# fferflo/semantic-meshes

Measured on AMD Instinct MI355X. Metric: views/sec fused (1080p, 19 classes, 1M-tri mesh), higher is better.
Workload: dtype f32; 1 GPU; cfg2: 1000000-triangle grid mesh, 11763 views/GPU at 1920x1080, 19 classes, probs resident in HBM; views_per_call=8, group_pipeline=True, repeats=1, allreduce=none, exchange=allreduce, nranks=1, allreduce_bytes=0, exchange_parts=1, held_views=0

## Files before the change

semantic_meshes_amd/csrc/common.hpp:

```cpp
#pragma once

#include <hip/hip_runtime.h>

#include <algorithm>
#include <cstdint>
#include <cstdio>
#include <cstdlib>
#include <functional>
#include <mutex>
#include <string>
#include <vector>

#include "../../include/smesh.h"

namespace smesh {

int fail(int code, const std::string& msg);
int fail_hip(hipError_t e, const char* what, const char* file, int line);

#define SMESH_HIP(expr)                                                         \
  do {                                                                          \
    hipError_t _e = (expr);                                                     \
    if (_e != hipSuccess) return ::smesh::fail_hip(_e, #expr, __FILE__, __LINE__); \
  } while (0)

#define SMESH_TRY(expr)              \
  do {                               \
    int _s = (expr);                 \
    if (_s != SMESH_OK) return _s;   \
  } while (0)

struct ProfSlot {
  std::vector<std::pair<hipEvent_t, hipEvent_t>> pending;
  std::vector<std::pair<hipEvent_t, hipEvent_t>> pool;
  double total_ms = 0.0;
  uint64_t launches = 0;
  uint64_t seen = 0;
  int depth = 0;
  bool open_timed = false;
  uint64_t timed_launches = 0;
  uint64_t timed_views = 0;
};

struct DeviceCtx {
  int device = -1;
  hipStream_t stream = nullptr;
  hipStream_t raster_stream = nullptr;
  hipStream_t exchange_stream = nullptr;
  hipEvent_t ev_order = nullptr;
  hipEvent_t ev_release = nullptr;
  int num_cus = 256;
  uint32_t lds_per_cu = 65536;
  unsigned profiling = 0;
  unsigned profile_every = 1;
  ProfSlot slots[SMESH_PROF_SLOTS];
  hipEvent_t marks[SMESH_STREAM_MARKS] = {};
  std::vector<hipEvent_t> token_pool;
  std::recursive_mutex mu;
};

int get_ctx(int device, DeviceCtx** out);

struct ProfScope {
  DeviceCtx* ctx;
  int slot;
  hipEvent_t start = nullptr, stop = nullptr;
  hipStream_t st;
  bool counted = false;
  ProfScope(DeviceCtx* c, int s, hipStream_t stream = nullptr);
  ~ProfScope();
};

void prof_note(DeviceCtx* ctx, int slot, uint64_t launches, uint64_t views);

hipError_t dev_malloc(void** out, size_t bytes);
hipError_t dev_free(void* p, bool foreign = false);
uint64_t dev_cached_bytes(int device);
void dev_trim(int device);
void dev_cache_stats(uint64_t* live_blocks, uint64_t* cached_blocks, uint64_t* cached_bytes);

bool opt_group_pipeline();
constexpr int kRasterMeshletsDefault = 1;
bool opt_raster_meshlets();
constexpr int kPipelineFitDefault = 1;
constexpr int kPipelineFuseWaves = 5;
int opt_pipeline_fit();
int opt_pipeline_fuse_waves();
int opt_pipeline_fuse_pad();

struct PipelineNeighbour {
  uint32_t wg_lds = 0, wg_vgprs = 0;
};

inline uint32_t pipeline_fuse_pad(uint32_t lds_per_cu, uint32_t static_lds, uint32_t vgprs, int want, const PipelineNeighbour& nb,
                                  int* beside = nullptr) {
  constexpr uint32_t kBlock = 1280u;
  auto blocks = [&](uint32_t bytes) { return (bytes + kBlock - 1u) / kBlock * kBlock; };
  const uint32_t n = (uint32_t)std::min(32, std::max(2, want));
  const uint32_t wg = std::max(blocks(static_lds), (lds_per_cu / (n + 1u)) / kBlock * kBlock + kBlock);
  if (beside) {
    const uint32_t alloc_f = std::max(8u, (vgprs + 7u) / 8u * 8u), alloc_r = std::max(8u, (nb.wg_vgprs + 7u) / 8u * 8u);
    const uint32_t per_simd = (n + 3u) / 4u;
    const uint32_t left = (uint64_t)wg * n <= lds_per_cu ? lds_per_cu - wg * n : 0u;
    const uint32_t regs_left = per_simd * alloc_f < 512u ? 512u - per_simd * alloc_f : 0u;
    const uint32_t by_regs = std::min(regs_left / alloc_r, per_simd < 8u ? 8u - per_simd : 0u);
    *beside = (int)std::min(by_regs, nb.wg_lds ? left / blocks(nb.wg_lds) : by_regs);
  }
  return wg - static_lds;
}
bool opt_confusion_wave_aggregate();

bool opt_probs_labels_tiles();
bool opt_resize_vector();
bool opt_fuse_sampled();
bool opt_points_grid();
constexpr uint32_t kProbsLabelsTileMaxC = 255;

constexpr uint32_t kConfusionLdsMaxC = 180;

struct Scratch {
  void* ptr = nullptr;
  size_t bytes = 0;
  int reserve(size_t need);
  void release();
};

inline uint64_t div_up(uint64_t a, uint64_t b) { return (a + b - 1) / b; }

inline int env_int(const char* name, int def) {
  const char* e = getenv(name);
  return e ? atoi(e) : def;
}

struct TriFrag {
  uint16_t x0, y0;
  uint16_t kind;
  uint16_t pad;
  unsigned long long mask;
};
static_assert(sizeof(TriFrag) == 16, "TriFrag must be 16 bytes");

struct TriFuseArgs {
  const TriFrag* frags;
  const uint32_t* idx;
  const float* probs;
  const float* weights;
  float* acc;
  float* acc_lo;
  uint64_t F;
  uint32_t C, W, H;
  float iew;
  const uint32_t* big_queue;
  const uint32_t* big_len;
  uint32_t big_capacity;
  uint32_t tri_blocks;
  uint32_t big_blocks;
  const uint32_t* prim_id;
  const uint32_t* tex_first;
  const uint32_t* tex_res;
  const uint8_t* tex_kinds;
  uint32_t* count;
  double* acc_d;
  int mid;
  uint32_t ps0, ps1;
  uint32_t blk_first;
  uint32_t f_lo, f_hi;
  uint32_t lds_pad;
};

struct TriView {
  const TriFrag* frags;
  const uint32_t* idx;
  const float* probs;
  const float* weights;
  const uint32_t* big_queue;
  const uint32_t* big_len;
  uint32_t W, H;
  uint32_t ps0, ps1;
  const uint8_t* kinds;
};
template <int NV>
struct TriViews {
  TriView v[NV];
};

struct RenderedView {
  const TriFrag* frags;
  const uint32_t* big_queue;
  const uint32_t* big_len;
  const uint32_t* idx;
  const float* probs;
  const float* weights;
  uint64_t W, H;
  int64_t ps0 = 0, ps1 = 0;
  bool mid_queue = false;
  bool no_big = false;
  const uint8_t* kinds = nullptr;
  bool fine = false;
  PipelineNeighbour beside;
  const void* image = nullptr;
};

constexpr int kMidBox = 256;

struct ImageRecords {
  TriFrag* frags = nullptr;
  uint32_t* cand = nullptr;
  uint4* big4 = nullptr;
  uint32_t* big_queue = nullptr;
  uint32_t* big_count = nullptr;
  unsigned long long* mom = nullptr;
  uint64_t P = 0;
  bool clean = false;
  bool moments = false;
  uint32_t tag = 2;
  void release();
};
int image_records_build(DeviceCtx* ctx, ImageRecords& r, const uint32_t* d_idx, uint64_t W, uint64_t H, uint64_t P);
int image_records_pending(DeviceCtx* ctx, ImageRecords& r, const uint32_t* d_idx, uint64_t W, uint64_t H, hipStream_t st);
int image_records_scatter_sparse(DeviceCtx* ctx, ImageRecords& r, int kind, const uint32_t* d_idx, const float* d_probs, const float* d_w,
                                 uint64_t W, uint64_t H, uint32_t C, float iew, float* acc, float* acc_lo, double* acc_d, hipStream_t st);
int image_records_clear(DeviceCtx* ctx, ImageRecords& r, const uint32_t* d_idx, uint64_t W, uint64_t H, hipStream_t st);
bool image_records_build_group(DeviceCtx* ctx, ImageRecords* const* recs, const uint32_t* const* d_idx, int n, uint64_t W, uint64_t H, uint64_t P,
                               int* status);
int image_records_scatter_sparse_group(DeviceCtx* ctx, ImageRecords* const* recs, int n, int kind, const uint32_t* const* d_idx,
                                       const float* const* d_probs, const float* const* d_w, uint64_t W, uint64_t H, uint32_t C, float iew,
                                       float* acc, float* acc_lo, double* acc_d, hipStream_t st);

}

struct smesh_aggregator;
struct smesh_renderer;
int smesh_aggregator_with_final_rows(smesh_aggregator* a,
                                     const std::function<int(smesh::DeviceCtx* ctx, const float* rows, uint64_t P, uint32_t C)>& use);
int smesh_renderer_texel_tables(const smesh_renderer* r, smesh::DeviceCtx** ctx, uint64_t* F, uint64_t* P, const uint32_t** first,
                                const uint32_t** res);
int smesh_rows_labels(smesh::DeviceCtx* ctx, const float* d_rows, uint64_t n, uint32_t C, float dont_care_threshold, int32_t* out_labels,
                      int out_memkind);
struct smesh_vertex_map;
int smesh_rows_finish(smesh::DeviceCtx* ctx, const float* d_rows, uint64_t n, uint32_t C, int mode, float dont_care_threshold,
                      float* out_rows, int32_t* out_labels, int out_memkind);
int smesh_vertex_map_tables(const smesh_vertex_map* m, smesh::DeviceCtx** ctx, const uint32_t** offsets, const uint32_t** list);
struct smesh_face_graph;
int smesh_face_graph_tables(const smesh_face_graph* graph, smesh::DeviceCtx** ctx, const uint32_t** offsets, const uint32_t** neighbours,
                            uint64_t* F, uint64_t* nnz);
int smesh_renderer_with_index_planes(smesh_renderer* r, const smesh_camera_t* cams, int n, uint64_t P, smesh::DeviceCtx* ctx,
                                     const std::function<int(int view, const uint32_t* idx, uint64_t W, uint64_t H)>& use);
```

semantic_meshes_amd/csrc/context.cpp:

```cpp
#include "common.hpp"
#include "labels_scratch.hpp"
#include "half_scratch.hpp"
#include "../../include/smesh_label_prep.h"
#include "../../include/smesh_label_colors.h"

#include <algorithm>
#include <atomic>

#include <cstdlib>
#include <cstring>
#include <map>
#include <memory>
#include <unordered_map>
#include <vector>

namespace smesh {

static thread_local std::string g_err;

int fail(int code, const std::string& msg) {
  g_err = msg;
  return code;
}

int fail_hip(hipError_t e, const char* what, const char* file, int line) {
  char buf[512];
  snprintf(buf, sizeof buf, "HIP error %d (%s) at %s:%d: %s", (int)e, hipGetErrorString(e), file, line, what);
  g_err = buf;
  (void)hipGetLastError();
  return (e == hipErrorNoDevice || e == hipErrorInvalidDevice) ? SMESH_ERR_NODEVICE : SMESH_ERR_RUNTIME;
}

static std::atomic<int> g_confusion_wave_aggregate{1};
bool opt_confusion_wave_aggregate() { return g_confusion_wave_aggregate.load() != 0; }

static std::atomic<int> g_probs_labels_tiles{1};
bool opt_probs_labels_tiles() { return g_probs_labels_tiles.load() != 0; }

static std::atomic<int> g_resize_vector{1};
bool opt_resize_vector() { return g_resize_vector.load() != 0; }

static std::atomic<int> g_points_grid{1};
bool opt_points_grid() { return g_points_grid.load() != 0; }

uint64_t smesh_label_prep_launches();
uint64_t smesh_label_colors_launches();
uint64_t smesh_depth_weights_launches();
uint64_t smesh_view_weights_launches();

static std::atomic<int> g_fuse_sampled{-1};
bool opt_fuse_sampled() {
  const int v = g_fuse_sampled.load();
  return (v < 0 ? env_int("SMESH_FUSE_SAMPLED", 1) : v) != 0;
}

static std::atomic<int> g_group_pipeline{-1};
bool opt_group_pipeline() {
  int v = g_group_pipeline.load();
  if (v < 0) {
    const char* e = getenv("SMESH_GROUP_PIPELINE");
    v = e ? (atoi(e) != 0 ? 1 : 0) : 1;
    g_group_pipeline.store(v);
  }
  return v != 0;
}

static std::atomic<int> g_raster_meshlets{-1};
bool opt_raster_meshlets() {
  int v = g_raster_meshlets.load();
  if (v < 0) {
    const char* e = getenv("SMESH_RASTER_MESHLETS");
    v = e ? (atoi(e) != 0 ? 1 : 0) : kRasterMeshletsDefault;
    g_raster_meshlets.store(v);
  }
  return v != 0;
}

static std::atomic<int> g_pipeline_fit{-2}, g_pipeline_fuse_waves{-2}, g_pipeline_fuse_pad{-2};
static int opt_env_once(std::atomic<int>& g, const char* env, int def, int lo, int hi) {
  int v = g.load();
  if (v == -2) {
    v = std::min(hi, std::max(lo, env_int(env, def)));
    g.store(v);
  }
  return v;
}
int opt_pipeline_fit() { return opt_env_once(g_pipeline_fit, "SMESH_PIPELINE_FIT", kPipelineFitDefault, 0, 1); }
int opt_pipeline_fuse_waves() { return opt_env_once(g_pipeline_fuse_waves, "SMESH_PIPELINE_FUSE_WAVES", kPipelineFuseWaves, 2, 32); }
int opt_pipeline_fuse_pad() { return opt_env_once(g_pipeline_fuse_pad, "SMESH_PIPELINE_FUSE_PAD", -1, -1, 65536 - 16384); }

static std::mutex g_ctx_mu;
static std::vector<std::unique_ptr<DeviceCtx>> g_ctx;

DeviceCtx* peek_ctx(int device) {
  std::lock_guard<std::mutex> lock(g_ctx_mu);
  return (device >= 0 && device < (int)g_ctx.size()) ? g_ctx[device].get() : nullptr;
}

int get_ctx(int device, DeviceCtx** out) {
  std::lock_guard<std::mutex> lock(g_ctx_mu);
  int n = 0;
  hipError_t e = hipGetDeviceCount(&n);
  if (e != hipSuccess || n <= 0) {
    (void)hipGetLastError();
    return fail(SMESH_ERR_NODEVICE, "no HIP device available (libsmesh_hip has no CPU fallback)");
  }
  if (device < 0 || device >= n) return fail(SMESH_ERR_INVALID, "device index out of range");
  if ((int)g_ctx.size() < n) g_ctx.resize(n);
  if (!g_ctx[device]) {
    SMESH_HIP(hipSetDevice(device));
    auto ctx = std::make_unique<DeviceCtx>();
    ctx->device = device;
    hipDeviceProp_t prop;
    SMESH_HIP(hipGetDeviceProperties(&prop, device));
    ctx->num_cus = prop.multiProcessorCount > 0 ? prop.multiProcessorCount : 256;
    ctx->lds_per_cu = (uint32_t)std::min<size_t>(std::max<size_t>(prop.maxSharedMemoryPerMultiProcessor, 65536), 1u << 20);
    SMESH_HIP(hipStreamCreateWithFlags(&ctx->stream, hipStreamNonBlocking));
    SMESH_HIP(hipStreamCreateWithFlags(&ctx->raster_stream, hipStreamNonBlocking));
    {
      int least = 0, greatest = 0;
      if (hipDeviceGetStreamPriorityRange(&least, &greatest) != hipSuccess) { (void)hipGetLastError(); least = greatest = 0; }
      if (hipStreamCreateWithPriority(&ctx->exchange_stream, hipStreamNonBlocking, greatest) != hipSuccess) {
        (void)hipGetLastError();
        SMESH_HIP(hipStreamCreateWithFlags(&ctx->exchange_stream, hipStreamNonBlocking));
      }
    }
    g_ctx[device] = std::move(ctx);
  }
  *out = g_ctx[device].get();
  return SMESH_OK;
}

ProfScope::ProfScope(DeviceCtx* c, int s, hipStream_t stream) : ctx(c), slot(s), st(stream ? stream : c->stream) {
  if (!(ctx->profiling & (1u << slot))) return;
  ProfSlot& ps = ctx->slots[slot];
  if (ps.depth++ > 0) { counted = true; return; }
  counted = true;
  if (ps.seen++ % (slot <= SMESH_PROF_RASTER ? std::max(1u, ctx->profile_every) : 1u) != 0) return;
  if (!ps.pool.empty()) {
    start = ps.pool.back().first;
    stop = ps.pool.back().second;
    ps.pool.pop_back();
  } else {
    if (hipEventCreate(&start) != hipSuccess || hipEventCreate(&stop) != hipSuccess) {
      start = stop = nullptr;
      return;
    }
  }
  (void)hipEventRecord(start, st);
  ps.open_timed = true;
}

void prof_note(DeviceCtx* ctx, int slot, uint64_t launches, uint64_t views) {
  ProfSlot& ps = ctx->slots[slot];
  if (ps.depth > 0 && ps.open_timed) { ps.timed_launches += launches; ps.timed_views += views; }
}
// ... 94 lines not shown
    std::lock_guard<std::mutex> lock(g_alloc_mu);
    auto it = g_live.find(p);
    if (it != g_live.end()) owner = it->second.device;
  }
  int cur = 0;
  (void)hipGetDevice(&cur);
  if (owner >= 0 && owner != cur) (void)hipSetDevice(owner);
  DeviceCtx* ctx = (owner >= 0 && !foreign) ? peek_ctx(owner) : nullptr;
  hipError_t e = hipSuccess;
  if (ctx) {
    for (hipStream_t st : {ctx->raster_stream, ctx->stream, ctx->exchange_stream})
      if (st && e == hipSuccess) e = hipStreamSynchronize(st);
  } else {
    e = hipDeviceSynchronize();
  }
  if (e != hipSuccess) (void)hipGetLastError();
  hipError_t ret = hipSuccess;
  {
    std::lock_guard<std::mutex> lock(g_alloc_mu);
    auto it = g_live.find(p);
    if (it == g_live.end()) ret = hipFree(p);
    else {
      const DevBlock b = it->second;
      g_live.erase(it);
      const size_t cap = cache_cap(b.device);
      if (b.bytes > cap) ret = hipFree(p);
      else {
        evict_locked(b.device, b.bytes, cap);
        g_cached.emplace(b.bytes, CachedBlock{p, b.device, g_alloc_stamp++});
        g_cached_bytes[b.device] += b.bytes;
      }
    }
  }
  if (owner >= 0 && owner != cur) (void)hipSetDevice(cur);
  return ret;
}

void dev_trim(int device) {
  std::lock_guard<std::mutex> lock(g_alloc_mu);
  for (auto it = g_cached.begin(); it != g_cached.end();) {
    if (device >= 0 && it->second.device != device) { ++it; continue; }
    auto victim = it++;
    really_free_locked(victim);
  }
}

void dev_cache_stats(uint64_t* live_blocks, uint64_t* cached_blocks, uint64_t* cached_bytes) {
  std::lock_guard<std::mutex> lock(g_alloc_mu);
  if (live_blocks) *live_blocks = g_live.size();
  if (cached_blocks) *cached_blocks = g_cached.size();
  if (cached_bytes) { *cached_bytes = 0; for (auto& kv : g_cached_bytes) *cached_bytes += kv.second; }
}
uint64_t dev_cached_bytes(int device) {
  std::lock_guard<std::mutex> lock(g_alloc_mu);
  uint64_t n = 0;
  for (auto& kv : g_cached_bytes) if (device < 0 || kv.first == device) n += kv.second;
  return n;
}

int Scratch::reserve(size_t need) {
  if (need <= bytes) return SMESH_OK;
  if (ptr) SMESH_HIP(dev_free(ptr));
  ptr = nullptr;
  bytes = 0;
  size_t want = need + need / 8 + 256;
  SMESH_HIP(dev_malloc(&ptr, want));
  bytes = want;
  return SMESH_OK;
}

void Scratch::release() {
  if (ptr) (void)dev_free(ptr);
  ptr = nullptr;
  bytes = 0;
}

}

using namespace smesh;

void smesh_last_fuse_instance(int* slot, int* views);
uint32_t smesh_last_fuse_lds_pad();
int smesh_last_fuse_beside();
int smesh_last_fuse_probs_dtype();

extern "C" {

const char* smesh_backend(void) { return "hip-gfx950"; }

const char* smesh_last_error(void) { return g_err.c_str(); }

int smesh_set_option(const char* name, int64_t value) {
  if (!name) return fail(SMESH_ERR_INVALID, "option name is NULL");
  if (!strcmp(name, "group_pipeline")) { g_group_pipeline.store(value != 0 ? 1 : 0); return SMESH_OK; }
  if (!strcmp(name, "raster_meshlets")) { g_raster_meshlets.store(value != 0 ? 1 : 0); return SMESH_OK; }
  if (!strcmp(name, "pipeline_fit")) { g_pipeline_fit.store(value != 0 ? 1 : 0); return SMESH_OK; }
  if (!strcmp(name, "pipeline_fuse_waves")) { g_pipeline_fuse_waves.store((int)std::min<int64_t>(32, std::max<int64_t>(2, value))); return SMESH_OK; }
  if (!strcmp(name, "pipeline_fuse_pad")) { g_pipeline_fuse_pad.store((int)std::min<int64_t>(65536 - 16384, std::max<int64_t>(-1, value))); return SMESH_OK; }
  if (!strcmp(name, "confusion_wave_aggregate")) { g_confusion_wave_aggregate.store(value != 0 ? 1 : 0); return SMESH_OK; }
  if (!strcmp(name, "probs_labels_tiles")) { g_probs_labels_tiles.store(value != 0 ? 1 : 0); return SMESH_OK; }
  if (!strcmp(name, "resize_vector")) { g_resize_vector.store(value != 0 ? 1 : 0); return SMESH_OK; }
  if (!strcmp(name, "fuse_sampled")) { g_fuse_sampled.store(value != 0 ? 1 : 0); return SMESH_OK; }
  if (!strcmp(name, "points_grid")) { g_points_grid.store(value != 0 ? 1 : 0); return SMESH_OK; }
  return fail(SMESH_ERR_INVALID, std::string("unknown option: ") + name);
}
int smesh_get_option(const char* name, int64_t* value) {
  if (!name || !value) return fail(SMESH_ERR_INVALID, "NULL argument");
  if (!strcmp(name, "group_pipeline")) { *value = opt_group_pipeline() ? 1 : 0; return SMESH_OK; }
  if (!strcmp(name, "raster_meshlets")) { *value = opt_raster_meshlets() ? 1 : 0; return SMESH_OK; }
  if (!strcmp(name, "pipeline_fit")) { *value = opt_pipeline_fit(); return SMESH_OK; }
  if (!strcmp(name, "pipeline_fuse_waves")) { *value = opt_pipeline_fuse_waves(); return SMESH_OK; }
  if (!strcmp(name, "pipeline_fuse_pad")) { *value = opt_pipeline_fuse_pad(); return SMESH_OK; }
  if (!strcmp(name, "last_fuse_lds_pad")) { *value = (int64_t)smesh_last_fuse_lds_pad(); return SMESH_OK; }
  if (!strcmp(name, "last_fuse_beside")) { *value = (int64_t)smesh_last_fuse_beside(); return SMESH_OK; }
  if (!strcmp(name, "labels_lds_max_classes")) { *value = (int64_t)kLabelsLdsMaxC; return SMESH_OK; }
  if (!strcmp(name, "half_max_classes")) { *value = (int64_t)kHalfMaxClasses; return SMESH_OK; }
  if (!strcmp(name, "last_fuse_probs_dtype")) { *value = (int64_t)smesh_last_fuse_probs_dtype(); return SMESH_OK; }
  if (!strcmp(name, "confusion_lds_max_classes")) { *value = (int64_t)kConfusionLdsMaxC; return SMESH_OK; }
  if (!strcmp(name, "confusion_wave_aggregate")) { *value = opt_confusion_wave_aggregate() ? 1 : 0; return SMESH_OK; }
  if (!strcmp(name, "probs_labels_tiles")) { *value = opt_probs_labels_tiles() ? 1 : 0; return SMESH_OK; }
  if (!strcmp(name, "resize_vector")) { *value = opt_resize_vector() ? 1 : 0; return SMESH_OK; }
  if (!strcmp(name, "fuse_sampled")) { *value = opt_fuse_sampled() ? 1 : 0; return SMESH_OK; }
  if (!strcmp(name, "points_grid")) { *value = opt_points_grid() ? 1 : 0; return SMESH_OK; }
  if (!strcmp(name, "labels_prepare_map_lds_max")) { *value = (int64_t)SMESH_LABEL_PREP_MAP_LDS_MAX; return SMESH_OK; }
  if (!strcmp(name, "labels_prepare_launches")) { *value = (int64_t)smesh_label_prep_launches(); return SMESH_OK; }
  if (!strcmp(name, "labels_colors_lds_max")) { *value = (int64_t)SMESH_LABEL_COLORS_LDS_MAX; return SMESH_OK; }
  if (!strcmp(name, "labels_colors_launches")) { *value = (int64_t)smesh_label_colors_launches(); return SMESH_OK; }
  if (!strcmp(name, "depth_weights_launches")) { *value = (int64_t)smesh_depth_weights_launches(); return SMESH_OK; }
  if (!strcmp(name, "view_weights_launches")) { *value = (int64_t)smesh_view_weights_launches(); return SMESH_OK; }
  if (!strcmp(name, "probs_labels_tile_max_classes")) { *value = (int64_t)kProbsLabelsTileMaxC; return SMESH_OK; }
  const bool want_slot = !strcmp(name, "last_fuse_slot");
  if (want_slot || !strcmp(name, "last_fuse_views")) {
    int slot, views;
    smesh_last_fuse_instance(&slot, &views);
    *value = want_slot ? slot : views;
    return SMESH_OK;
  }
  return fail(SMESH_ERR_INVALID, std::string("unknown option: ") + name);
}

int smesh_device_count(int* count) {
  if (!count) return fail(SMESH_ERR_INVALID, "count is NULL");
  int n = 0;
  if (hipGetDeviceCount(&n) != hipSuccess) {
    (void)hipGetLastError();
    n = 0;
  }
  *count = n;
  return SMESH_OK;
}

int smesh_synchronize(int device) {
  DeviceCtx* ctx;
  SMESH_TRY(get_ctx(device, &ctx));
  SMESH_HIP(hipSetDevice(device));
  SMESH_HIP(hipStreamSynchronize(ctx->raster_stream));
  SMESH_HIP(hipStreamSynchronize(ctx->stream));
  SMESH_HIP(hipStreamSynchronize(ctx->exchange_stream));
  return SMESH_OK;
}

int smesh_stream_wait(int device, void* producer_stream) {
  DeviceCtx* ctx;
  SMESH_TRY(get_ctx(device, &ctx));
  std::lock_guard<std::recursive_mutex> lock(ctx->mu);
  SMESH_HIP(hipSetDevice(device));
  hipStream_t ps = static_cast<hipStream_t>(producer_stream);
  if (ps == ctx->raster_stream) return SMESH_OK;
  if (!ctx->ev_order) SMESH_HIP(hipEventCreateWithFlags(&ctx->ev_order, hipEventDisableTiming));
  SMESH_HIP(hipEventRecord(ctx->ev_order, ps));
  if (ps != ctx->stream) SMESH_HIP(hipStreamWaitEvent(ctx->stream, ctx->ev_order, 0));
  SMESH_HIP(hipStreamWaitEvent(ctx->raster_stream, ctx->ev_order, 0));
  return SMESH_OK;
}

int smesh_stream_release(int device, void* consumer_stream) {
  DeviceCtx* ctx;
  SMESH_TRY(get_ctx(device, &ctx));
  std::lock_guard<std::recursive_mutex> lock(ctx->mu);
  SMESH_HIP(hipSetDevice(device));
  hipStream_t cs = static_cast<hipStream_t>(consumer_stream);
  if (cs == ctx->stream) return SMESH_OK;
  if (!ctx->ev_release) SMESH_HIP(hipEventCreateWithFlags(&ctx->ev_release, hipEventDisableTiming));
  SMESH_HIP(hipEventRecord(ctx->ev_release, ctx->stream));
  SMESH_HIP(hipStreamWaitEvent(cs, ctx->ev_release, 0));
  return SMESH_OK;
}

int smesh_stream_handle(int device, void** stream) {
  if (!stream) return fail(SMESH_ERR_INVALID, "stream is NULL");
  DeviceCtx* ctx;
  SMESH_TRY(get_ctx(device, &ctx));
// ... 212 lines not shown
```

semantic_meshes_amd/csrc/fuse_mid.inc.hpp:

```cpp

constexpr int kMidHits = 256;
constexpr int kRowRor1 = 0x121, kRowRor2 = 0x122, kRowRor4 = 0x124, kRowRor8 = 0x128;

__device__ __forceinline__ float row16_sum(float v) {
  v += dpp_f<kRowRor8>(0.0f, v);
  v += dpp_f<kRowRor4>(0.0f, v);
  v += dpp_f<kRowRor2>(0.0f, v);
  v += dpp_f<kRowRor1>(0.0f, v);
  return v;
}
__device__ __forceinline__ uint32_t row16_sum_u(uint32_t v) {
  v += dpp_u<kRowRor8>(0u, v);
  v += dpp_u<kRowRor4>(0u, v);
  v += dpp_u<kRowRor2>(0u, v);
  v += dpp_u<kRowRor1>(0u, v);
  return v;
}
__device__ __forceinline__ float row16_max(float v) {
  v = fmaxf(v, dpp_f<kRowRor8>(-INFINITY, v));
  v = fmaxf(v, dpp_f<kRowRor4>(-INFINITY, v));
  v = fmaxf(v, dpp_f<kRowRor2>(-INFINITY, v));
  v = fmaxf(v, dpp_f<kRowRor1>(-INFINITY, v));
  return v;
}
__device__ __forceinline__ double row16_sum_d(double v) {
#define SMESH_ROR_D(CTRL)                                                                               \
  {                                                                                                     \
    const int hi = __builtin_amdgcn_update_dpp(0, __double2hiint(v), CTRL, 0xF, 0xF, false);            \
    const int lo = __builtin_amdgcn_update_dpp(0, __double2loint(v), CTRL, 0xF, 0xF, false);            \
    v += __hiloint2double(hi, lo);                                                                      \
  }
  SMESH_ROR_D(kRowRor8) SMESH_ROR_D(kRowRor4) SMESH_ROR_D(kRowRor2) SMESH_ROR_D(kRowRor1)
#undef SMESH_ROR_D
  return v;
}

typedef __attribute__((address_space(3))) uint16_t lds_u16;
template <int CT, int KIND, int NV>
__device__ __forceinline__ void fuse_mid_entries(const TriFuseArgs& a, const TriViews<NV>& vw, const uint32_t worker, const uint32_t nworkers,
                                                 lds_u16* __restrict__ hit_lds) {
  static_assert(KIND != SMESH_AGG_MUL, "fuse_mid_entries adds with float atomics: Sum and Summax only");
  const int C = (int)a.C;
  const int l16 = (int)(threadIdx.x & 15u);
  const uint32_t slot = worker * 4u + (threadIdx.x >> 4), nslots = nworkers * 4u;
  uint32_t len[NV], total = 0u;
#pragma unroll
  for (int v = 0; v < NV; v++) { len[v] = min(vw.v[v].big_len[3], a.big_capacity); total += len[v]; }
  if (total == 0u) return;
  lds_u16* __restrict__ my_hits = hit_lds + ((threadIdx.x >> 4) & 3u) * kMidHits;
  struct Entry { uint32_t fi; int view; TriFrag rec; };
  auto fetch = [&](const uint32_t q) -> Entry {
    Entry e;
    e.fi = 0u; e.view = -1;
    e.rec.x0 = 0; e.rec.y0 = 0; e.rec.kind = 0; e.rec.pad = 0; e.rec.mask = 0ull;
    uint32_t qq = q;
    int jsel = -1;
    bool located = q >= total;
#pragma unroll
    for (int j = 0; j < NV; j++) {
      if (!located) {
        if (qq < len[j]) { jsel = j; located = true; }
        else qq -= len[j];
      }
    }
    if (jsel >= 0) {
      const TriView& w = vw.v[jsel];
      e.fi = w.big_queue[(uint64_t)a.big_capacity + qq];
      e.rec = w.frags[e.fi];
      e.view = jsel;
    }
    return e;
  };
  Entry next = fetch(slot);
  for (uint32_t q0 = 0; q0 < total; q0 += nslots) {
    const uint32_t q = q0 + slot;
    const Entry cur = next;
    next = fetch(q + nslots);
    const uint32_t fi = cur.fi;
    const TriFrag rec = cur.rec;
    const TriView& cw = vw.v[cur.view >= 0 ? cur.view : 0];
    const uint32_t* __restrict__ idx = cw.idx;
    const float* __restrict__ probs = cw.probs;
    const float* __restrict__ weights = cw.weights;
    const uint32_t vH = cw.H, ps0 = cw.ps0, ps1 = cw.ps1;
    const bool on = cur.view >= 0 && rec.kind == 2 && mid_box(rec, 0u, 0u);
    if (__ballot(on) == 0ull) continue;
    const uint32_t pid = (a.prim_id && on) ? a.prim_id[fi] : fi;
    const int x0 = rec.x0, y0 = rec.y0;
    const int x1 = (int)(rec.mask & 0xFFFFu), y1 = (int)((rec.mask >> 16) & 0xFFFFu);
    const int bh = on ? y1 - y0 + 1 : 1;
    const int npx = on ? (x1 - x0 + 1) * bh : 0;
    unsigned long long hits = 0ull;
    {
      int cx = l16 / bh, cy = l16 - cx * bh;
      for (int base = 0; __ballot(base < npx) != 0ull; base += 16 * 8) {
        uint32_t got[8];
#pragma unroll
        for (int u = 0; u < 8; u++) {
          const bool in = base + u * 16 + l16 < npx;
          got[u] = idx[(uint64_t)(uint32_t)(x0 + (in ? cx : 0)) * vH + (uint32_t)(y0 + (in ? cy : 0))];
          if (!in) got[u] = ~pid;
          cy += 16;
          while (cy >= bh) { cy -= bh; cx++; }
        }
#pragma unroll
        for (int u = 0; u < 8; u++) if (got[u] == pid) hits |= 1ull << (base / 16 + u);
      }
    }
    const uint32_t mine_n = (uint32_t)__popcll(hits);
    const uint32_t ntot = row16_sum_u(mine_n);
    const float w0 = ntot ? a.iew * (1.0f / (float)ntot) + (1 - a.iew) * 1.0f : 0.0f;
    uint32_t incl = mine_n;
    incl += dpp_u<kDppRowShr1>(0u, incl);
    incl += dpp_u<kDppRowShr2>(0u, incl);
    incl += dpp_u<kDppRowShr4>(0u, incl);
    incl += dpp_u<kDppRowShr8>(0u, incl);
    const bool compact = ntot <= (uint32_t)kMidHits;
    if (compact) {
      uint32_t at = incl - mine_n;
      for (unsigned long long m = hits; m; m &= m - 1ull) my_hits[at++] = (uint16_t)(l16 + 16 * (__ffsll((long long)m) - 1));
    }
    wave_sync();
    float tri[CT];
#pragma unroll
    for (int c = 0; c < CT; c++) tri[c] = 0.0f;
    const float inv_bh = 1.0f / (float)bh;
    uint32_t round = 0u;
    while (true) {
      bool have;
      int i;
      if (compact) {
        const uint32_t e = round * 16u + (uint32_t)l16;
        have = e < ntot;
        i = have ? (int)my_hits[e] : 0;
      } else {
        have = hits != 0ull;
        i = have ? l16 + 16 * (__ffsll((long long)hits) - 1) : 0;
        hits &= hits - 1ull;
      }
      round++;
      if (__ballot(have) == 0ull) break;
      int ix = (int)(((float)i + 0.5f) * inv_bh);
      int iy = i - ix * bh;
      if (iy < 0) { ix--; iy += bh; } else if (iy >= bh) { ix++; iy -= bh; }
      const uint32_t hx = (uint32_t)(x0 + ix), hy = (uint32_t)(y0 + iy);
      float p[CT];
      load_row<CT, false>(probs + ((uint64_t)hx * ps0 + (uint64_t)hy * ps1), C, p);
      const float wt = (weights && have) ? weights[(uint64_t)hx * vH + hy] : 1.0f;
      float sum = 0.0f;
#pragma unroll
      for (int c = 0; c < CT; c++) if (c < C) sum = sum + p[c];
// ... 34 lines not shown
```

semantic_meshes_amd/csrc/fuse_tri.inc.hpp:

```cpp

constexpr int kWave = 64;

__device__ __forceinline__ float log_spec(float x) {
  if (!(x > 0.0f)) return x == 0.0f ? -INFINITY : NAN;
  if (x == INFINITY) return INFINITY;
  int e_adj = 0;
  uint32_t ix = __float_as_uint(x);
  if (ix < 0x00800000u) { x = x * 8388608.0f; e_adj = -23; ix = __float_as_uint(x); }
  int e = (int)(ix >> 23) - 127 + e_adj;
  uint32_t im = (ix & 0x007FFFFFu) | 0x3F800000u;
  if ((ix & 0x007FFFFFu) > 0x003504F3u) { im -= 0x00800000u; e += 1; }
  const float f = __uint_as_float(im) - 1.0f;
  const float z = f * f;
  float y = 7.0376836292e-2f;
  y = __builtin_fmaf(y, f, -1.1514610310e-1f);
  y = __builtin_fmaf(y, f, 1.1676998740e-1f);
  y = __builtin_fmaf(y, f, -1.2420140846e-1f);
  y = __builtin_fmaf(y, f, 1.4249322787e-1f);
  y = __builtin_fmaf(y, f, -1.6668057665e-1f);
  y = __builtin_fmaf(y, f, 2.0000714765e-1f);
  y = __builtin_fmaf(y, f, -2.4999993993e-1f);
  y = __builtin_fmaf(y, f, 3.3333331174e-1f);
  y = (y * f) * z;
  const float fe = (float)e;
// ... 189 lines not shown
    if (KIND == SMESH_AGG_SUMMAX) {
      float best = p[0];
      int am = 0;
#pragma unroll
      for (int c = 1; c < CT; c++) if (EXACT || c < C) if (p[c] > best) { best = p[c]; am = c; }
#pragma unroll
      for (int c = 0; c < CT; c++) if (EXACT || c < C) part[c] = (c == am) ? part[c] + p[c] * w : part[c];
    } else {
#pragma unroll
      for (int c = 0; c < CT; c++) if (EXACT || c < C) part[c] += (bpart_t)contribution<KIND>(p[c], w);
    }
  };
  if (one_step && n <= (uint32_t)kWave) {
    uint32_t at = upto - mine_n;
#pragma unroll
    for (int u = 0; u < U; u++)
      if (hits & (1u << u)) lds_list[at++] = (uint32_t)pix_of((long long)u * kWave + l);
    wave_sync();
    const bool hit = (uint32_t)l < n;
    const uint64_t pix = lds_list[hit ? l : 0];
    wave_sync();
    float p[CT];
    load_row<CT, EXACT>(probs_at(pix), C, p);
    const float wt = (a.weights && hit) ? a.weights[pix] : 1.0f;
    accumulate(p, hit, wt);
    float* rows = reinterpret_cast<float*>(lds_list);
    if (hit) {
#pragma unroll
      for (int c = 0; c < CT; c++) if (EXACT || c < C) rows[l * C + c] = (float)part[c];
    }
    wave_sync();
    bpart_t col = (bpart_t)0;
    if (l < C)
      for (uint32_t j = 0; j < n; j++) col += (bpart_t)rows[j * (uint32_t)C + (uint32_t)l];
    wave_sync();
    if (l < C) write_back(col);
    return;
  } else {
    for (long long base = 0; base < npx; base += (long long)kWave * U) {
      uint64_t pix[U];
      bool hit[U];
#pragma unroll
      for (int u = 0; u < U; u++) {
        const long long i = base + (long long)u * kWave + l;
        pix[u] = i < npx ? pix_of(i) : pix_of(0);
        hit[u] = a.idx[pix[u]] == f && i < npx;
      }
      float p[U][CT];
      float wt[U];
#pragma unroll
      for (int u = 0; u < U; u++) {
        const float* __restrict__ pr = probs_at(hit[u] ? pix[u] : pix_of(0));
        load_row<CT, EXACT>(pr, C, p[u]);
        wt[u] = (a.weights && hit[u]) ? a.weights[pix[u]] : 1.0f;
      }
#pragma unroll
      for (int u = 0; u < U; u++) accumulate(p[u], hit[u], wt[u]);
    }
  }
  bpart_t mine = (bpart_t)0;
#pragma unroll
  for (int c = 0; c < CT; c++) if (EXACT || c < C) {
    bpart_t v;
    if constexpr (KIND == SMESH_AGG_MUL) v = wave_sum_d(part[c]); else v = wave_sum(part[c]);
    if (l == c) mine = v;
  }
  if (l < C) write_back(mine);
}

__device__ __forceinline__ TriFuseArgs with_view(const TriFuseArgs& a, const TriView& w) {
  TriFuseArgs x = a;
  x.frags = w.frags; x.idx = w.idx; x.probs = w.probs; x.weights = w.weights; x.big_queue = w.big_queue; x.big_len = w.big_len;
  x.W = w.W; x.H = w.H; x.ps0 = w.ps0; x.ps1 = w.ps1;
  return x;
}

__device__ __forceinline__ bool mid_box(const TriFrag& rec, uint32_t W, uint32_t H) {
  (void)W; (void)H;
  if (rec.kind != 2) return true;
  const int w = (int)(rec.mask & 0xFFFFu) - (int)rec.x0 + 1, h = (int)((rec.mask >> 16) & 0xFFFFu) - (int)rec.y0 + 1;
  return w * h <= kMidBox;
}

template <int CT, int KIND, bool EXACT, int NV>
__device__ __forceinline__ void fuse_big_triangles(const TriFuseArgs& a, const TriViews<NV>& vw, uint32_t worker, uint32_t nworkers,
                                                   uint32_t* __restrict__ lds_list) {
  uint32_t len[NV], total = 0u;
#pragma unroll
  for (int v = 0; v < NV; v++) { len[v] = min(*vw.v[v].big_len, a.big_capacity); total += len[v]; }
  const int l = threadIdx.x;
  const uint32_t chunk = max(1u, min((uint32_t)kWave, total / max(nworkers, 1u)));
  const uint32_t steps = (total + chunk - 1u) / chunk;
  for (uint32_t step = worker; step < steps; step += nworkers) {
    const uint32_t q = (uint32_t)l < chunk ? (uint32_t)l * steps + step : total;
    uint32_t fi = 0u;
    bool take = false;
    {
      uint32_t qq = q;
      bool located = q >= total;
      int jsel = -1;
#pragma unroll
      for (int j = 0; j < NV; j++) {
        if (!located) {
          if (qq < len[j]) { fi = vw.v[j].big_queue[qq]; jsel = j; located = true; }
          else qq -= len[j];
        }
      }
      if (jsel >= 0) {
        bool mine = false, earlier = false;
#pragma unroll
        for (int i = 0; i < NV; i++) {
          if (i <= jsel) {
            const TriFrag rec = vw.v[i].frags[fi];
            const bool counts = rec.kind == 2 && !(a.mid && mid_box(rec, vw.v[i].W, vw.v[i].H));
            if (i < jsel) earlier = earlier || counts;
            else mine = counts;
          }
        }
        take = mine && !earlier && fi >= a.f_lo && fi < a.f_hi;
      }
    }
    unsigned long long todo = __ballot(take);
    while (todo) {
      const int src = __ffsll((long long)todo) - 1;
      todo &= todo - 1ull;
      const uint32_t fq = (uint32_t)__builtin_amdgcn_readlane((int)fi, src);
      const uint32_t f = a.prim_id ? a.prim_id[fq] : fq;
#pragma unroll
      for (int j = 0; j < NV; j++) {
        const TriFrag rec = vw.v[j].frags[fq];
        if (rec.kind == 0 || (a.mid && rec.kind == 2 && mid_box(rec, 0u, 0u))) continue;
        const TriFuseArgs x = with_view(a, vw.v[j]);
        int x1, y1;
        if (rec.kind == 2) { x1 = (int)(rec.mask & 0xFFFFu); y1 = (int)((rec.mask >> 16) & 0xFFFFu); }
        else { x1 = min((int)rec.x0 + 7, (int)x.W - 1); y1 = min((int)rec.y0 + 7, (int)x.H - 1); }
        const bool by_mask = rec.kind == 1 && !a.prim_id && vw.v[j].big_len[1] == 0u;
        fuse_box<CT, KIND, EXACT>(x, f, rec.x0, rec.y0, x1, y1, lds_list, by_mask, rec.mask);
      }
    }
  }
}

#include "fuse_mid.inc.hpp"

constexpr int fuse_tri_min_waves(int ct, int kind, int nv) { return (ct >= 19 && ct <= 21 && kind != SMESH_AGG_MUL && (nv != 2 || ct == 19)) ? 3 : 1; }
template <int CT, int KIND, bool EXACT, int NV>
__global__ __launch_bounds__(kWave) __attribute__((amdgpu_waves_per_eu(fuse_tri_min_waves(CT, KIND, NV)))) void k_fuse_tri(TriFuseArgs a, TriViews<NV> vw) {
  const int C = EXACT ? CT : (int)a.C;
  constexpr int PB = CT <= 24 ? 2 : 1;
  constexpr int KV = (kWave * CT / 4 + kWave - 1) / kWave;
  constexpr int kSrow = (kWave * CT + 4) > (4 * kMidHits / 2) ? (kWave * CT + 4) : (4 * kMidHits / 2);
  __shared__ __attribute__((aligned(16))) float srow[kSrow];
  const int l = threadIdx.x;
  if (blockIdx.x >= a.tri_blocks) {
    const uint32_t tail = blockIdx.x - a.tri_blocks;
    if (tail < a.big_blocks) {
      uint32_t* lds_list = reinterpret_cast<uint32_t*>(srow);
      fuse_big_triangles<CT, KIND, EXACT, NV>(a, vw, tail, a.big_blocks, lds_list);
    } else if constexpr (KIND != SMESH_AGG_MUL) {
      constexpr int MCT = (CT + 7) / 8 * 8;
      fuse_mid_entries<MCT, KIND, NV>(a, vw, tail - a.big_blocks, gridDim.x - a.tri_blocks - a.big_blocks, (lds_u16*)srow);
    }
    return;
  }
  const uint64_t f0 = ((uint64_t)a.blk_first + blockIdx.x) * kWave;
  const uint64_t f = f0 + l;
  uint32_t org[NV];
  unsigned long long msk[NV];
  bool big = false, large = false;
#pragma unroll
  for (int v = 0; v < NV; v++) { org[v] = 0u; msk[v] = 0ull; }
  if (f < a.F) {
#pragma unroll
    for (int v = 0; v < NV; v++) {
      const TriFrag rec = vw.v[v].frags[f];
      org[v] = (uint32_t)rec.x0 | ((uint32_t)rec.y0 << 16);
      msk[v] = rec.kind == 1 ? rec.mask : 0ull;
      big = big || rec.kind == 2;
      large = large || (rec.kind == 2 && !(KIND != SMESH_AGG_MUL && a.mid && mid_box(rec, 0u, 0u)));
    }
  }
  if (large) {
#pragma unroll
    for (int v = 0; v < NV; v++) msk[v] = 0ull;
  }
  const bool scattered = a.prim_id != nullptr;
  const uint32_t pid = (scattered && f < a.F) ? a.prim_id[f] : (uint32_t)f;
  auto pixel = [&](int v, int k) -> uint64_t {
    return (uint64_t)((org[v] & 0xFFFFu) + (uint32_t)(k >> 3)) * vw.v[v].H + (org[v] >> 16) + (uint32_t)(k & 7);
  };

  bool verify = scattered;
#pragma unroll
  for (int v = 0; v < NV; v++) verify = verify || vw.v[v].big_len[1] != 0u;
  if (verify) {
#pragma unroll
    for (int v = 0; v < NV; v++) {
      if (!scattered && vw.v[v].big_len[1] == 0u) continue;
      const uint32_t* __restrict__ idx = vw.v[v].idx;
      unsigned long long m = msk[v], win = 0ull;
      while (__ballot(m != 0ull) != 0ull) {
        int k[4];
        uint32_t got[4];
#pragma unroll
        for (int j = 0; j < 4; j++) {
          k[j] = -1;
          if (m) { k[j] = __ffsll((long long)m) - 1; m &= m - 1ull; }
          got[j] = idx[k[j] >= 0 ? pixel(v, k[j]) : 0];
        }
#pragma unroll
        for (int j = 0; j < 4; j++)
          if (k[j] >= 0 && got[j] == pid) win |= 1ull << k[j];
      }
      msk[v] = win;
    }
  }
  unsigned long long any_win = 0ull;
#pragma unroll
  for (int v = 0; v < NV; v++) any_win |= msk[v];
  if (__ballot(any_win != 0ull) == 0ull) return;

  const int nrows = (int)min((uint64_t)kWave, a.F - f0);
  float* __restrict__ blk = a.acc + f0 * C;
  f4 br[KV];
  if (nrows == kWave && !scattered) {
    const f4* b4 = reinterpret_cast<const f4*>(blk);
#pragma unroll
    for (int q = 0; q < KV; q++) br[q] = b4[min(l + q * kWave, kWave * C / 4 - 1)];
  }
  float accr[CT];
  bool rows_loaded = false;
  typedef double part_t;
  constexpr int PT = KIND == SMESH_AGG_MUL ? CT : 1;
#pragma unroll
  for (int v = 0; v < NV; v++) {
    part_t part[PT];
#pragma unroll
    for (int c = 0; c < PT; c++) part[c] = (part_t)0;
    const float* __restrict__ probs = vw.v[v].probs;
    const float* __restrict__ weights = vw.v[v].weights;
    const uint32_t nv = (uint32_t)__popcll(msk[v]);
    float w0 = 0.0f;
    if (nv) {
      const float image_weight = 1.0f / ((float)nv);
      const float pixel_w = 1.0f;
      w0 = a.iew * image_weight + (1 - a.iew) * pixel_w;
    }
    unsigned long long mm = msk[v];
    while (__ballot(mm != 0ull) != 0ull) {
      float p[PB][CT];
      float wt[PB];
      bool have[PB];
#pragma unroll
      for (int j = 0; j < PB; j++) {
        have[j] = mm != 0ull;
// ... 100 lines not shown
```

semantic_meshes_amd/csrc/fusion.hip:

```cpp
#include "common.hpp"
#include "labels_scratch.hpp"
#include "half_scratch.hpp"

#include <algorithm>
#include <cmath>
#include <cstdlib>
#include <new>
#include <cstring>
#include <string>
#include <sys/mman.h>
#include <thread>
#include <type_traits>

using namespace smesh;

void smesh_launch_fuse_tri_multi(int kind, int tri_ct, int nviews, dim3 grid, hipStream_t st, const TriFuseArgs& t, const TriViews<8>& tv);
bool smesh_fuse_tri_8_resources(int kind, int tri_ct, uint32_t* static_lds, uint32_t* vgprs);

namespace {

#include "fuse_tri.inc.hpp"


template <typename T>
// ... 2006 lines not shown
      SMESH_HIP(hipGetLastError());
    }
  }
  return SMESH_OK;
}

int normalize_idx(DeviceCtx* ctx, Scratch& scratch, const void* d_idx, int idx_dtype, const int64_t is[2],
                  uint64_t W, uint64_t H, const uint32_t** out) {
  const uint64_t N = W * H;
  if (is[0] == (int64_t)H && is[1] == 1 && (idx_dtype == SMESH_IDX_U32 || idx_dtype == SMESH_IDX_I32)) {
    *out = static_cast<const uint32_t*>(d_idx);
    return SMESH_OK;
  }
  SMESH_TRY(scratch.reserve(N * 4));
  uint32_t* o = static_cast<uint32_t*>(scratch.ptr);
  const dim3 g((uint32_t)div_up(N, 256)), b(256);
  hipStream_t st = ctx->stream;
  switch (idx_dtype) {
    case SMESH_IDX_U32: hipLaunchKernelGGL(k_gather_idx<uint32_t>, g, b, 0, st, (const uint32_t*)d_idx, is[0], is[1], o, N, (uint32_t)H); break;
    case SMESH_IDX_I32: hipLaunchKernelGGL(k_gather_idx<int32_t>, g, b, 0, st, (const int32_t*)d_idx, is[0], is[1], o, N, (uint32_t)H); break;
    case SMESH_IDX_U64: hipLaunchKernelGGL(k_gather_idx<uint64_t>, g, b, 0, st, (const uint64_t*)d_idx, is[0], is[1], o, N, (uint32_t)H); break;
    default:            hipLaunchKernelGGL(k_gather_idx<int64_t>, g, b, 0, st, (const int64_t*)d_idx, is[0], is[1], o, N, (uint32_t)H); break;
  }
  SMESH_HIP(hipGetLastError());
  *out = o;
  return SMESH_OK;
}

int check_strides(const int64_t* s, int n, const char* what) {
  if (!s) return fail(SMESH_ERR_INVALID, std::string(what) + ": strides are NULL");
  for (int i = 0; i < n; i++)
    if (s[i] < 0) return fail(SMESH_ERR_INVALID, std::string(what) + ": negative strides are not supported");
  return SMESH_OK;
}

}

int smesh_aggregator_add_device_contig(smesh_aggregator* a, const uint32_t* d_idx, const float* d_probs,
                                       const float* d_w, uint64_t W, uint64_t H) {
  const int64_t is[2] = {(int64_t)H, 1};
  const int64_t ps[3] = {(int64_t)(H * a->C), (int64_t)a->C, 1};
  return add_device(a, d_idx, SMESH_IDX_U32, is, d_probs, ps, d_w, is, W, H);
}

static bool fuse_strip_forced() {
  static const bool on = [] { const char* e = getenv("SMESH_FUSE"); return e && std::string(e) == "strip"; }();
  return on;
}

bool smesh_aggregator_can_fuse_triangles(smesh_aggregator* a, uint64_t F) {
  return !fuse_strip_forced() && a->P == F && a->C <= 64u * (uint32_t)kSliceAny;
}

constexpr uint32_t kFuseTriMaxC = 48;

static bool fuse_wide_enabled() {
  static const bool on = env_int("SMESH_FUSE_WIDE", 1) != 0;
  return on;
}
const char* smesh_aggregator_fuse_kernel_name(smesh_aggregator* a, bool reordered) {
  if (a->C <= kFuseTriMaxC) return "k_fuse_tri";
  (void)reordered;
  if (fuse_wide_enabled() && a->C >= 128 && a->C <= 1024) return "k_fuse_tri_wide";
  return "k_fuse_tri_any";
}

int smesh_aggregator_max_fused_views(smesh_aggregator* a);
bool smesh_aggregator_fuses_small_views_by_mask(smesh_aggregator* a);
bool smesh_aggregator_takes_strided_probs(smesh_aggregator* a, int64_t ps0, int64_t ps1, int nviews);
bool smesh_aggregator_can_fuse_pair(smesh_aggregator* a) { return smesh_aggregator_max_fused_views(a) >= 2; }

int smesh_aggregator_max_fused_views(smesh_aggregator* a) {
  static const int cap = std::max(1, env_int("SMESH_FUSE_VIEWS", 8));
  int m = a->C <= 40u ? 8 : (a->C <= (uint32_t)kFuseTriMaxC ? 2 : 1);
  if (a->C > (uint32_t)kFuseTriMaxC) m = 8;
  if (a->C > 40u && a->C <= (uint32_t)kFuseTriMaxC && a->kind != SMESH_AGG_MUL) m = 8;
  return std::min(m, cap);
}

bool smesh_aggregator_fuses_small_views_by_mask(smesh_aggregator* a) {
  return a->C <= 40u || (a->C <= (uint32_t)kFuseTriMaxC && a->kind == SMESH_AGG_MUL && smesh_aggregator_max_fused_views(a) <= 2);
}

bool smesh_aggregator_takes_strided_probs(smesh_aggregator* a, int64_t ps0, int64_t ps1, int nviews) {
  if (ps0 <= 0 || ps1 <= 0 || ps0 > 0xFFFFFFFFll || ps1 > 0xFFFFFFFFll) return false;
  return a->C <= kFuseTriMaxC && !(a->C > 40u && nviews > 2);
}

void smesh_fuse_part_rows(uint64_t F, int part, int nparts, uint64_t* f_lo, uint64_t* f_hi) {
  const uint64_t B = div_up(F, 64);
  *f_lo = std::min(F, 64 * (B * (uint64_t)part / (uint64_t)nparts));
  *f_hi = std::min(F, 64 * (B * (uint64_t)(part + 1) / (uint64_t)nparts));
}

template <int KIND>
static bool launch_fuse_wide_list(int wide_chunks, uint32_t C, dim3 grid, hipStream_t st, const TriFuseArgs& t, const TriViews<8>& tv, int nviews) {
  static const bool off = env_int("SMESH_WIDE_LIST", 1) == 0;
  if constexpr (KIND != SMESH_AGG_SUM) return false;
  else {
    if (off || wide_chunks != 1 || C >= 256u) return false;
    hipLaunchKernelGGL((k_fuse_tri_wide_list<KIND, 1>), grid, dim3(kWave), 0, st, t, tv, nviews);
    return true;
  }
}

static thread_local int g_last_fuse_slot = -1;
static thread_local int g_last_fuse_views = 0;
static thread_local uint32_t g_last_fuse_lds_pad = 0u;
static thread_local int g_last_fuse_beside = -1;
uint32_t smesh_last_fuse_lds_pad() { return g_last_fuse_lds_pad; }
int smesh_last_fuse_beside() { return g_last_fuse_beside; }
void smesh_last_fuse_instance(int* slot, int* views) { *slot = g_last_fuse_slot; *views = g_last_fuse_views; }
void smesh_set_last_fuse_instance(int slot, int views) { g_last_fuse_slot = slot; g_last_fuse_views = views; }

int smesh_aggregator_fuse_triangles(smesh_aggregator* a, uint64_t F, const uint32_t* prim_id, uint32_t big_capacity,
                                    const RenderedView* views, int nviews, int part, int nparts) {
  DeviceCtx* ctx = a->ctx;
  hipStream_t st = ctx->stream;
  if (F == 0) return SMESH_OK;
  if (nparts < 1 || part < 0 || part >= nparts) return fail(SMESH_ERR_INVALID, "fuse_triangles: bad part");
  SMESH_TRY(smesh_aggregator_refuse_scattered(a, "fuse_view()"));
  uint64_t f_lo, f_hi;
  smesh_fuse_part_rows(F, part, nparts, &f_lo, &f_hi);
  if (f_lo >= f_hi && part != 0) return SMESH_OK;
  if ((nviews != 1 && nviews != 2 && nviews != 4 && nviews != 8) || nviews > smesh_aggregator_max_fused_views(a))
    return fail(SMESH_ERR_INVALID, "fuse_triangles: unsupported view count");
  const uint64_t N = views[0].W * views[0].H;
  TriFuseArgs t;
  TriViews<8> tv;
  for (int v = 0; v < 8; v++) {
    const RenderedView& rv = views[v < nviews ? v : 0];
    tv.v[v] = TriView{rv.frags, rv.idx, rv.probs, rv.weights, rv.big_queue, rv.big_len, (uint32_t)rv.W, (uint32_t)rv.H,
                      rv.ps0 ? (uint32_t)rv.ps0 : (uint32_t)(rv.H * a->C), rv.ps1 ? (uint32_t)rv.ps1 : a->C};
  }
  for (int v = 0; v < nviews; v++)
    if ((views[v].ps0 || views[v].ps1) && !smesh_aggregator_takes_strided_probs(a, views[v].ps0, views[v].ps1, nviews))
      return fail(SMESH_ERR_INVALID, "fuse_triangles: strided class vectors need the narrow-row kernel");
  for (int v = 0; v < 1; v++) {
    const RenderedView& rv = views[0];
    TriFuseArgs& x = t;
    x.frags = rv.frags; x.idx = rv.idx; x.probs = rv.probs; x.weights = rv.weights; x.acc = a->acc; x.acc_lo = a->acc_lo; x.F = F; x.C = a->C;
    x.W = (uint32_t)rv.W; x.H = (uint32_t)rv.H; x.iew = a->iew; x.big_queue = rv.big_queue; x.big_len = rv.big_len;
    x.ps0 = tv.v[0].ps0; x.ps1 = tv.v[0].ps1;
    x.big_capacity = big_capacity;
    x.tri_blocks = (uint32_t)div_up(F, kWave);
    x.tex_first = nullptr; x.tex_res = nullptr; x.count = nullptr; x.acc_d = nullptr;
    x.prim_id = prim_id;
    x.mid = 0;
    x.lds_pad = 0u;
    x.blk_first = (uint32_t)(f_lo / kWave);
    x.tri_blocks = (uint32_t)div_up(f_hi - f_lo, kWave);
    x.f_lo = (uint32_t)f_lo; x.f_hi = (uint32_t)f_hi;
  }
  int tri_ct = 0;
  if (a->C <= kFuseTriMaxC && !(a->C > 40u && nviews > 2)) {
    if (a->C == 5 || a->C == 13 || a->C == 19 || a->C == 20 || a->C == 21 || a->C == 40) tri_ct = (int)a->C;
    else tri_ct = a->C <= 8 ? 8 : a->C <= 16 ? 16 : a->C <= 24 ? 24 : a->C <= 32 ? 32 : a->C <= 40 ? 41 : 48;
  }
  const bool specialised = tri_ct != 0;
  float* pw = nullptr;
  uint32_t* amax = nullptr;
  uint64_t scratch_stride = N;
  int G = 1;
  const int wide_chunks = (fuse_wide_enabled() && a->C >= 128 && a->C <= 1024) ? (a->C <= 256 ? 1 : a->C <= 512 ? 2 : 4) : 0;
  if (!specialised) {
    while ((((a->C + G - 1) / G + 3u) & ~3u) > (uint32_t)kSliceAny) G *= 2;
    for (int v = 0; v < nviews; v++) scratch_stride = std::max<uint64_t>(scratch_stride, views[v].W * views[v].H);
    SMESH_TRY(a->pw.reserve(scratch_stride * (uint64_t)nviews * 4));
    pw = static_cast<float*>(a->pw.ptr);
    if (a->kind == SMESH_AGG_SUMMAX) {
      SMESH_TRY(a->fb_amax.reserve(scratch_stride * (uint64_t)nviews * 4));
      amax = static_cast<uint32_t*>(a->fb_amax.ptr);
    }
    const uint64_t tpb = wide_chunks ? (uint64_t)kWave : (uint64_t)(kWave / G);
    t.blk_first = (uint32_t)(f_lo / tpb);
    t.tri_blocks = (uint32_t)div_up(f_hi - f_lo, tpb);
  }
  constexpr uint32_t big_per_cu = 16;
  bool no_big = true;
  for (int v = 0; v < nviews; v++) no_big = no_big && views[v].no_big;
  const uint32_t big_waves = no_big ? 0u : std::max((uint32_t)std::max(1, ctx->num_cus), big_per_cu * (uint32_t)std::max(1, ctx->num_cus) / (uint32_t)nparts);
  uint32_t mid_waves = 0;
  if (specialised) {
    bool listed = true;
    for (int v = 0; v < nviews; v++) listed = listed && views[v].mid_queue;
    if (listed && a->kind != SMESH_AGG_MUL) {
      t.mid = 1;
      constexpr uint32_t mid_per_cu = 32;
      if (part == 0 && !no_big) mid_waves = mid_per_cu * (uint32_t)std::max(1, ctx->num_cus);
    }
  }
  t.big_blocks = big_waves;
  {
    bool fine = true;
    for (int v = 0; v < nviews; v++) fine = fine && views[v].fine;
    t.lds_pad = 0u;
    if (fine && opt_group_pipeline() && nparts == 1 && nviews == 8 && specialised) {
      uint32_t static_lds = 0u, vgprs = 0u;
      const int forced = opt_pipeline_fuse_pad();
      if (forced >= 0) t.lds_pad = (uint32_t)forced;
      else if (!opt_pipeline_fit() || !smesh_fuse_tri_8_resources(a->kind, tri_ct, &static_lds, &vgprs)) t.lds_pad = 24576u;
      else t.lds_pad = pipeline_fuse_pad(ctx->lds_per_cu, static_lds, vgprs, opt_pipeline_fuse_waves(), views[0].beside, &g_last_fuse_beside);
    }
    g_last_fuse_lds_pad = t.lds_pad;
  }
  const dim3 grid(t.tri_blocks + big_waves + mid_waves), block(kWave);
  const dim3 tgrid(t.tri_blocks), bgrid(big_waves);
  if (!specialised && part == 0) SMESH_TRY(mul_recentre(a));
  {
    ProfScope prof(ctx, SMESH_PROF_FUSE_SCATTER);
    prof_note(ctx, SMESH_PROF_FUSE_SCATTER, 1, part == 0 ? (uint64_t)nviews : 0);
    g_last_fuse_slot = tri_ct; g_last_fuse_views = nviews;
#define SMESH_FA(K)                                                                            \
    switch (G) {                                                                               \
      case 1:  hipLaunchKernelGGL((k_fuse_tri_any<K, 1>), tgrid, block, 0, st, t, tv, nviews); break;  \
      case 2:  hipLaunchKernelGGL((k_fuse_tri_any<K, 2>), tgrid, block, 0, st, t, tv, nviews); break;  \
      case 4:  hipLaunchKernelGGL((k_fuse_tri_any<K, 4>), tgrid, block, 0, st, t, tv, nviews); break;  \
      case 8:  hipLaunchKernelGGL((k_fuse_tri_any<K, 8>), tgrid, block, 0, st, t, tv, nviews); break;  \
      case 16: hipLaunchKernelGGL((k_fuse_tri_any<K, 16>), tgrid, block, 0, st, t, tv, nviews); break; \
      case 32: hipLaunchKernelGGL((k_fuse_tri_any<K, 32>), tgrid, block, 0, st, t, tv, nviews); break; \
      default: hipLaunchKernelGGL((k_fuse_tri_any<K, 64>), tgrid, block, 0, st, t, tv, nviews); break; \
    }
#define SMESH_FW(K)                                                                            \
    switch (wide_chunks) {                                                                     \
      case 1:  if (K == SMESH_AGG_MUL) hipLaunchKernelGGL((k_fuse_tri_wide<K, 1, 4>), tgrid, block, 0, st, t, tv, nviews); \
               else hipLaunchKernelGGL((k_fuse_tri_wide<K, 1, 2>), tgrid, block, 0, st, t, tv, nviews); break; \
      case 2:  hipLaunchKernelGGL((k_fuse_tri_wide<K, 2, 2>), tgrid, block, 0, st, t, tv, nviews); break; \
      default: hipLaunchKernelGGL((k_fuse_tri_wide<K, 4, 2>), tgrid, block, 0, st, t, tv, nviews); break; \
    }
#define SMESH_FT(K)                                                                           \
    switch (tri_ct) {                                                                         \
      case 5:  hipLaunchKernelGGL((k_fuse_tri<5, K, true, 1>), grid, block, 0, st, t, tv1); break;     \
      case 13: hipLaunchKernelGGL((k_fuse_tri<13, K, true, 1>), grid, block, 0, st, t, tv1); break;    \
      case 19: hipLaunchKernelGGL((k_fuse_tri<19, K, true, 1>), grid, block, 0, st, t, tv1); break;    \
      case 20: hipLaunchKernelGGL((k_fuse_tri<20, K, true, 1>), grid, block, 0, st, t, tv1); break;    \
      case 21: hipLaunchKernelGGL((k_fuse_tri<21, K, true, 1>), grid, block, 0, st, t, tv1); break;    \
      case 40: hipLaunchKernelGGL((k_fuse_tri<40, K, true, 1>), grid, block, 0, st, t, tv1); break;    \
      case 8:  hipLaunchKernelGGL((k_fuse_tri<8, K, false, 1>), grid, block, 0, st, t, tv1); break;    \
      case 16: hipLaunchKernelGGL((k_fuse_tri<16, K, false, 1>), grid, block, 0, st, t, tv1); break;   \
      case 24: hipLaunchKernelGGL((k_fuse_tri<24, K, false, 1>), grid, block, 0, st, t, tv1); break;   \
      case 32: hipLaunchKernelGGL((k_fuse_tri<32, K, false, 1>), grid, block, 0, st, t, tv1); break;   \
      case 41: hipLaunchKernelGGL((k_fuse_tri<40, K, false, 1>), grid, block, 0, st, t, tv1); break;   \
// ... 761 lines not shown
```

semantic_meshes_amd/csrc/raster.hip:

```cpp
#include "common.hpp"
#include "meshlets.hpp"
#include "half_scratch.hpp"
#include "depth_gate.hpp"
#include "../../include/smesh_meshlets.h"

#include <algorithm>
#include <cmath>
#include <cstdlib>
#include <cstring>
#include <new>
#include <string>
#include <utility>
#include <vector>

#pragma clang fp contract(off)

using namespace smesh;

struct smesh_aggregator;
int smesh_aggregator_add_device_contig(smesh_aggregator* a, const uint32_t* d_idx, const float* d_probs,
                                       const float* d_w, uint64_t W, uint64_t H);
bool smesh_aggregator_can_fuse_triangles(smesh_aggregator* a, uint64_t F);
bool smesh_aggregator_can_fuse_pair(smesh_aggregator* a);
int smesh_aggregator_max_fused_views(smesh_aggregator* a);
bool smesh_aggregator_takes_strided_probs(smesh_aggregator* a, int64_t ps0, int64_t ps1, int nviews);
int smesh_aggregator_dense_probs(smesh_aggregator* a, const float* d_probs, const int64_t ps[3], uint64_t W, uint64_t H, const float** out);
bool smesh_aggregator_fuses_small_views_by_mask(smesh_aggregator* a);
int smesh_aggregator_fuse_triangles(smesh_aggregator* a, uint64_t F, const uint32_t* prim_id, uint32_t big_capacity,
                                    const RenderedView* views, int nviews, int part = 0, int nparts = 1);
void smesh_fuse_part_rows(uint64_t F, int part, int nparts, uint64_t* f_lo, uint64_t* f_hi);
uint64_t smesh_aggregator_primitives(smesh_aggregator* a);
int smesh_aggregator_join_exchange(smesh_aggregator* a);
const char* smesh_aggregator_fuse_kernel_name(smesh_aggregator* a, bool reordered);
bool smesh_aggregator_can_fuse_texels(smesh_aggregator* a, uint64_t P);
int smesh_aggregator_fuse_texels(smesh_aggregator* a, const TriFrag* frags, const uint8_t* kinds, uint64_t F, const uint32_t* tex_first,
                                 const uint32_t* tex_res, const uint32_t* big_queue, const uint32_t* big_len,
                                 uint32_t big_capacity, const uint32_t* d_idx, const float* d_probs, const float* d_w, uint64_t H);
int smesh_aggregator_fuse_texels_multi(smesh_aggregator* a, uint64_t F, const uint32_t* tex_first, const uint32_t* tex_res, uint32_t big_capacity,
                                       const RenderedView* views, int nviews);
DeviceCtx* smesh_aggregator_ctx(smesh_aggregator* a);
uint32_t smesh_aggregator_classes(smesh_aggregator* a);
std::mutex& smesh_aggregator_mutex(smesh_aggregator* a);
Scratch& smesh_aggregator_stage_probs(smesh_aggregator* a);
Scratch& smesh_aggregator_stage_w(smesh_aggregator* a);
bool smesh_labels_native(smesh_aggregator* a, uint64_t F, uint64_t N);
int smesh_labels_fuse_triangles(smesh_aggregator* a, uint64_t F, uint32_t big_capacity, const RenderedView* views, int nviews, int label_bytes);
int smesh_labels_expand(smesh_aggregator* a, const void* plane, int label_bytes, uint64_t N, const float** probs);
bool smesh_half_native(smesh_aggregator* a, uint64_t F);
bool smesh_half_takes_strides(int64_t ps0, int64_t ps1);
int smesh_half_fuse_triangles(smesh_aggregator* a, uint64_t F, uint32_t big_capacity, const RenderedView* views, int nviews, int probs_dtype);
bool smesh_sampled_native(smesh_aggregator* a, uint64_t F);
int smesh_sampled_fuse_triangles(smesh_aggregator* a, uint64_t F, uint32_t big_capacity, const RenderedView* views, int nviews, const SampledSrc& src);
int smesh_half_widen(smesh_aggregator* a, const void* probs, int probs_dtype, const int64_t s[3], uint64_t W, uint64_t H, const float** out,
                     int slot = 0, size_t slot_bytes = 0, int nslots = 1);

namespace {

constexpr float kNear = 1e-6f;
constexpr unsigned long long kBackgroundKey = (0x7F800000ull << 32) | 0xFFFFFFFFull;

struct ScreenVertex {
  double u, v;
  double iz;
};
constexpr double kBehind = -1.0;

struct CameraArgs {
  float R[9];
  float t[3];
  double fx, fy, cx, cy;
  uint32_t W, H;
};

__device__ __forceinline__ ScreenVertex project_point(const CameraArgs& cam, const float X, const float Y, const float Z) {
  const float xc = ((cam.R[0] * X + cam.R[1] * Y) + cam.R[2] * Z) + cam.t[0];
  const float yc = ((cam.R[3] * X + cam.R[4] * Y) + cam.R[5] * Z) + cam.t[1];
  const float zc = ((cam.R[6] * X + cam.R[7] * Y) + cam.R[8] * Z) + cam.t[2];
  ScreenVertex s;
  s.u = 0.0; s.v = 0.0; s.iz = 0.0;
  const bool fin = isfinite(xc) && isfinite(yc) && isfinite(zc);
  if (zc > kNear && fin) {
    const double zd = (double)zc;
    const double u = cam.fx * ((double)xc / zd) + cam.cx;
    const double v = cam.fy * ((double)yc / zd) + cam.cy;
    if (isfinite(u) && isfinite(v)) {
      s.u = u; s.v = v; s.iz = 1.0 / zd;
    }
  } else if (fin) {
    s.iz = kBehind;
  }
  return s;
}

__device__ __forceinline__ void project_vertex(const float* __restrict__ verts, uint64_t V, const CameraArgs& cam,
                                               ScreenVertex* __restrict__ sv, uint32_t* __restrict__ big_count, const uint64_t i) {
  if (i == 0) { big_count[0] = 0u; big_count[1] = 0u; big_count[2] = 0u; big_count[3] = 0u; big_count[4] = 0u; big_count[5] = 0u; }
  if (i >= V) return;
  sv[i] = project_point(cam, verts[3 * i + 0], verts[3 * i + 1], verts[3 * i + 2]);
}

__global__ void k_project_vertices(const float* __restrict__ verts, uint64_t V, CameraArgs cam,
                                   ScreenVertex* __restrict__ sv, uint32_t* __restrict__ big_count) {
  project_vertex(verts, V, cam, sv, big_count, (uint64_t)blockIdx.x * blockDim.x + threadIdx.x);
}

constexpr int kMaxGroup = 8;
struct ProjectGroup {
  const float* verts;
  uint64_t V;
  CameraArgs cam[kMaxGroup];
// ... 55 lines not shown
  t.e0 = make_edge(b.u, b.v, c.u, c.v);
  t.e1 = make_edge(c.u, c.v, a.u, a.v);
  t.e2 = make_edge(a.u, a.v, b.u, b.v);
  const double area2 = eval_edge(t.e2, c.u, c.v);
  if (!(area2 != 0.0) || !isfinite(area2)) return false;
  if (area2 < 0.0) { flip_edge(t.e0); flip_edge(t.e1); flip_edge(t.e2); }
  t.cls0 = edge_classes(t.e0);
  t.cls1 = edge_classes(t.e1);
  t.cls2 = edge_classes(t.e2);
  t.iz0 = a.iz; t.iz1 = b.iz; t.iz2 = c.iz;
  return true;
}

struct Shaded { bool ok; float z; double b1, b2; };
__device__ __forceinline__ Shaded shade(const Tri& t, int x, int y, bool want_bary) {
  Shaded r; r.ok = false; r.z = 0.0f; r.b1 = 0.0; r.b2 = 0.0;
  const double px = (double)x + 0.5, py = (double)y + 0.5;
  const double w0 = eval_edge(t.e0, px, py);
  if (!edge_accepts(w0, t.cls0)) return r;
  const double w1 = eval_edge(t.e1, px, py);
  if (!edge_accepts(w1, t.cls1)) return r;
  const double w2 = eval_edge(t.e2, px, py);
  if (!edge_accepts(w2, t.cls2)) return r;
  const double num = (w0 + w1) + w2;
  const double den = __builtin_fma(w2, t.iz2, __builtin_fma(w1, t.iz1, w0 * t.iz0));
  const float zf = (float)(num / den);
  if (!(zf > 0.0f) || !isfinite(zf)) return r;
  r.ok = true; r.z = zf;
  if (want_bary) { r.b1 = w1 / num; r.b2 = w2 / num; }
  return r;
}

__device__ __forceinline__ bool covered(const Tri& t, int x, int y) {
  const double px = (double)x + 0.5, py = (double)y + 0.5;
  const double w0 = eval_edge(t.e0, px, py);
  if (!edge_accepts(w0, t.cls0)) return false;
  const double w1 = eval_edge(t.e1, px, py);
  if (!edge_accepts(w1, t.cls1)) return false;
  const double w2 = eval_edge(t.e2, px, py);
  return edge_accepts(w2, t.cls2);
}

__device__ __forceinline__ uint32_t texel_of(uint32_t res, double b1, double b2) {
  const float u = (float)b1, v = (float)b2;
  const float fu = (u - 1e-6f) * (float)res, fv = (v - 1e-6f) * (float)res;
  int tu = (int)fu, tv = (int)fv;
  if (tu < 0) tu = 0;
  if (tv < 0) tv = 0;
  const int r1 = (int)res - 1;
  if (tu > r1) tu = r1;
  if (tv > r1 - tu) tv = r1 - tu;
  const int row = tu + tv;
  return (uint32_t)(row * (row + 1) / 2 + tu);
}

constexpr int kQW = 32, kQH = 64, kQPixels = kQW * kQH;
constexpr int kQSub = 4;
constexpr int kMedium = 64;
constexpr unsigned long long kNullKey = ~0ull;

struct FragQueues {
  unsigned long long* key = nullptr;
  uint16_t* pix = nullptr;
  uint32_t* count = nullptr;
  uint32_t* flag = nullptr;
  uint32_t cap = 0, tiles_y = 0;
};

struct RasterArgs {
  const int32_t* faces;
  const float* verts;
  CameraArgs cam;
  const ScreenVertex* sv;
  const uint32_t* prim_id;
  const uint32_t* tex_res;
  const uint32_t* tex_first;
  unsigned long long* keys;
  uint64_t F, V;
  uint32_t W, H;
  uint32_t* big_queue;
  uint32_t* huge_queue;
  uint32_t* big_count;
  uint32_t big_capacity;
  TriFrag* frags;
  uint8_t* kinds;
  FragQueues q;
  uint32_t tpw;
  uint32_t groups;
  uint32_t* med_queue;
  uint32_t balance;
  uint32_t wg_push;
  uint32_t spread;
  uint32_t idx_optional;
};

__device__ __forceinline__ uint64_t key_index(uint32_t x, uint32_t y, uint32_t H) { return (uint64_t)x * H + y; }

__device__ __forceinline__ ScreenVertex screen_vertex(const RasterArgs& a, const int32_t i) {
  if (a.sv) return a.sv[i];
  return project_point(a.cam, a.verts[3 * (uint64_t)i + 0], a.verts[3 * (uint64_t)i + 1], a.verts[3 * (uint64_t)i + 2]);
}

__device__ __forceinline__ bool load_tri(const RasterArgs& a, uint64_t f, Tri& t, const int32_t i0, const int32_t i1, const int32_t i2);
__device__ __forceinline__ bool load_tri(const RasterArgs& a, uint64_t f, Tri& t) {
  return load_tri(a, f, t, a.faces[3 * f + 0], a.faces[3 * f + 1], a.faces[3 * f + 2]);
}
__device__ __forceinline__ bool load_tri(const RasterArgs& a, uint64_t f, Tri& t, const int32_t i0, const int32_t i1, const int32_t i2) {
  if ((uint64_t)max((uint32_t)i0, max((uint32_t)i1, (uint32_t)i2)) >= a.V) return false;
  if (a.tex_res && a.tex_res[f] == 0) return false;
  const ScreenVertex va = screen_vertex(a, i0), vb = screen_vertex(a, i1), vc = screen_vertex(a, i2);
  return setup_tri(va, vb, vc, a.W, a.H, t);
}

struct CamPoint { float x, y, z; };
__device__ __forceinline__ CamPoint camera_point(const CameraArgs& cam, const float* __restrict__ verts, const int32_t i) {
  const float X = verts[3 * (uint64_t)i + 0], Y = verts[3 * (uint64_t)i + 1], Z = verts[3 * (uint64_t)i + 2];
  CamPoint c;
  c.x = ((cam.R[0] * X + cam.R[1] * Y) + cam.R[2] * Z) + cam.t[0];
  c.y = ((cam.R[3] * X + cam.R[4] * Y) + cam.R[5] * Z) + cam.t[1];
  c.z = ((cam.R[6] * X + cam.R[7] * Y) + cam.R[8] * Z) + cam.t[2];
  return c;
}
struct ClipVertex { ScreenVertex s; double b1, b2; };
__device__ __forceinline__ bool clip_edge(const CameraArgs& cam, const CamPoint& F, const double fb1, const double fb2,
                                          const CamPoint& B, const double bb1, const double bb2, ClipVertex& out) {
  const double zn = (double)kNear;
  const double t = ((double)F.z - zn) / ((double)F.z - (double)B.z);
  const double x = __builtin_fma(t, (double)B.x - (double)F.x, (double)F.x);
  const double y = __builtin_fma(t, (double)B.y - (double)F.y, (double)F.y);
  const double u = cam.fx * (x / zn) + cam.cx;
  const double v = cam.fy * (y / zn) + cam.cy;
  out.s.u = u; out.s.v = v; out.s.iz = 1.0 / zn;
  out.b1 = __builtin_fma(t, bb1 - fb1, fb1);
  out.b2 = __builtin_fma(t, bb2 - fb2, fb2);
  return isfinite(u) && isfinite(v);
}

__device__ __forceinline__ int clip_class(const ScreenVertex& va, const ScreenVertex& vb, const ScreenVertex& vc) {
  if (va.iz == 0.0 || vb.iz == 0.0 || vc.iz == 0.0) return -1;
  const int nfront = (va.iz > 0.0 ? 1 : 0) + (vb.iz > 0.0 ? 1 : 0) + (vc.iz > 0.0 ? 1 : 0);
  return nfront == 3 ? 0 : (nfront == 0 ? -1 : nfront);
}

__device__ __forceinline__ bool clip_piece(const RasterArgs& a, const int32_t i0, const int32_t i1, const int32_t i2,
                                           const ScreenVertex& va, const ScreenVertex& vb, const ScreenVertex& vc,
                                           const int nfront, const int p, ClipVertex& q0, ClipVertex& q1, ClipVertex& q2) {
  if (nfront == 1 && p != 0) return false;
  const int k = nfront == 1 ? (va.iz > 0.0 ? 0 : (vb.iz > 0.0 ? 1 : 2)) : (!(va.iz > 0.0) ? 0 : (!(vb.iz > 0.0) ? 1 : 2));
  const int32_t is = k == 0 ? i0 : (k == 1 ? i1 : i2), in = k == 0 ? i1 : (k == 1 ? i2 : i0), ip = k == 0 ? i2 : (k == 1 ? i0 : i1);
  const CamPoint cs = camera_point(a.cam, a.verts, is), cn = camera_point(a.cam, a.verts, in), cp = camera_point(a.cam, a.verts, ip);
  const double s1 = k == 1 ? 1.0 : 0.0, s2 = k == 2 ? 1.0 : 0.0;
  const double n1 = k == 0 ? 1.0 : 0.0, n2 = k == 1 ? 1.0 : 0.0;
  const double p1 = k == 2 ? 1.0 : 0.0, p2 = k == 0 ? 1.0 : 0.0;
  const ScreenVertex& ss = k == 0 ? va : (k == 1 ? vb : vc);
  const ScreenVertex& sn = k == 0 ? vb : (k == 1 ? vc : va);
  const ScreenVertex& sp = k == 0 ? vc : (k == 1 ? va : vb);
  if (nfront == 1) {
    q0.s = ss; q0.b1 = s1; q0.b2 = s2;
    const bool ok1 = clip_edge(a.cam, cs, s1, s2, cn, n1, n2, q1);
    const bool ok2 = clip_edge(a.cam, cs, s1, s2, cp, p1, p2, q2);
    return ok1 && ok2;
  }
  ClipVertex inb, ipb;
  const bool ok1 = clip_edge(a.cam, cn, n1, n2, cs, s1, s2, inb);
  const bool ok2 = clip_edge(a.cam, cp, p1, p2, cs, s1, s2, ipb);
  if (!ok1 || !ok2) return false;
  q0.s = sn; q0.b1 = n1; q0.b2 = n2;
  if (p == 0) { q1.s = sp; q1.b1 = p1; q1.b2 = p2; q2 = ipb; }
  else        { q1 = ipb; q2 = inb; }
  return true;
}

__device__ __forceinline__ bool clip_bbox(const RasterArgs& a, const int32_t i0, const int32_t i1, const int32_t i2,
                                          const ScreenVertex& va, const ScreenVertex& vb, const ScreenVertex& vc, const int nfront,
                                          int& x0, int& y0, int& x1, int& y1) {
  ClipVertex q0, q1, q2;
  if (!clip_piece(a, i0, i1, i2, va, vb, vc, nfront, nfront == 2 ? 1 : 0, q0, q1, q2)) return false;
  double minu = fmin(q0.s.u, fmin(q1.s.u, q2.s.u)), maxu = fmax(q0.s.u, fmax(q1.s.u, q2.s.u));
  double minv = fmin(q0.s.v, fmin(q1.s.v, q2.s.v)), maxv = fmax(q0.s.v, fmax(q1.s.v, q2.s.v));
// ... 277 lines not shown
constexpr int kSpread = (kLaneBox / 8) * (kLaneBox / 8);
constexpr int kSpreadTris = 64 / kSpread;
__device__ __forceinline__ void coop_reserve(const RasterArgs& a, const Tri& t, const uint32_t sub, uint32_t (&rb)[6]) {
  const int tX0 = t.x0 / kQW, tY0 = t.y0 / kQH;
  const int ntx = t.x1 / kQW - tX0 + 1, nty = t.y1 / kQH - tY0 + 1;
  auto reserve = [&](int j) -> uint32_t {
    if (j >= ntx * nty) return 0u;
    const int jx = tX0 + j / nty, jy = tY0 + j % nty;
    const int wx = min(t.x1, jx * kQW + kQW - 1) - max(t.x0, jx * kQW) + 1, hy = min(t.y1, jy * kQH + kQH - 1) - max(t.y0, jy * kQH) + 1;
    return atomicAdd(&a.q.count[((uint32_t)jx * a.q.tiles_y + (uint32_t)jy) * kQSub + sub], (uint32_t)(wx * hy));
  };
#pragma unroll
  for (int j = 0; j < 6; j++) rb[j] = reserve(j);
}
template <bool TEX>
__device__ __forceinline__ void coop_walk(const RasterArgs& a, const Tri& t, const uint32_t (&rb)[6], const int src, const uint64_t fsrc,
                                          const uint32_t psrc, const uint32_t sub) {
  const int lane = threadIdx.x & 63;
  const uint32_t rb0 = rb[0], rb1 = rb[1], rb2 = rb[2], rb3 = rb[3], rb4 = rb[4], rb5 = rb[5];
    auto bi = [&](int v) -> int { return __builtin_amdgcn_readlane(v, src); };
    auto bd = [&](double v) -> double { return __hiloint2double(bi(__double2hiint(v)), bi(__double2loint(v))); };
    const int X0 = bi(t.x0), X1 = bi(t.x1), Y0 = bi(t.y0), Y1 = bi(t.y1);
    const double e0A = bd(t.e0.A), e0B = bd(t.e0.B), e0C = bd(t.e0.C);
    const double e1A = bd(t.e1.A), e1B = bd(t.e1.B), e1C = bd(t.e1.C);
    const double e2A = bd(t.e2.A), e2B = bd(t.e2.B), e2C = bd(t.e2.C);
    const double iz0 = bd(t.iz0), iz1 = bd(t.iz1), iz2 = bd(t.iz2);
    const int c0 = bi(t.cls0), c1 = bi(t.cls1), c2 = bi(t.cls2);
    const uint32_t fb = (uint32_t)bi((int)(uint32_t)fsrc);
    const uint32_t fbid = (uint32_t)bi((int)psrc);
    uint32_t tfirst = 0u, tres = 0u;
    if constexpr (TEX) { tfirst = a.tex_first[fb]; tres = a.tex_res[fb]; }
    const int tX0 = X0 / kQW, tY0 = Y0 / kQH, nty = Y1 / kQH - tY0 + 1;
    const uint32_t sb0 = (uint32_t)bi((int)rb0), sb1 = (uint32_t)bi((int)rb1), sb2 = (uint32_t)bi((int)rb2),
                   sb3 = (uint32_t)bi((int)rb3), sb4 = (uint32_t)bi((int)rb4), sb5 = (uint32_t)bi((int)rb5);
    const int bh = Y1 - Y0 + 1, area = (X1 - X0 + 1) * bh;
    const uint32_t bh_rcp = bh > 1 ? 0xFFFFFFFFu / (uint32_t)bh + 1u : 0u;
    for (int i = lane; i < area + lane; i += 64) {
      const bool in_box = i < area;
      const int col = bh > 1 ? (int)__umulhi((uint32_t)i, bh_rcp) : i;
      const int x = X0 + (in_box ? col : 0), y = Y0 + (in_box ? i - col * bh : 0);
      const double px = (double)x + 0.5, py = (double)y + 0.5;
      const double w0 = __builtin_fma(e0A, px, __builtin_fma(e0B, py, e0C));
      const double w1 = __builtin_fma(e1A, px, __builtin_fma(e1B, py, e1C));
      const double w2 = __builtin_fma(e2A, px, __builtin_fma(e2B, py, e2C));
      const bool cov = edge_accepts(w0, c0) && edge_accepts(w1, c1) && edge_accepts(w2, c2);
      unsigned long long key = kNullKey;
      if (in_box && cov) {
        const double num = (w0 + w1) + w2;
        const double den = __builtin_fma(w2, iz2, __builtin_fma(w1, iz1, w0 * iz0));
        const float zf = (float)(num / den);
        if (zf > 0.0f && isfinite(zf)) {
          uint32_t prim = fbid;
          if constexpr (TEX) prim = tfirst + texel_of(tres, w1 / num, w2 / num);
          key = ((unsigned long long)__float_as_uint(zf) << 32) | prim;
        }
      }
      const int jx = x / kQW, jy = y / kQH;
      const int xlo = max(X0, jx * kQW), ylo = max(Y0, jy * kQH), hy = min(Y1, jy * kQH + kQH - 1) - ylo + 1;
      const int jt = (jx - tX0) * nty + (jy - tY0);
      const uint32_t tb = jt == 0 ? sb0 : jt == 1 ? sb1 : jt == 2 ? sb2 : jt == 3 ? sb3 : jt == 4 ? sb4 : sb5;
      const uint32_t slot = tb + (uint32_t)((x - xlo) * hy + (y - ylo));
      const uint32_t tile = (uint32_t)jx * a.q.tiles_y + (uint32_t)jy;
      if (!in_box) continue;
      if (slot < a.q.cap) {
        const uint64_t e = ((uint64_t)tile * kQSub + sub) * a.q.cap + slot;
        a.q.key[e] = key;
        a.q.pix[e] = (uint16_t)((x - jx * kQW) * kQH + (y - jy * kQH));
      } else if (key != kNullKey) {
        atomicMin(&a.keys[key_index((uint32_t)x, (uint32_t)y, a.H)], key);
        atomicOr(&a.q.flag[tile], 1u);
        a.big_count[1] = 1u;
      }
    }
}

template <int MODE, bool ML = false, bool NULLABLE_SV = false>
__device__ __forceinline__ void raster_frag_64(const RasterArgs& a, const uint64_t f, const int32_t i0, const int32_t i1, const int32_t i2,
                                               const uint32_t sub, const int part_in = -1, const bool listed = false,
                                               const MeshletTri* ml = nullptr) {
  constexpr bool kWgPush = (MODE & 1) != 0, kSpreadMode = (MODE & 2) != 0, kTex = (MODE & 4) != 0;
  const int lane = threadIdx.x & 63;
  const int part = kSpreadMode ? part_in : -1;
  const bool owner = part <= 0 && !listed;
  TriFrag rec;
  rec.x0 = 0; rec.y0 = 0; rec.kind = 0; rec.pad = 0; rec.mask = 0ull;
  Tri t;
  t.x0 = 0; t.y0 = 0; t.x1 = -1; t.y1 = -1;
  unsigned long long cover = 0ull;
  int CX0 = 0, CY0 = 0;
  bool medium = false, lanebox = false, small = false;
  bool q_big = false, q_mid = false, q_huge = false;
  const uint32_t pid = (a.prim_id && f < a.F) ? a.prim_id[f] : (uint32_t)f;
  int have = 0;
  if constexpr (ML) { if (f < a.F) have = load_tri_ml(a, f, t, *ml); }
  else { if (f < a.F) have = load_tri_ex<NULLABLE_SV>(a, f, t, i0, i1, i2); }
  if (have) {
    const int bw = t.x1 - t.x0 + 1, bh = t.y1 - t.y0 + 1;
    rec.x0 = (uint16_t)t.x0; rec.y0 = (uint16_t)t.y0;
    CX0 = t.x0; CY0 = t.y0;
    if (bw > 8 || bh > 8 || have == 2) {
      q_big = owner;
      q_mid = owner && bw * bh <= kMidBox;
      rec.kind = 2;
      rec.mask = (unsigned long long)(uint32_t)t.x1 | ((unsigned long long)(uint32_t)t.y1 << 16);
      if (bw <= kLaneBox && bh <= kLaneBox && have == 1) {
        if (part < 0) lanebox = true;
        else {
          constexpr int kSub = kLaneBox / 8;
          CX0 = t.x0 + 8 * (part / kSub); CY0 = t.y0 + 8 * (part % kSub);
          const int sw = min(t.x1 - CX0 + 1, 8), sh = min(t.y1 - CY0 + 1, 8);
          if (sw > 0 && sh > 0) cover = walk_box(t, CX0, CY0, sw, sh);
        }
      } else if (owner) {
        if (bw <= kMedium && bh <= kMedium && have == 1) medium = true;
        else q_huge = true;
      }
    } else if (owner) {
      small = true;
      cover = walk_box(t, t.x0, t.y0, bw, bh);
    }
  }
  {
    __shared__ uint32_t s_push[kWgPush ? 3 : 1][6];
    const int wv = (int)(threadIdx.x >> 6);
    (void)wv; (void)s_push;
    uint32_t* const counter[3] = {a.big_count, a.big_count + 3, a.big_count + 2};
    const bool want[3] = {q_big, q_mid, q_huge};
    uint32_t slot[3];
    if constexpr (kWgPush) {
      unsigned long long m[3];
#pragma unroll
      for (int q = 0; q < 3; q++) {
        m[q] = __ballot(want[q]);
        if (lane == 0) s_push[q][wv] = (uint32_t)__popcll(m[q]);
      }
      __syncthreads();
      if (threadIdx.x == 0u) {
        uint32_t total[3], base[3] = {0u, 0u, 0u};
#pragma unroll
        for (int q = 0; q < 3; q++) total[q] = s_push[q][0] + s_push[q][1] + s_push[q][2] + s_push[q][3];
        if (total[0]) base[0] = atomicAdd(a.big_count, total[0]);
        if (total[1]) base[1] = atomicAdd(a.big_count + 3, total[1]);
        if (total[2]) base[2] = atomicAdd(a.big_count + 2, total[2]);
#pragma unroll
        for (int q = 0; q < 3; q++) s_push[q][4] = base[q];
      }
      __syncthreads();
#pragma unroll
      for (int q = 0; q < 3; q++) {
        uint32_t before = s_push[q][4];
        for (int w = 0; w < wv; w++) before += s_push[q][w];
        slot[q] = want[q] ? before + (uint32_t)__popcll(m[q] & ((1ull << lane) - 1ull)) : 0xFFFFFFFFu;
      }
      __syncthreads();
    } else {
#pragma unroll
      for (int q = 0; q < 3; q++) {
        const unsigned long long m = __ballot(want[q]);
        slot[q] = 0xFFFFFFFFu;
        if (m == 0ull) continue;
        const int leader = __ffsll((long long)m) - 1;
        uint32_t base = 0u;
        if (lane == leader) base = atomicAdd(counter[q], (uint32_t)__popcll(m));
        base = (uint32_t)__shfl((int)base, leader);
        if (want[q]) slot[q] = base + (uint32_t)__popcll(m & ((1ull << lane) - 1ull));
      }
    }
    if (q_big && slot[0] < a.big_capacity) a.big_queue[slot[0]] = (uint32_t)f;
    if (q_mid && slot[1] < a.big_capacity) a.big_queue[(uint64_t)a.big_capacity + slot[1]] = (uint32_t)f;
    if (q_huge && slot[2] < a.big_capacity) a.huge_queue[slot[2]] = (uint32_t)f;
  }
  {
    const unsigned long long mask = emit_cover<kTex>(a, t, f, pid, CX0, CY0, cover, sub);
    if (mask && small) rec.kind = 1;
    if (rec.kind == 1) rec.mask = mask;
  }
  if (owner) {
    if (a.frags && f < a.F && (rec.kind != 0 || !a.kinds)) a.frags[f] = rec;
    if (a.kinds && f < a.F) a.kinds[f] = (uint8_t)rec.kind;
  }
  if constexpr (kWgPush && !kSpreadMode) {
    if (a.balance >= 2u) {
      const unsigned long long m = __ballot(lanebox);
      if (m != 0ull) {
        const int leader = __ffsll((long long)m) - 1;
        uint32_t base = 0u;
        if (lane == leader) base = atomicAdd(a.big_count + 5, (uint32_t)__popcll(m));
        base = (uint32_t)__shfl((int)base, leader);
        if (lanebox) a.med_queue[a.big_capacity - 1u - (base + (uint32_t)__popcll(m & ((1ull << lane) - 1ull)))] = (uint32_t)f;
      }
      lanebox = false;
    }
  }
  if ((int)__popcll(__ballot(lanebox)) < kLaneBoxMin) { medium = medium || lanebox; lanebox = false; }
  if (__ballot(lanebox) != 0ull) {
    constexpr int kSub = kLaneBox / 8;
    for (int k = 0; k < kSub * kSub; k++) {
      const int X0 = t.x0 + 8 * (k / kSub), Y0 = t.y0 + 8 * (k % kSub);
      const int bw = lanebox ? min(t.x1 - X0 + 1, 8) : 0, bh = lanebox ? min(t.y1 - Y0 + 1, 8) : 0;
      const bool on = bw > 0 && bh > 0;
      if (__ballot(on) == 0ull) continue;
      const unsigned long long cv = on ? walk_box(t, X0, Y0, bw, bh) : 0ull;
      (void)emit_cover<kTex>(a, t, f, pid, on ? X0 : 0, on ? Y0 : 0, cv, sub);
    }
  }

  uint32_t rb[6] = {0u, 0u, 0u, 0u, 0u, 0u};
  if constexpr (kWgPush) {
    if (a.balance) {
      const unsigned long long m = __ballot(medium);
      if (m != 0ull) {
        const int leader = __ffsll((long long)m) - 1;
        uint32_t base = 0u;
        if (lane == leader) base = atomicAdd(a.big_count + 4, (uint32_t)__popcll(m));
        base = (uint32_t)__shfl((int)base, leader);
        if (medium) a.med_queue[base + (uint32_t)__popcll(m & ((1ull << lane) - 1ull))] = (uint32_t)f;
      }
      return;
    }
  }
  if (medium) coop_reserve(a, t, sub, rb);
  unsigned long long todo = __ballot(medium);
  while (todo) {
    const int src = __ffsll((long long)todo) - 1;
    todo &= todo - 1ull;
    coop_walk<kTex>(a, t, rb, src, f, pid, sub);
  }
}

template <bool TEX>
__device__ __forceinline__ void raster_medium_wave(const RasterArgs& a, const uint32_t wave, const uint32_t nwaves) {
  const int lane = threadIdx.x & 63;
  const uint32_t n = min(a.big_count[4], a.big_capacity);
  for (uint32_t i = wave; i < n; i += nwaves) {
    const uint32_t g = a.med_queue[i];
    if (g >= a.F) continue;
    const int32_t g0 = a.faces[3 * (uint64_t)g + 0], g1 = a.faces[3 * (uint64_t)g + 1], g2 = a.faces[3 * (uint64_t)g + 2];
    Tri t;
    if (load_tri_ex<true>(a, g, t, g0, g1, g2) != 1) continue;
    uint32_t rb[6] = {0u, 0u, 0u, 0u, 0u, 0u};
    if (lane == 0) coop_reserve(a, t, i & (kQSub - 1), rb);
    coop_walk<TEX>(a, t, rb, 0, g, a.prim_id ? a.prim_id[g] : g, i & (kQSub - 1));
  }
  constexpr int kLanes = kSpread, kTris = kSpreadTris;
  const uint32_t nl = min(a.big_count[5], a.big_capacity);
  const uint32_t turns = (nl + (uint32_t)kTris - 1u) / (uint32_t)kTris;
  for (uint32_t i = wave; i < turns; i += nwaves) {
    const int tri = lane / kLanes;
    const uint32_t e = i * (uint32_t)kTris + (uint32_t)tri;
    uint64_t fs = a.F;
    if (tri < kTris && e < nl) fs = a.med_queue[a.big_capacity - 1u - e];
    int32_t s0 = 0, s1 = 0, s2 = 0;
    if (fs < a.F) { s0 = a.faces[3 * fs + 0]; s1 = a.faces[3 * fs + 1]; s2 = a.faces[3 * fs + 2]; }
    raster_frag_64<TEX ? 6 : 2, false, true>(a, fs, s0, s1, s2, i & (kQSub - 1), lane % kLanes, true);
  }
}
template <bool TEX>
__global__ __launch_bounds__(256) void k_raster_medium(RasterArgs a) {
  raster_medium_wave<TEX>(a, (blockIdx.x * blockDim.x + threadIdx.x) >> 6, (gridDim.x * blockDim.x) >> 6);
}

template <bool LOOP, int MODE>
// ... 51 lines not shown
__global__ __launch_bounds__(256) __attribute__((amdgpu_waves_per_eu((MODE & 3) ? 4 : 5, 5))) void k_raster_frag_group(RasterGroup g) {
  uint32_t v, tb;
  if (g.chunk) {
    const uint32_t k = blockIdx.x >> 3, sq = k / g.n;
    v = k - sq * g.n;
    tb = xcd_block(blockIdx.x & 7u, sq, g.chunk);
    if (tb >= g.blocks_per_view) return;
  } else {
    v = blockIdx.x / g.blocks_per_view;
    tb = blockIdx.x - v * g.blocks_per_view;
  }
  raster_frag_wave<true, MODE>(g.view[v], ((uint64_t)tb * blockDim.x + threadIdx.x) >> 6);
}
template <int MODE>
__global__ __launch_bounds__(256) __attribute__((amdgpu_waves_per_eu(5, 5))) void k_raster_frag_group_ml(RasterGroup g) {
  static_assert((MODE & 3) == 0, "one triangle per lane only");
  __shared__ double s_u[kMeshletMaxVerts], s_v[kMeshletMaxVerts], s_iz[kMeshletMaxVerts];
  uint32_t v, tb;
  if (g.chunk) {
    const uint32_t k = blockIdx.x >> 3, sq = k / g.n;
    v = k - sq * g.n;
    tb = xcd_block(blockIdx.x & 7u, sq, g.chunk);
    if (tb >= g.blocks_per_view) return;
  } else {
    v = blockIdx.x / g.blocks_per_view;
    tb = blockIdx.x - v * g.blocks_per_view;
  }
  const RasterArgs& a = g.view[v];
  const uint32_t id0 = g.ml_first[tb];
  const uint32_t nv = min(g.ml_first[tb + 1] - id0, kMeshletMaxVerts);
  const uint32_t* __restrict__ ids = g.ml_ids + id0;
  const float* __restrict__ pos = g.ml_pos + 3u * (uint64_t)id0;
  for (uint32_t i = threadIdx.x; i < nv; i += 256u) {
    const ScreenVertex s = project_point(a.cam, pos[3u * i + 0u], pos[3u * i + 1u], pos[3u * i + 2u]);
    s_u[i] = s.u; s_v[i] = s.v; s_iz[i] = s.iz;
  }
  __syncthreads();
  const uint64_t f = (uint64_t)tb * 256u + threadIdx.x;
  MeshletTri m;
  m.ids = ids;
  m.l0 = 0u; m.l1 = 0u; m.l2 = 0u;
  if (f < a.F) {
    const uint32_t w = g.ml_tris[f];
    constexpr uint32_t kMask = (1u << kMeshletIndexBits) - 1u;
    m.l0 = min(w & kMask, kMeshletMaxVerts - 1u); m.l1 = min((w >> kMeshletIndexBits) & kMask, kMeshletMaxVerts - 1u);
    m.l2 = min((w >> (2u * kMeshletIndexBits)) & kMask, kMeshletMaxVerts - 1u);
  }
  m.va.u = s_u[m.l0]; m.va.v = s_v[m.l0]; m.va.iz = s_iz[m.l0];
  m.vb.u = s_u[m.l1]; m.vb.v = s_v[m.l1]; m.vb.iz = s_iz[m.l1];
  m.vc.u = s_u[m.l2]; m.vc.v = s_v[m.l2]; m.vc.iz = s_iz[m.l2];
  const uint64_t wave_id = ((uint64_t)tb * 256u + threadIdx.x) >> 6;
  raster_frag_64<MODE, true>(a, f < a.F ? f : a.F, 0, 0, 0, (uint32_t)wave_id & (kQSub - 1), -1, false, &m);
}
struct CountGroup {
  uint32_t* big_count[kMaxGroup];
  uint32_t n;
};
__global__ void k_reset_big_counts(CountGroup g) {
  const uint32_t v = threadIdx.x / 6u, k = threadIdx.x - v * 6u;
  if (v < g.n) g.big_count[v][k] = 0u;
}
template <bool TEX>
__global__ __launch_bounds__(256) void k_raster_medium_group(RasterGroup g, uint32_t blocks_per_view) {
  const uint32_t v = blockIdx.x / blocks_per_view;
  raster_medium_wave<TEX>(g.view[v], ((blockIdx.x - v * blocks_per_view) * blockDim.x + threadIdx.x) >> 6, (blocks_per_view * blockDim.x) >> 6);
}
__device__ __forceinline__ void raster_huge_block(const RasterArgs& a, const uint32_t tile) {
  __shared__ uint32_t s_hits[256];
  __shared__ uint32_t s_nhits;
  const uint32_t nbig = min(a.big_count[2], a.big_capacity);
  if (nbig == 0u) return;
  const FragQueues& q = a.q;
  const int t = threadIdx.x;
  const uint32_t tx = tile / q.tiles_y, ty = tile - tx * q.tiles_y;
  const uint32_t x0 = tx * kQW, y0 = ty * kQH;
  const int tx1 = (int)min(x0 + kQW, a.W) - 1, ty1 = (int)min(y0 + kQH, a.H) - 1;
  bool any = false;
  if (t == 0) s_nhits = 0u;
  __syncthreads();
  for (uint32_t qb = 0; qb < nbig; qb += 256u) {
    const uint32_t qi = qb + (uint32_t)t;
    if (qi < nbig) {
      const uint32_t f = a.huge_queue[qi];
      const TriFrag rec = a.frags[f];
      const int bx1 = (int)(rec.mask & 0xFFFFu), by1 = (int)((rec.mask >> 16) & 0xFFFFu);
      if (rec.kind == 2 && (int)rec.x0 <= tx1 && bx1 >= (int)x0 && (int)rec.y0 <= ty1 && by1 >= (int)y0)
        s_hits[atomicAdd(&s_nhits, 1u)] = f;
    }
    __syncthreads();
    const uint32_t nh = s_nhits;
    for (uint32_t h = 0; h < nh; h++) {
      const uint64_t f = s_hits[h];
      for (int p = 0; p < 2; p++) {
        Piece pc;
        if (!load_piece(a, f, p, pc)) continue;
        const Tri& tr = pc.t;
        const int xa = max(tr.x0, (int)x0), xb = min(tr.x1, tx1), ya = max(tr.y0, (int)y0), yb = min(tr.y1, ty1);
        const int hh = yb - ya + 1, area = (xb - xa + 1) * hh;
        if (hh <= 0) continue;
        for (int i = t; i < area; i += 256) {
          const int x = xa + i / hh, y = ya + i % hh;
          const unsigned long long key = shade_piece_key(a, f, pc, x, y);
          if (key != kNullKey) { atomicMin(&a.keys[key_index((uint32_t)x, (uint32_t)y, a.H)], key); any = true; }
        }
      }
    }
    __syncthreads();
    if (t == 0) s_nhits = 0u;
    __syncthreads();
  }
  if (any) atomicOr(&q.flag[tile], 2u);
}

__global__ __launch_bounds__(256) void k_raster_huge(RasterArgs a, uint32_t ntiles) {
  if (min(a.big_count[2], a.big_capacity) == 0u) return;
  for (uint32_t tile = blockIdx.x; tile < ntiles; tile += gridDim.x) { raster_huge_block(a, tile); __syncthreads(); }
}

template <typename PlanesWanted>
__device__ __forceinline__ void tile_resolve_block(const RasterArgs& a, uint32_t* __restrict__ idx_out, float* __restrict__ depth_out,
                                                   const uint32_t tile, PlanesWanted planes_wanted) {
  __shared__ unsigned long long skeys[kQPixels];
  __shared__ uint32_t scount[kQSub];
  const FragQueues& q = a.q;
  const int t = threadIdx.x;
  const uint32_t W = a.W, H = a.H;
  const uint32_t tx = tile / q.tiles_y, ty = tile - tx * q.tiles_y;
  const uint32_t x0 = tx * kQW, y0 = ty * kQH;
  constexpr uint32_t kGroup = 256u / kQSub, kSpec = 6;
  const uint32_t sq = (uint32_t)t / kGroup, sq_lane = (uint32_t)t % kGroup;
  const uint64_t qbase = ((uint64_t)tile * kQSub + sq) * q.cap;
  unsigned long long spec_key[kSpec];
  uint16_t spec_pix[kSpec];
#pragma unroll
  for (uint32_t k = 0; k < kSpec; k++) {
    const uint32_t i = min(sq_lane + k * kGroup, q.cap - 1u);
    spec_key[k] = q.key[qbase + i];
    spec_pix[k] = q.pix[qbase + i];
  }
  const uint32_t n = min(q.count[tile * kQSub + sq], q.cap);
  if (sq_lane == 0u) scount[sq] = n;
  const uint32_t tile_flag = q.flag[tile];
  const bool merge = tile_flag != 0u;
  for (int p = t; p < kQPixels; p += 256) {
    const uint32_t gx = x0 + (uint32_t)(p >> 6), gy = y0 + (uint32_t)(p & 63);
    unsigned long long k = kBackgroundKey;
    if (merge && gx < W && gy < H) {
      const uint64_t g = key_index(gx, gy, H);
      k = a.keys[g];
      a.keys[g] = kBackgroundKey;
    }
    skeys[p] = k;
  }
  __syncthreads();
#pragma unroll
  for (uint32_t k = 0; k < kSpec; k++)
    if (sq_lane + k * kGroup < n) atomicMin(&skeys[spec_pix[k]], spec_key[k]);
  constexpr uint32_t kHead = kSpec * kGroup;
  uint32_t rest[kQSub], total = 0u;
#pragma unroll
  for (int s = 0; s < kQSub; s++) { rest[s] = scount[s] > kHead ? scount[s] - kHead : 0u; total += rest[s]; }
  auto entry_of = [&](uint32_t j) -> uint64_t {
    uint32_t sub = 0u;
#pragma unroll
    for (int s = 0; s < kQSub - 1; s++) if (sub == (uint32_t)s && j >= rest[s]) { j -= rest[s]; sub = (uint32_t)s + 1u; }
    return ((uint64_t)tile * kQSub + sub) * q.cap + kHead + j;
  };
  for (uint32_t j0 = (uint32_t)t; j0 < total; j0 += 4u * 256u) {
    unsigned long long k4[4];
    uint16_t p4[4];
#pragma unroll
    for (uint32_t u = 0; u < 4u; u++) {
      const uint32_t j = j0 + u * 256u;
      const uint64_t e = j < total ? entry_of(j) : qbase;
      k4[u] = q.key[e];
      p4[u] = q.pix[e];
    }
#pragma unroll
    for (uint32_t u = 0; u < 4u; u++)
      if (j0 + u * 256u < total) atomicMin(&skeys[p4[u]], k4[u]);
  }
  __syncthreads();
  if (a.frags && !a.prim_id && !a.tex_res) {
    if (tile_flag & 1u) {
      if (t == 0) a.big_count[1] = 1u;
    } else {
      auto lost = [&](const unsigned long long key, const uint32_t pin) {
        if (key == kNullKey || skeys[pin] == key) return;
        const uint32_t f = (uint32_t)(key & 0xFFFFFFFFull);
        const TriFrag rec = a.frags[f];
        if (rec.kind != 1) return;
        const int bit = (int)(x0 + (pin >> 6) - rec.x0) * 8 + (int)(y0 + (pin & 63u) - rec.y0);
        atomicAnd(&a.frags[f].mask, ~(1ull << bit));
      };
#pragma unroll
      for (uint32_t k = 0; k < kSpec; k++)
        if (sq_lane + k * kGroup < n) lost(spec_key[k], spec_pix[k]);
      for (uint32_t j0 = (uint32_t)t; j0 < total; j0 += 4u * 256u) {
        unsigned long long k4[4];
        uint16_t p4[4];
#pragma unroll
        for (uint32_t u = 0; u < 4u; u++) {
          const uint32_t j = j0 + u * 256u;
          const uint64_t e = j < total ? entry_of(j) : qbase;
          k4[u] = q.key[e];
          p4[u] = q.pix[e];
        }
#pragma unroll
        for (uint32_t u = 0; u < 4u; u++)
          if (j0 + u * 256u < total) lost(k4[u], p4[u]);
      }
    }
  }
  if (planes_wanted())
  for (int p = t; p < kQPixels; p += 256) {
    const uint32_t gx = x0 + (uint32_t)(p >> 6), gy = y0 + (uint32_t)(p & 63);
    if (gx < W && gy < H) {
      const unsigned long long k = skeys[p];
      const uint64_t g = (uint64_t)gx * H + gy;
      idx_out[g] = (uint32_t)(k & 0xFFFFFFFFull);
      if (depth_out) depth_out[g] = __uint_as_float((uint32_t)(k >> 32));
    }
  }
  if (t < kQSub) q.count[tile * kQSub + t] = 0u;
  if (t == 0) q.flag[tile] = 0u;
}

__device__ __forceinline__ bool view_needs_planes(const RasterArgs& a) { return !a.idx_optional || a.big_count[0] != 0u || a.big_count[1] != 0u; }

__global__ __launch_bounds__(256) void k_tile_resolve(RasterArgs a, uint32_t* __restrict__ idx_out, float* __restrict__ depth_out) {
  tile_resolve_block(a, idx_out, depth_out, blockIdx.x, [&] { return view_needs_planes(a); });
}

__global__ __launch_bounds__(256) void k_raster_huge_group(RasterGroup g) {
  bool any = false;
  for (uint32_t v = 0; v < g.n; v++) any = any || min(g.view[v].big_count[2], g.view[v].big_capacity) != 0u;
  if (!any) return;
  for (uint32_t tile = blockIdx.x; tile < g.tile_end[g.n - 1]; tile += gridDim.x) {
    uint32_t v = 0;
    while (v + 1 < g.n && tile >= g.tile_end[v]) v++;
    raster_huge_block(g.view[v], tile - (v ? g.tile_end[v - 1] : 0u));
    __syncthreads();
  }
}

__global__ __launch_bounds__(256) void k_tile_resolve_group(RasterGroup g) {
  uint32_t v = 0;
  while (v + 1 < g.n && blockIdx.x >= g.tile_end[v]) v++;
  tile_resolve_block(g.view[v], g.idx[v], nullptr, blockIdx.x - (v ? g.tile_end[v - 1] : 0u), [&] {
    if (g.view[v].idx_optional == 2u) return view_needs_planes(g.view[v]);
    bool planes = false;
    for (uint32_t u = 0; u < g.n; u++) planes = planes || view_needs_planes(g.view[u]);
    return planes;
  });
}

__global__ __launch_bounds__(256) void k_tile_resolve_group_depth(RasterGroup g) {
  uint32_t v = 0;
  while (v + 1 < g.n && blockIdx.x >= g.tile_end[v]) v++;
  float* depth = reinterpret_cast<float*>(g.idx[v] + (uint64_t)g.view[v].W * g.view[v].H);
  tile_resolve_block(g.view[v], g.idx[v], depth, blockIdx.x - (v ? g.tile_end[v - 1] : 0u), [] { return true; });
}

__global__ void k_resolve(unsigned long long* __restrict__ keys, uint32_t* __restrict__ idx, float* __restrict__ depth,
                          uint32_t W, uint32_t H) {
  const uint64_t i = (uint64_t)blockIdx.x * blockDim.x + threadIdx.x;
  if (i >= (uint64_t)W * H) return;
  const uint32_t x = (uint32_t)(i / H), y = (uint32_t)(i - (uint64_t)x * H);
  const uint64_t g = key_index(x, y, H);
  const unsigned long long k = keys[g];
  keys[g] = kBackgroundKey;
  idx[i] = (uint32_t)(k & 0xFFFFFFFFull);
  if (depth) depth[i] = __uint_as_float((uint32_t)(k >> 32));
}

__global__ void k_fill_keys(unsigned long long* __restrict__ keys, uint64_t N) {
  const uint64_t i = (uint64_t)blockIdx.x * blockDim.x + threadIdx.x;
  if (i < N) keys[i] = kBackgroundKey;
}

__global__ void k_texel_area(const float* __restrict__ verts, const int32_t* __restrict__ faces, uint64_t F, uint64_t V,
                             const smesh_camera_t* __restrict__ cams, uint32_t K, float* __restrict__ best_area) {
  const uint64_t f = (uint64_t)blockIdx.x * blockDim.x + threadIdx.x;
  if (f >= F) return;
  const int32_t id[3] = {faces[3 * f], faces[3 * f + 1], faces[3 * f + 2]};
  float best = 0.0f;
  bool valid = true;
  for (int k = 0; k < 3; k++) if (id[k] < 0 || (uint64_t)id[k] >= V) valid = false;
  if (valid) {
    float P[3][3];
    for (int k = 0; k < 3; k++)
      for (int d = 0; d < 3; d++) P[k][d] = verts[3 * (uint64_t)id[k] + d];
    for (uint32_t ci = 0; ci < K; ci++) {
      const smesh_camera_t& cam = cams[ci];
      float pu[3], pv[3];
      bool in_front = false;
      for (int k = 0; k < 3; k++) {
        const float xc = ((cam.rotation[0] * P[k][0] + cam.rotation[1] * P[k][1]) + cam.rotation[2] * P[k][2]) + cam.translation[0];
        const float yc = ((cam.rotation[3] * P[k][0] + cam.rotation[4] * P[k][1]) + cam.rotation[5] * P[k][2]) + cam.translation[1];
        const float zc = ((cam.rotation[6] * P[k][0] + cam.rotation[7] * P[k][1]) + cam.rotation[8] * P[k][2]) + cam.translation[2];
        in_front |= zc > 0.0f;
        pu[k] = (float)(cam.focal[0] * ((double)xc / (double)zc) + cam.principal[0]);
        pv[k] = (float)(cam.focal[1] * ((double)yc / (double)zc) + cam.principal[1]);
      }
      const float border = 0.5f;
      const float rw = (float)(int)cam.width, rh = (float)(int)cam.height;
      bool inside = in_front;
      for (int k = 0; k < 3; k++)
        inside = inside && (-border * rw <= pu[k]) && (pu[k] < (1 + border) * rw) &&
                 (-border * rh <= pv[k]) && (pv[k] < (1 + border) * rh);
      if (inside) {
        const float area = 0.5f * fabsf((pu[0] * (pv[1] - pv[2]) + pu[1] * (pv[2] - pv[0])) + pu[2] * (pv[0] - pv[1]));
        if (area > best) best = area;
      }
    }
  }
  best_area[f] = best;
}

}

constexpr int kSlots = 2 * kMaxGroup;
constexpr int kHeld = 32;
constexpr int kSides = kSlots + kHeld;
constexpr int kRecordSides = 6;

struct ImagePair {
  uint32_t* idx;
  float* depth;
  uint64_t pixels;
  bool idx_out, depth_out;
};

struct smesh_renderer {
  DeviceCtx* ctx = nullptr;
  uint64_t V = 0, F = 0, num_primitives = 0;
  float* verts = nullptr;
  int32_t* faces = nullptr;
  struct Bounds { bool valid = false; double lo[3] = {0, 0, 0}, hi[3] = {0, 0, 0}, max_edge = 0, mean_edge = 0; } bounds;
  uint32_t* prim_id = nullptr;
  struct Meshlets { uint32_t* first = nullptr; uint32_t* ids = nullptr; uint32_t* tris = nullptr; float* pos = nullptr; } ml;
  struct ViewScratch {
    ScreenVertex* sv = nullptr;
    uint32_t* huge_queue = nullptr;
    uint32_t* med_queue = nullptr;
    unsigned long long* keys = nullptr;
    uint64_t keys_pixels = 0;
    FragQueues fq;
    uint64_t fq_tiles = 0;
  } vs[kSlots];
  bool texels = false;
  uint32_t* tex_res = nullptr;
  uint32_t* tex_first = nullptr;
  std::vector<int32_t> h_faces;
  std::vector<uint32_t> h_res, h_first;
  struct Side {
    uint32_t* big_queue = nullptr;
    uint32_t* big_count = nullptr;
    TriFrag* frags = nullptr;
    uint8_t* kinds = nullptr;
  } side[kSides];
  uint32_t big_capacity = 0;
  std::vector<ImagePair> images;
  Scratch own_idx;
  Scratch fused[kSides];
  struct HeldJob {
    int n = 0, nparts = 0, next_part = 0;
    bool ranged = false;
    smesh_aggregator* agg = nullptr;
    const float* probs[kHeld] = {};
    const float* weights[kHeld] = {};
    uint64_t W[kHeld] = {}, H[kHeld] = {};
  } held;
  hipEvent_t ev_bank_rendered[2] = {nullptr, nullptr}, ev_bank_consumed[2] = {nullptr, nullptr}, ev_main_fence = nullptr;
  hipEvent_t ev_raster_done = nullptr;
  uint64_t group_seq = 0;
  bool bank_used[2] = {false, false};
  uint64_t fused_seq = 0;
  const uint32_t* last_idx[kRecordSides] = {};
  uint64_t last_W[kRecordSides] = {}, last_H[kRecordSides] = {};
  uint64_t render_seq = 0;
  bool rec_valid[kRecordSides] = {};
  bool hash_valid[kRecordSides] = {};
  unsigned long long* d_hash = nullptr;
  hipEvent_t hash_ev[kRecordSides] = {};
  Scratch match_stage;
  DepthScratch gate;
  float* normals = nullptr;
  int last_render_side = 0;
  bool raster_pending = false;
  bool main_pending = false;
  std::mutex mu;
};

namespace {
__device__ __forceinline__ unsigned long long mix64(unsigned long long z) {
  z = (z ^ (z >> 30)) * 0xBF58476D1CE4E5B9ull;
  z = (z ^ (z >> 27)) * 0x94D049BB133111EBull;
  return z ^ (z >> 31);
}
__global__ __launch_bounds__(256) void k_plane_checksum(const uint32_t* __restrict__ img, uint64_t N, unsigned long long* __restrict__ out) {
  __shared__ unsigned long long part[4];
  unsigned long long h = 0ull;
  for (uint64_t i = (uint64_t)blockIdx.x * blockDim.x + threadIdx.x; i < N; i += (uint64_t)gridDim.x * blockDim.x)
    h += mix64((i << 32) | (unsigned long long)img[i]);
  for (int off = 32; off > 0; off >>= 1) h += __shfl_down(h, off);
  if ((threadIdx.x & 63) == 0) part[threadIdx.x >> 6] = h;
  __syncthreads();
  if (threadIdx.x == 0) atomicAdd(out, ((part[0] + part[1]) + part[2]) + part[3]);
}
int plane_checksum(DeviceCtx* ctx, hipStream_t st, const uint32_t* d_img, uint64_t N, unsigned long long* d_out) {
  SMESH_HIP(hipMemsetAsync(d_out, 0, sizeof(unsigned long long), st));
  const uint32_t blocks = (uint32_t)std::max<uint64_t>(1, std::min<uint64_t>(div_up(N, 256 * 16), (uint64_t)ctx->num_cus));
  hipLaunchKernelGGL(k_plane_checksum, dim3(blocks), dim3(256), 0, st, d_img, N, d_out);
  SMESH_HIP(hipGetLastError());
  return SMESH_OK;
}
}

namespace {
bool no_huge_possible(const smesh_renderer* r, const smesh_camera_t* cam);
bool no_big_possible(const smesh_renderer* r, const smesh_camera_t* cam);
void mesh_bounds(const float* v, uint64_t V, const int32_t* f, uint64_t F, smesh_renderer::Bounds& b);

int ensure_keys(smesh_renderer::ViewScratch& vs, uint64_t W, uint64_t H, hipStream_t st) {
  const uint64_t N = div_up(W, 4) * div_up(H, 4) * 16;
  if (N <= vs.keys_pixels) return SMESH_OK;
  if (vs.keys) SMESH_HIP(dev_free(vs.keys));
  vs.keys = nullptr;
  vs.keys_pixels = 0;
  SMESH_HIP(dev_malloc(reinterpret_cast<void**>(&vs.keys), N * 8));
  vs.keys_pixels = N;
  hipLaunchKernelGGL(k_fill_keys, dim3((uint32_t)div_up(N, 256)), dim3(256), 0, st, vs.keys, N);
  SMESH_HIP(hipGetLastError());
  return SMESH_OK;
}

int main_after_raster(smesh_renderer* r) {
  if (!r->raster_pending) return SMESH_OK;
  if (!r->ev_raster_done) SMESH_HIP(hipEventCreateWithFlags(&r->ev_raster_done, hipEventDisableTiming));
  SMESH_HIP(hipEventRecord(r->ev_raster_done, r->ctx->raster_stream));
  SMESH_HIP(hipStreamWaitEvent(r->ctx->stream, r->ev_raster_done, 0));
  r->raster_pending = false;
  return SMESH_OK;
}

enum class RasterPath { Frag, Direct };

RasterPath raster_path() {
  static const RasterPath p = [] {
    const char* e = getenv("SMESH_RASTER");
    const std::string v = e ? e : "";
    if (v == "direct") return RasterPath::Direct;
    return RasterPath::Frag;
  }();
  return p;
}

bool plane_optional_allowed(const smesh_renderer* r) {
  return !r->texels && !r->prim_id && raster_path() == RasterPath::Frag;
}

int plane_optional_level(smesh_renderer* r, smesh_aggregator* a) {
  if (r->texels || !smesh_aggregator_can_fuse_triangles(a, r->F)) return 0;
  return smesh_aggregator_fuses_small_views_by_mask(a) ? 2 : 1;
}

constexpr uint32_t kRasterXcdRun = 8;

uint64_t frag_cap_forced() {
  const char* e = getenv("SMESH_FRAG_CAP");
  return e ? std::max<uint64_t>(1, (uint64_t)atoll(e)) : 0u;
}

bool ensure_queues(smesh_renderer* r, smesh_renderer::ViewScratch& vs, uint64_t W, uint64_t H, hipStream_t st, int* status) {
  *status = SMESH_OK;
  const uint64_t tiles_x = div_up(W, kQW), tiles_y = div_up(H, kQH), ntiles = tiles_x * tiles_y;
  uint64_t cap = frag_cap_forced();
  if (!cap) {
    cap = 16ull * kQPixels / kQSub;
    const uint64_t budget = 8ull << 30;
    if (ntiles * kQSub * cap * 10 > budget) cap = budget / (ntiles * kQSub * 10);
    if (cap < 256) return false;
  }
  if (ntiles > vs.fq_tiles || (uint32_t)cap != vs.fq.cap) {
    (void)hipStreamSynchronize(r->ctx->stream);
    (void)hipStreamSynchronize(r->ctx->raster_stream);
    for (void* p : {(void*)vs.fq.key, (void*)vs.fq.pix, (void*)vs.fq.count, (void*)vs.fq.flag})
      if (p) (void)dev_free(p);
    vs.fq = FragQueues();
    vs.fq_tiles = 0;
    hipError_t e = dev_malloc(reinterpret_cast<void**>(&vs.fq.key), ntiles * kQSub * cap * 8);
    if (e == hipSuccess) e = dev_malloc(reinterpret_cast<void**>(&vs.fq.pix), ntiles * kQSub * cap * 2);
    if (e == hipSuccess) e = dev_malloc(reinterpret_cast<void**>(&vs.fq.count), ntiles * kQSub * 4);
    if (e == hipSuccess) e = dev_malloc(reinterpret_cast<void**>(&vs.fq.flag), ntiles * 4);
    if (e == hipSuccess) e = hipMemsetAsync(vs.fq.count, 0, ntiles * kQSub * 4, st);
    if (e == hipSuccess) e = hipMemsetAsync(vs.fq.flag, 0, ntiles * 4, st);
    if (e != hipSuccess) { *status = fail_hip(e, "fragment queue allocation", __FILE__, __LINE__); return false; }
    vs.fq.cap = (uint32_t)cap;
    vs.fq_tiles = ntiles;
  }
  vs.fq.tiles_y = (uint32_t)tiles_y;
  return true;
}

CameraArgs camera_args(const smesh_camera_t* cam) {
  CameraArgs ca;
  memcpy(ca.R, cam->rotation, sizeof ca.R);
  memcpy(ca.t, cam->translation, sizeof ca.t);
  ca.fx = cam->focal[0]; ca.fy = cam->focal[1]; ca.cx = cam->principal[0]; ca.cy = cam->principal[1];
  ca.W = (uint32_t)cam->width; ca.H = (uint32_t)cam->height;
  return ca;
}

double typical_edge_pixels(const smesh_renderer* r, const smesh_camera_t* cam) {
  const smesh_renderer::Bounds& b = r->bounds;
  if (!b.valid || !(b.mean_edge > 0.0)) return 0.0;
  double z = cam->translation[2];
  for (int d = 0; d < 3; d++) z += (double)cam->rotation[6 + d] * 0.5 * (b.lo[d] + b.hi[d]);
  if (!(z > 1e-3)) return 0.0;
  const double e = b.mean_edge * std::max(std::fabs(cam->focal[0]), std::fabs(cam->focal[1])) / z;
  return std::isfinite(e) ? e : 0.0;
}
double depth_spread(const smesh_renderer* r, const smesh_camera_t* cam) {
  const smesh_renderer::Bounds& b = r->bounds;
  if (!b.valid) return 1.0;
  double zmin = INFINITY, zmax = -INFINITY;
  for (int c = 0; c < 8; c++) {
    double z = cam->translation[2];
    for (int d = 0; d < 3; d++) z += (double)cam->rotation[6 + d] * ((c >> d) & 1 ? b.hi[d] : b.lo[d]);
    zmin = std::min(zmin, z); zmax = std::max(zmax, z);
  }
  if (!(zmax > 0.0)) return 1.0;
  return zmin > 1e-3 * zmax ? zmax / zmin : INFINITY;
}
bool want_spread(const smesh_renderer* r, const smesh_camera_t* cam, int nviews) {
  static const int knob = env_int("SMESH_RASTER_SPREAD", -1);
  if (knob == 0 || !cam) return false;
  if (knob == 1) return true;
  if (nviews > 1) return false;
  if (depth_spread(r, cam) > 6.0) return false;
  const double e = typical_edge_pixels(r, cam);
  return e >= 10.5 && e <= 19.0;
}

RasterArgs raster_args(smesh_renderer* r, smesh_renderer::ViewScratch& vs, int side, uint64_t W, uint64_t H, int nviews = 1,
                       const smesh_camera_t* cam = nullptr) {
  RasterArgs a;
  a.faces = r->faces; a.verts = r->verts; a.sv = vs.sv; a.tex_res = r->texels ? r->tex_res : nullptr; a.tex_first = r->tex_first;
  a.prim_id = r->prim_id;
  a.keys = vs.keys; a.F = r->F; a.V = r->V; a.W = (uint32_t)W; a.H = (uint32_t)H;
  a.big_queue = r->side[side].big_queue; a.big_count = r->side[side].big_count; a.big_capacity = r->big_capacity;
  a.huge_queue = vs.huge_queue;
  a.med_queue = vs.med_queue;
  {
    static const int knob = env_int("SMESH_RASTER_BALANCE", -1);
    a.balance = (vs.med_queue && (knob >= 0 ? knob != 0 : (cam && depth_spread(r, cam) > 6.0))) ? (nviews > 1 ? 1u : 2u) : 0u;
  }
  a.frags = r->side[side].frags;
  a.kinds = r->side[side].kinds;
  a.q = FragQueues();
  a.idx_optional = 0u;
  a.tpw = 64;
  const bool fine = r->F >= 32768u;
  const uint64_t min_waves = fine ? 1024u : 2048u;
  const uint64_t launch_views = fine ? (uint64_t)std::max(1, nviews) : 1u;
  while (a.tpw > 1 && launch_views * r->F / a.tpw < min_waves) a.tpw >>= 1;
  a.groups = 1;
  a.spread = 0u;
  {
    static const int knob = env_int("SMESH_RASTER_WG_PUSH", -1);
    a.wg_push = knob >= 0 ? (uint32_t)(knob != 0) : (cam && typical_edge_pixels(r, cam) >= 5.0 ? 1u : 0u);
  }
  if (want_spread(r, cam, nviews)) { a.spread = (uint32_t)kSpread; a.tpw = (uint32_t)kSpreadTris; }
  return a;
}

uint32_t frag_groups(uint64_t F, int views, uint32_t tpw) {
  static const int knob = env_int("SMESH_RASTER_GROUPS", 0);
  if (tpw != 64u) return 1u;
  if (knob >= 1) return (uint32_t)knob;
  return (F >= 4000000u && (uint64_t)views * div_up(F, 256u) >= 20480u) ? 4u : 1u;
}

int render_into(smesh_renderer* r, const smesh_camera_t* cam, uint32_t* d_idx, float* d_depth, hipStream_t st = nullptr,
                int side = 0, int idx_optional = 0) {
  DeviceCtx* ctx = r->ctx;
  r->last_render_side = side;
  if (!st) {
    st = ctx->stream;
    SMESH_TRY(main_after_raster(r));
    r->main_pending = true;
  }
  const uint64_t W = cam->width, H = cam->height, N = W * H;
  smesh_renderer::ViewScratch& vs = r->vs[0];
  SMESH_TRY(ensure_keys(vs, W, H, st));
  ProfScope prof(ctx, SMESH_PROF_RASTER, st);
  const CameraArgs ca = camera_args(cam);
  RasterArgs a = raster_args(r, vs, side, W, H, 1, cam);
  a.cam = ca;
  if (r->V) {
    hipLaunchKernelGGL(k_project_vertices, dim3((uint32_t)div_up(r->V, 256)), dim3(256), 0, st, r->verts, r->V, ca, vs.sv,
                       r->side[side].big_count);
    SMESH_HIP(hipGetLastError());
  } else {
    SMESH_HIP(hipMemsetAsync(r->side[side].big_count, 0, 32, st));
  }
  if (r->F) {
    a.idx_optional = (idx_optional && plane_optional_allowed(r)) ? (uint32_t)idx_optional : 0u;
    const uint32_t big_grid = (uint32_t)std::min<uint64_t>(r->F, (uint64_t)ctx->num_cus);
    int qs = SMESH_OK;
    if (raster_path() == RasterPath::Frag && ensure_queues(r, vs, W, H, st, &qs)) {
      a.q = vs.fq;
      {
        const uint32_t nblocks = (uint32_t)div_up(div_up(r->F, a.tpw), 4);
        const uint32_t chunk = nblocks >= 64u ? kRasterXcdRun : 0u;
        const dim3 grid(chunk ? 8u * xcd_slots(nblocks, chunk) : nblocks);
        switch (raster_mode(a)) {
          case 7:  hipLaunchKernelGGL(k_raster_frag<7>, grid, dim3(256), 0, st, a, nblocks, chunk); break;
          case 5:  hipLaunchKernelGGL(k_raster_frag<5>, grid, dim3(256), 0, st, a, nblocks, chunk); break;
          case 4:  hipLaunchKernelGGL(k_raster_frag<4>, grid, dim3(256), 0, st, a, nblocks, chunk); break;
          case 3:  hipLaunchKernelGGL(k_raster_frag<3>, grid, dim3(256), 0, st, a, nblocks, chunk); break;
          case 1:  hipLaunchKernelGGL(k_raster_frag<1>, grid, dim3(256), 0, st, a, nblocks, chunk); break;
          default: hipLaunchKernelGGL(k_raster_frag<0>, grid, dim3(256), 0, st, a, nblocks, chunk); break;
        }
        if ((raster_mode(a) & 3) != 0 && a.balance) {
          const dim3 mgrid(4u * (uint32_t)std::max(1, ctx->num_cus));
          if (a.tex_res) hipLaunchKernelGGL(k_raster_medium<true>, mgrid, dim3(256), 0, st, a);
          else hipLaunchKernelGGL(k_raster_medium<false>, mgrid, dim3(256), 0, st, a);
        }
      }
      SMESH_HIP(hipGetLastError());
      const uint32_t ntiles = (uint32_t)(div_up(W, kQW) * div_up(H, kQH));
      if (!no_huge_possible(r, cam)) hipLaunchKernelGGL(k_raster_huge, dim3(std::min<uint32_t>(ntiles, 2u * (uint32_t)ctx->num_cus)), dim3(256), 0, st, a, ntiles);
      SMESH_HIP(hipGetLastError());
      hipLaunchKernelGGL(k_tile_resolve, dim3((uint32_t)(div_up(W, kQW) * div_up(H, kQH))), dim3(256), 0, st, a, d_idx, d_depth);
      SMESH_HIP(hipGetLastError());
      return SMESH_OK;
    }
    SMESH_TRY(qs);
    hipLaunchKernelGGL(k_raster_small, dim3((uint32_t)div_up(r->F, 256)), dim3(256), 0, st, a);
    SMESH_HIP(hipGetLastError());
    hipLaunchKernelGGL(k_raster_big, dim3(big_grid), dim3(256), 0, st, a, 0u);
    SMESH_HIP(hipGetLastError());
  }
  hipLaunchKernelGGL(k_resolve, dim3((uint32_t)div_up(N, 256)), dim3(256), 0, st, vs.keys, d_idx, d_depth, (uint32_t)W, (uint32_t)H);
  SMESH_HIP(hipGetLastError());
  SMESH_HIP(hipMemsetAsync(r->side[side].big_count + 1, 0xFF, 4, st));
  return SMESH_OK;
}

hipError_t alloc_side(smesh_renderer* r, int i);
thread_local const char* g_last_raster_path = "none";

PipelineNeighbour raster_pipeline_neighbour(const smesh_renderer* r) {
  static std::once_flag once;
  static uint32_t ml_vgprs = 96u, ml_lds = 0u, plain_vgprs = 96u, plain_lds = 0u;
  std::call_once(once, [] {
    hipFuncAttributes fa;
    if (hipFuncGetAttributes(&fa, reinterpret_cast<const void*>(&k_raster_frag_group_ml<0>)) == hipSuccess) { ml_vgprs = (uint32_t)std::max(1, fa.numRegs); ml_lds = (uint32_t)fa.sharedSizeBytes; }
    if (hipFuncGetAttributes(&fa, reinterpret_cast<const void*>(&k_raster_frag_group<0>)) == hipSuccess) { plain_vgprs = (uint32_t)std::max(1, fa.numRegs); plain_lds = (uint32_t)fa.sharedSizeBytes; }
    (void)hipGetLastError();
  });
  PipelineNeighbour nb;
  const bool meshlets = r->ml.tris != nullptr && opt_raster_meshlets();
  nb.wg_vgprs = meshlets ? ml_vgprs : plain_vgprs;
  nb.wg_lds = meshlets ? ml_lds : plain_lds;
  return nb;
}

hipError_t alloc_scratch(smesh_renderer* r, int i, bool need_sv) {
  smesh_renderer::ViewScratch& vs = r->vs[i];
  hipError_t e = hipSuccess;
  if (!vs.sv && need_sv) e = dev_malloc(reinterpret_cast<void**>(&vs.sv), std::max<uint64_t>(r->V * sizeof(ScreenVertex), 16));
  if (e == hipSuccess && !vs.huge_queue) e = dev_malloc(reinterpret_cast<void**>(&vs.huge_queue), (size_t)r->big_capacity * 4);
  if (e == hipSuccess && !vs.med_queue) e = dev_malloc(reinterpret_cast<void**>(&vs.med_queue), (size_t)r->big_capacity * 4);
  return e;
}

bool queues_fit_group(uint64_t W, uint64_t H) {
  if (raster_path() != RasterPath::Frag) return false;
  if (frag_cap_forced()) return true;
  const uint64_t ntiles = div_up(W, kQW) * div_up(H, kQH);
  const uint64_t cap = 16ull * kQPixels / kQSub;
  return ntiles * kQSub * cap * 10 <= (2ull << 30);
}

int prepare_group_slots(smesh_renderer* r, const smesh_camera_t* cams, int n, hipStream_t st, int base) {
  for (int v = 0; v < n; v++) {
    const uint64_t W = cams[v].width, H = cams[v].height, N = W * H;
    SMESH_HIP(alloc_side(r, base + v));
    SMESH_HIP(alloc_scratch(r, base + v, !(r->ml.tris && opt_raster_meshlets())));
    smesh_renderer::ViewScratch& vs = r->vs[base + v];
    SMESH_TRY(ensure_keys(vs, W, H, st));
    int qs = SMESH_OK;
    if (!ensure_queues(r, vs, W, H, st, &qs)) return qs != SMESH_OK ? qs : fail(SMESH_ERR_RUNTIME, "fragment queues unavailable");
    if (r->fused[base + v].bytes < N * 8) {
      SMESH_HIP(hipStreamSynchronize(st));
      SMESH_HIP(hipStreamSynchronize(r->ctx->stream));
      SMESH_TRY(r->fused[base + v].reserve(N * 8));
    }
  }
  return SMESH_OK;
}

int render_group_into(smesh_renderer* r, const smesh_camera_t* cams, int n, hipStream_t st, int base = 0, int side_base = -1,
                      int idx_optional = 0, bool with_depth = false) {
  if (side_base < 0) side_base = base;
  if (!plane_optional_allowed(r) || with_depth) idx_optional = 0;
  DeviceCtx* ctx = r->ctx;
  ProjectGroup pg;
  RasterGroup rg;
  memset(&pg, 0, sizeof pg);
  memset(&rg, 0, sizeof rg);
  uint32_t tiles = 0;
  for (int v = 0; v < n; v++) {
    const uint64_t W = cams[v].width, H = cams[v].height, N = W * H;
    SMESH_HIP(alloc_side(r, side_base + v));
    SMESH_HIP(alloc_scratch(r, base + v,  false));
    smesh_renderer::ViewScratch& vs = r->vs[base + v];
    SMESH_TRY(ensure_keys(vs, W, H, st));
    int qs = SMESH_OK;
    if (!ensure_queues(r, vs, W, H, st, &qs)) return qs != SMESH_OK ? qs : fail(SMESH_ERR_RUNTIME, "fragment queues unavailable");
    if (r->fused[side_base + v].bytes < N * 8) {
      SMESH_HIP(hipStreamSynchronize(st));
      SMESH_HIP(hipStreamSynchronize(r->ctx->stream));
      SMESH_TRY(r->fused[side_base + v].reserve(N * 8));
    }
    if (side_base + v < kRecordSides) { r->last_idx[side_base + v] = nullptr; r->rec_valid[side_base + v] = false; }
    pg.cam[v] = camera_args(&cams[v]);
    pg.sv[v] = vs.sv;
    pg.big_count[v] = r->side[side_base + v].big_count;
    rg.view[v] = raster_args(r, vs, side_base + v, W, H, n);
    { const RasterArgs own = raster_args(r, vs, side_base + v, W, H, 1, &cams[v]); rg.view[v].wg_push = own.wg_push; rg.view[v].balance = own.balance; }
    rg.view[v].cam = pg.cam[v];
    rg.view[v].q = vs.fq;
    rg.view[v].idx_optional = (uint32_t)idx_optional;
    rg.idx[v] = static_cast<uint32_t*>(r->fused[side_base + v].ptr);
    tiles += (uint32_t)(div_up(W, kQW) * div_up(H, kQH));
    rg.tile_end[v] = tiles;
  }
  pg.verts = r->verts; pg.V = r->V;
  pg.n = (uint32_t)n;
  rg.n = (uint32_t)n;
  {
    int votes = 0;
    for (int v = 0; v < n; v++) votes += want_spread(r, &cams[v], n) ? 1 : 0;
    if (2 * votes >= n && votes > 0)
      for (int v = 0; v < n; v++) { rg.view[v].spread = (uint32_t)kSpread; rg.view[v].tpw = (uint32_t)kSpreadTris; }
    int push_votes = 0;
    for (int v = 0; v < n; v++) push_votes += rg.view[v].wg_push ? 1 : 0;
    for (int v = 0; v < n; v++) rg.view[v].wg_push = 2 * push_votes >= n && push_votes > 0 ? 1u : 0u;
    int balance_votes = 0;
    for (int v = 0; v < n; v++) balance_votes += rg.view[v].balance ? 1 : 0;
    for (int v = 0; v < n; v++) rg.view[v].balance = 2 * balance_votes >= n && balance_votes > 0 ? (n > 1 ? 1u : 2u) : 0u;
  }
  for (int v = 0; v < n; v++) rg.view[v].groups = frag_groups(r->F, n, rg.view[0].tpw);
  const int mode = raster_mode(rg.view[0]);
  const bool meshlets = (mode & 3) == 0 && r->ml.tris != nullptr && opt_raster_meshlets();
  if (meshlets) {
    for (int v = 0; v < n; v++) { rg.view[v].tpw = 64u; rg.view[v].groups = 1u; rg.view[v].sv = nullptr; }
    rg.ml_first = r->ml.first; rg.ml_ids = r->ml.ids; rg.ml_tris = r->ml.tris; rg.ml_pos = r->ml.pos;
  } else {
    for (int v = 0; v < n; v++) {
      SMESH_HIP(alloc_scratch(r, base + v, true));
      pg.sv[v] = r->vs[base + v].sv;
      rg.view[v].sv = r->vs[base + v].sv;
    }
  }
  g_last_raster_path = meshlets ? "meshlets" : "vertex-stage";
  rg.blocks_per_view = (uint32_t)div_up(div_up(r->F, rg.view[0].tpw * rg.view[0].groups), 4);
  ProfScope prof(ctx, SMESH_PROF_RASTER, st);
  if (meshlets) {
    CountGroup cg;
    memset(&cg, 0, sizeof cg);
    for (int v = 0; v < n; v++) cg.big_count[v] = pg.big_count[v];
    cg.n = (uint32_t)n;
    hipLaunchKernelGGL(k_reset_big_counts, dim3(1), dim3(64), 0, st, cg);
  } else {
    hipLaunchKernelGGL(k_project_vertices_group, dim3((uint32_t)div_up(r->V, 256)), dim3(256), 0, st, pg);
  }
  SMESH_HIP(hipGetLastError());
  {
    rg.chunk = rg.blocks_per_view >= 64u ? kRasterXcdRun : 0u;
    const dim3 grid(rg.chunk ? 8u * xcd_slots(rg.blocks_per_view, rg.chunk) * (uint32_t)n : (uint32_t)n * rg.blocks_per_view);
    if (meshlets) {
      if (mode & 4) hipLaunchKernelGGL(k_raster_frag_group_ml<4>, grid, dim3(256), 0, st, rg);
      else hipLaunchKernelGGL(k_raster_frag_group_ml<0>, grid, dim3(256), 0, st, rg);
    } else
    switch (mode) {
      case 7:  hipLaunchKernelGGL(k_raster_frag_group<7>, grid, dim3(256), 0, st, rg); break;
      case 5:  hipLaunchKernelGGL(k_raster_frag_group<5>, grid, dim3(256), 0, st, rg); break;
      case 4:  hipLaunchKernelGGL(k_raster_frag_group<4>, grid, dim3(256), 0, st, rg); break;
      case 3:  hipLaunchKernelGGL(k_raster_frag_group<3>, grid, dim3(256), 0, st, rg); break;
      case 1:  hipLaunchKernelGGL(k_raster_frag_group<1>, grid, dim3(256), 0, st, rg); break;
      default: hipLaunchKernelGGL(k_raster_frag_group<0>, grid, dim3(256), 0, st, rg); break;
    }
    if ((raster_mode(rg.view[0]) & 3) != 0 && rg.view[0].balance) {
      const uint32_t per_view = std::max(64u, 4u * (uint32_t)std::max(1, ctx->num_cus) / (uint32_t)n);
      if (rg.view[0].tex_res) hipLaunchKernelGGL(k_raster_medium_group<true>, dim3((uint32_t)n * per_view), dim3(256), 0, st, rg, per_view);
      else hipLaunchKernelGGL(k_raster_medium_group<false>, dim3((uint32_t)n * per_view), dim3(256), 0, st, rg, per_view);
    }
  }
  SMESH_HIP(hipGetLastError());
  bool huge_needed = false;
  for (int v = 0; v < n; v++) huge_needed = huge_needed || !no_huge_possible(r, &cams[v]);
  if (huge_needed) hipLaunchKernelGGL(k_raster_huge_group, dim3(std::min<uint32_t>(tiles, 4u * (uint32_t)ctx->num_cus)), dim3(256), 0, st, rg);
  SMESH_HIP(hipGetLastError());
  if (with_depth) hipLaunchKernelGGL(k_tile_resolve_group_depth, dim3(tiles), dim3(256), 0, st, rg);
  else hipLaunchKernelGGL(k_tile_resolve_group, dim3(tiles), dim3(256), 0, st, rg);
  SMESH_HIP(hipGetLastError());
  return SMESH_OK;
}

int acquire_image(smesh_renderer* r, uint64_t N, ImagePair** out) {
  for (auto& im : r->images)
    if (!im.idx_out && !im.depth_out && im.pixels == N) { *out = &im; return SMESH_OK; }
  for (size_t i = 0; i < r->images.size();) {
    ImagePair& im = r->images[i];
    if (!im.idx_out && !im.depth_out) {
      SMESH_HIP(hipStreamSynchronize(r->ctx->stream));
      (void)dev_free(im.idx);
      (void)dev_free(im.depth);
      r->images.erase(r->images.begin() + i);
    } else {
      i++;
    }
  }
  ImagePair im{nullptr, nullptr, N, false, false};
  SMESH_HIP(dev_malloc(reinterpret_cast<void**>(&im.idx), N * 4));
  hipError_t e = dev_malloc(reinterpret_cast<void**>(&im.depth), N * 4);
  if (e != hipSuccess) { (void)dev_free(im.idx); return fail_hip(e, "hipMalloc depth plane", __FILE__, __LINE__); }
  r->images.push_back(im);
  *out = &r->images.back();
  return SMESH_OK;
}

int check_camera(const smesh_camera_t* cam) {
  if (!cam) return fail(SMESH_ERR_INVALID, "camera is NULL");
  if (cam->width == 0 || cam->height == 0 || cam->width > 65536 || cam->height > 65536)
    return fail(SMESH_ERR_INVALID, "camera resolution must be in [1, 65536]");
  if (cam->width * cam->height >= 0x7FFFFFFFull / 4) return fail(SMESH_ERR_INVALID, "image too large");
  return SMESH_OK;
}

hipError_t alloc_side(smesh_renderer* r, int i) {
  smesh_renderer::Side& sd = r->side[i];
  if (sd.frags) return hipSuccess;
  hipError_t e = dev_malloc(reinterpret_cast<void**>(&sd.big_queue), (size_t)r->big_capacity * 8);
  if (e == hipSuccess) e = dev_malloc(reinterpret_cast<void**>(&sd.big_count), 32);
  if (e == hipSuccess) e = dev_malloc(reinterpret_cast<void**>(&sd.frags), std::max<uint64_t>(r->F * sizeof(TriFrag), 16));
  if (e == hipSuccess && r->texels) e = dev_malloc(reinterpret_cast<void**>(&sd.kinds), std::max<uint64_t>(r->F, 16));
  if (e == hipSuccess) e = hipMemsetAsync(sd.big_count, 0, 32, r->ctx->stream);
  if (e == hipSuccess) e = hipStreamSynchronize(r->ctx->stream);
  return e;
}

void mesh_bounds(const float* v, uint64_t V, const int32_t* f, uint64_t F, smesh_renderer::Bounds& b) {
  b.valid = false;
  if (!V || !F) return;
  float lo[3] = {INFINITY, INFINITY, INFINITY}, hi[3] = {-INFINITY, -INFINITY, -INFINITY};
  bool finite = true;
  for (uint64_t i = 0; i < V; i++)
    for (int d = 0; d < 3; d++) {
      const float x = v[3 * i + d];
      finite = finite && std::isfinite(x);
      lo[d] = std::min(lo[d], x); hi[d] = std::max(hi[d], x);
    }
  if (!finite) return;
  double m2 = 0.0, sum_edges = 0.0;
  uint64_t edges = 0;
  for (uint64_t i = 0; i < F; i++) {
    const int32_t a = f[3 * i], c = f[3 * i + 1], e = f[3 * i + 2];
    if (a < 0 || c < 0 || e < 0 || (uint64_t)a >= V || (uint64_t)c >= V || (uint64_t)e >= V) continue;
    const float* p[3] = {v + 3 * (uint64_t)a, v + 3 * (uint64_t)c, v + 3 * (uint64_t)e};
    for (int k = 0; k < 3; k++) {
      const float* q = p[k]; const float* w = p[(k + 1) % 3];
      const double dx = (double)q[0] - w[0], dy = (double)q[1] - w[1], dz = (double)q[2] - w[2];
      m2 = std::max(m2, dx * dx + dy * dy + dz * dz);
      sum_edges += std::sqrt(dx * dx + dy * dy + dz * dz);
      edges++;
    }
  }
  b.mean_edge = edges ? sum_edges / (double)edges : 0.0;
  for (int d = 0; d < 3; d++) { b.lo[d] = lo[d]; b.hi[d] = hi[d]; }
  b.max_edge = std::sqrt(m2);
  b.valid = std::isfinite(b.max_edge);
}

double box_extent_bound(const smesh_renderer::Bounds& b, const smesh_camera_t* cam) {
  if (!b.valid) return INFINITY;
  const double W = (double)cam->width, H = (double)cam->height;
  double zmin = INFINITY, mag = 0.0, frob2 = 0.0;
  for (int row = 0; row < 3; row++) {
    double m = std::fabs((double)cam->translation[row]);
    for (int d = 0; d < 3; d++) {
      const double R = cam->rotation[3 * row + d];
      m += std::fabs(R) * std::max(std::fabs(b.lo[d]), std::fabs(b.hi[d]));
      frob2 += R * R;
    }
    mag = std::max(mag, m);
  }
  for (int c = 0; c < 8; c++) {
    double z = cam->translation[2];
    for (int d = 0; d < 3; d++) z += (double)cam->rotation[6 + d] * ((c >> d) & 1 ? b.hi[d] : b.lo[d]);
    zmin = std::min(zmin, z);
  }
  const double eps = 32.0 * 5.9604644775390625e-08 * mag;
  const double z_lo = zmin - eps;
  const double L = std::sqrt(frob2) * b.max_edge + 4.0 * eps;
  if (!(z_lo > 1e-3) || !std::isfinite(mag) || !std::isfinite(L)) return INFINITY;
  const double ratio = L / z_lo;
  if (!(ratio < 0.25)) return INFINITY;
  const double fx = std::fabs(cam->focal[0]), fy = std::fabs(cam->focal[1]);
  const double ax = std::max(std::fabs(cam->principal[0]), std::fabs(W - cam->principal[0])) + 1.0;
  const double ay = std::max(std::fabs(cam->principal[1]), std::fabs(H - cam->principal[1])) + 1.0;
  const double du = (fx + ax) * ratio / (1.0 - ratio), dv = (fy + ay) * ratio / (1.0 - ratio);
  if (!std::isfinite(du) || !std::isfinite(dv)) return INFINITY;
  return std::max(du, dv);
}
bool no_huge_possible(const smesh_renderer* r, const smesh_camera_t* cam) { return box_extent_bound(r->bounds, cam) <= (double)kMedium - 4.0; }
bool no_big_possible(const smesh_renderer* r, const smesh_camera_t* cam) { return box_extent_bound(r->bounds, cam) <= 6.5; }

int create_common(const float* vertices, uint64_t V, const int32_t* faces, uint64_t F, int device,
                  smesh_renderer** out) {
  if (!out) return fail(SMESH_ERR_INVALID, "out is NULL");
  *out = nullptr;
  if ((V && !vertices) || (F && !faces)) return fail(SMESH_ERR_INVALID, "NULL mesh arrays");
  if (F >= 0xFFFFFFFFull || V >= 0x7FFFFFFFull) return fail(SMESH_ERR_INVALID, "mesh too large for 32-bit indices");
  DeviceCtx* ctx;
  SMESH_TRY(get_ctx(device, &ctx));
  SMESH_HIP(hipSetDevice(device));
  auto* r = new (std::nothrow) smesh_renderer();
  if (!r) return fail(SMESH_ERR_RUNTIME, "out of memory");
// ... 40 lines not shown
  const bool force = env && atoi(env) == 1;
  if (F < 4096 && !force) return false;
  std::vector<float> cx(F), cy(F), cz(F);
  double lo[3] = {1e300, 1e300, 1e300}, hi[3] = {-1e300, -1e300, -1e300}, edge_sum = 0.0;
  uint64_t edges = 0;
  for (uint64_t i = 0; i < F; i++) {
    const int32_t a = f[3 * i], b = f[3 * i + 1], c = f[3 * i + 2];
    if (a < 0 || b < 0 || c < 0 || (uint64_t)a >= V || (uint64_t)b >= V || (uint64_t)c >= V) { cx[i] = cy[i] = cz[i] = 0.f; continue; }
    const float* pa = v + 3 * (uint64_t)a; const float* pb = v + 3 * (uint64_t)b; const float* pc = v + 3 * (uint64_t)c;
    cx[i] = (pa[0] + pb[0] + pc[0]) / 3.f; cy[i] = (pa[1] + pb[1] + pc[1]) / 3.f; cz[i] = (pa[2] + pb[2] + pc[2]) / 3.f;
    if (!std::isfinite(cx[i]) || !std::isfinite(cy[i]) || !std::isfinite(cz[i])) { cx[i] = cy[i] = cz[i] = 0.f; continue; }
    const double c3[3] = {cx[i], cy[i], cz[i]};
    for (int d = 0; d < 3; d++) { lo[d] = std::min(lo[d], c3[d]); hi[d] = std::max(hi[d], c3[d]); }
    if ((i & 15) == 0) { edge_sum += std::sqrt((double)(pa[0] - pb[0]) * (pa[0] - pb[0]) + (double)(pa[1] - pb[1]) * (pa[1] - pb[1]) + (double)(pa[2] - pb[2]) * (pa[2] - pb[2])); edges++; }
  }
  if (!(lo[0] <= hi[0]) || !edges) return false;
  auto spread = [&](const uint32_t* ord) {
    double total = 0.0;
    for (uint64_t g = 0; g < F; g += 64) {
      float l0 = 1e30f, l1 = 1e30f, l2 = 1e30f, h0 = -1e30f, h1 = -1e30f, h2 = -1e30f;
      const uint64_t e = std::min<uint64_t>(F, g + 64);
      for (uint64_t i = g; i < e; i++) {
        const uint64_t j = ord ? ord[i] : i;
        l0 = std::min(l0, cx[j]); h0 = std::max(h0, cx[j]); l1 = std::min(l1, cy[j]); h1 = std::max(h1, cy[j]);
        l2 = std::min(l2, cz[j]); h2 = std::max(h2, cz[j]);
      }
      total += (double)(h0 - l0) + (double)(h1 - l1) + (double)(h2 - l2);
    }
    return total;
  };
  const double before = spread(nullptr);
  const double neighbours = (double)((F + 63) / 64) * 16.0 * (edge_sum / (double)edges);
  if (!force && before <= 6.0 * neighbours) return false;
  std::vector<std::pair<uint64_t, uint32_t>> keyed(F);
  auto spread_bits = [](uint64_t x) {
    x &= 0x1FFFFFull;
    x = (x | x << 32) & 0x1F00000000FFFFull; x = (x | x << 16) & 0x1F0000FF0000FFull; x = (x | x << 8) & 0x100F00F00F00F00Full;
    x = (x | x << 4) & 0x10C30C30C30C30C3ull; x = (x | x << 2) & 0x1249249249249249ull;
    return x;
  };
  const double sx = hi[0] > lo[0] ? 2097151.0 / (hi[0] - lo[0]) : 0.0, sy = hi[1] > lo[1] ? 2097151.0 / (hi[1] - lo[1]) : 0.0,
               sz = hi[2] > lo[2] ? 2097151.0 / (hi[2] - lo[2]) : 0.0;
  for (uint64_t i = 0; i < F; i++) {
    const uint64_t qx = (uint64_t)std::min(2097151.0, std::max(0.0, (cx[i] - lo[0]) * sx)), qy = (uint64_t)std::min(2097151.0, std::max(0.0, (cy[i] - lo[1]) * sy)),
                   qz = (uint64_t)std::min(2097151.0, std::max(0.0, (cz[i] - lo[2]) * sz));
    keyed[i] = {spread_bits(qx) | (spread_bits(qy) << 1) | (spread_bits(qz) << 2), (uint32_t)i};
  }
  std::sort(keyed.begin(), keyed.end());
  order.resize(F);
  for (uint64_t i = 0; i < F; i++) order[i] = keyed[i].second;
  if (!force && spread(order.data()) * 2.0 > before) { order.clear(); return false; }
  return true;
}

static thread_local const char* g_last_fuse_kernel = "none";
static thread_local const char* g_last_add_path = "none";
static thread_local int g_last_fuse_probs_dtype = 0;
void smesh_note_fuse(const char* kernel, const char* path) { g_last_fuse_kernel = kernel; g_last_add_path = path; g_last_fuse_probs_dtype = 0; }
int smesh_last_fuse_probs_dtype() { return g_last_fuse_probs_dtype; }
static void note_fuse_half(int probs_dtype) { smesh_note_fuse("k_fuse_tri_h16", "render-records"); g_last_fuse_probs_dtype = probs_dtype; }
static void note_fuse_sampled(int probs_dtype) { smesh_note_fuse("k_fuse_tri_sampled", "render-records"); g_last_fuse_probs_dtype = probs_dtype; }

static bool labels_native(smesh_renderer* r, smesh_aggregator* a, uint64_t N) {
  return !r->texels && !r->prim_id && smesh_labels_native(a, r->F, N);
}

constexpr int kLabelsPlaneLevel = 1;

static bool half_native(smesh_renderer* r, smesh_aggregator* a) { return !r->texels && !r->prim_id && smesh_half_native(a, r->F); }
static bool sampled_native(smesh_renderer* r, smesh_aggregator* a) { return !r->texels && !r->prim_id && smesh_sampled_native(a, r->F); }
static bool scans_all_planes(smesh_renderer* r, smesh_aggregator* a, ViewInput::Kind kind, uint64_t N) {
  switch (kind) {
    case ViewInput::SAMPLED: return sampled_native(r, a);
    case ViewInput::HALF: return half_native(r, a);
    case ViewInput::LABELS: return labels_native(r, a, N);
    default: return false;
  }
}

static RenderedView rendered_view(const smesh_renderer::Side& sd, const uint32_t* d_idx, const ViewInput& in, const float* d_w, uint64_t W, uint64_t H,
                                  bool mid_queue) {
  RenderedView rv{sd.frags, sd.big_queue, sd.big_count, d_idx, in.probs(), d_w, W, H, in.ps0, in.ps1, mid_queue};
  if (in.kind != ViewInput::F32) rv.image = in.image;
  return rv;
}

static int fuse_rendered(smesh_renderer* r, smesh_aggregator* a, int slot, const uint32_t* d_idx, const ViewInput& in, const float* weights,
                         int memkind, uint64_t W, uint64_t H) {
  DeviceCtx* ctx = r->ctx;
  const uint64_t N = W * H;
  const float* probs = in.probs();
  const float* d_probs = probs;
  const float* d_w = weights;
  int64_t ps0 = in.ps0, ps1 = in.ps1;
  const smesh_renderer::Side& sd = r->side[slot];
  switch (in.kind) {
    case ViewInput::SAMPLED: {
      if (!sampled_native(r, a)) return fail(SMESH_ERR_INVALID, "sampled view: k_fuse_tri_sampled does not serve this renderer and aggregator");
      const RenderedView rv = rendered_view(sd, d_idx, in, d_w, W, H, false);
      SMESH_TRY(smesh_sampled_fuse_triangles(a, r->F, r->big_capacity, &rv, 1, in.src));
      note_fuse_sampled(in.src.dtype);
      return SMESH_OK;
    }
    case ViewInput::HALF: {
      const int dt16 = in.dtype_or_bytes;
      if (half_native(r, a)) {
        const RenderedView rv = rendered_view(sd, d_idx, in, d_w, W, H, true);
        SMESH_TRY(smesh_half_fuse_triangles(a, r->F, r->big_capacity, &rv, 1, dt16));
        note_fuse_half(dt16);
        return SMESH_OK;
      }
      const int64_t C = (int64_t)smesh_aggregator_classes(a);
      const int64_t s[3] = {(ps0 || ps1) ? ps0 : (int64_t)H * C, (ps0 || ps1) ? ps1 : C, 1};
      SMESH_TRY(smesh_half_widen(a, in.image, dt16, s, W, H, &d_probs));
      ps0 = ps1 = 0;
      break;
    }
    case ViewInput::LABELS: {
      if (labels_native(r, a, N)) {
        const RenderedView rv = rendered_view(sd, d_idx, in, d_w, W, H, true);
        SMESH_TRY(smesh_labels_fuse_triangles(a, r->F, r->big_capacity, &rv, 1, in.dtype_or_bytes));
        smesh_note_fuse("k_fuse_tri_labels", "render-records");
        return SMESH_OK;
      }
      SMESH_TRY(smesh_labels_expand(a, in.image, in.dtype_or_bytes, N, &d_probs));
      break;
    }
    case ViewInput::F32: break;
  }
  if (memkind == SMESH_MEM_HOST) {
    const uint32_t C = smesh_aggregator_classes(a);
    Scratch& sp = smesh_aggregator_stage_probs(a);
    SMESH_TRY(sp.reserve(N * C * 4));
    SMESH_HIP(hipMemcpyAsync(sp.ptr, probs, N * C * 4, hipMemcpyHostToDevice, ctx->stream));
    d_probs = static_cast<const float*>(sp.ptr);
    if (weights) {
      Scratch& sw = smesh_aggregator_stage_w(a);
      SMESH_TRY(sw.reserve(N * 4));
      SMESH_HIP(hipMemcpyAsync(sw.ptr, weights, N * 4, hipMemcpyHostToDevice, ctx->stream));
      d_w = static_cast<const float*>(sw.ptr);
    }
    SMESH_HIP(hipStreamSynchronize(ctx->stream));
  }
  if (!r->texels && smesh_aggregator_can_fuse_triangles(a, r->F)) {
    const RenderedView rv{r->side[slot].frags, r->side[slot].big_queue, r->side[slot].big_count, d_idx, d_probs, d_w, W, H, ps0, ps1, true};
    SMESH_TRY(smesh_aggregator_fuse_triangles(a, r->F, r->prim_id, r->big_capacity, &rv, 1));
    smesh_note_fuse(smesh_aggregator_fuse_kernel_name(a, r->prim_id != nullptr), "render-records");
  } else if (r->texels && smesh_aggregator_can_fuse_texels(a, r->num_primitives)) {
    SMESH_TRY(smesh_aggregator_fuse_texels(a, r->side[slot].frags, r->side[slot].kinds, r->F, r->tex_first, r->tex_res, r->side[slot].big_queue,
                                           r->side[slot].big_count, r->big_capacity, d_idx, d_probs, d_w, H));
    smesh_note_fuse("k_fuse_texel", "render-records");
  } else {
    SMESH_TRY(smesh_aggregator_add_device_contig(a, d_idx, d_probs, d_w, W, H));
  }
  return SMESH_OK;
}

extern "C" {

const char* smesh_last_fuse_kernel(void) { return g_last_fuse_kernel; }
const char* smesh_last_add_path(void) { return g_last_add_path; }
const char* smesh_last_raster_path(void) { return g_last_raster_path; }

int smesh_renderer_create_triangles(const float* vertices, uint64_t V, const int32_t* faces, uint64_t F, int device,
                                    smesh_renderer_t** out) {
  DeviceCtx* ctx;
  SMESH_TRY(get_ctx(device, &ctx));
  std::lock_guard<std::recursive_mutex> lock(ctx->mu);
  if ((V && !vertices) || (F && !faces)) return fail(SMESH_ERR_INVALID, "NULL mesh arrays");
  std::vector<uint32_t> order;
  if (!spatial_order(vertices, V, faces, F, order)) return create_common(vertices, V, faces, F, device, out);
  std::vector<int32_t> hf(3 * F);
  for (uint64_t i = 0; i < F; i++)
    for (int k = 0; k < 3; k++) hf[3 * i + k] = faces[3 * (uint64_t)order[i] + k];
  smesh_renderer* r = nullptr;
  SMESH_TRY(create_common(vertices, V, hf.data(), F, device, &r));
  hipError_t e = dev_malloc(reinterpret_cast<void**>(&r->prim_id), F * 4);
  if (e == hipSuccess) e = hipMemcpyAsync(r->prim_id, order.data(), F * 4, hipMemcpyHostToDevice, ctx->stream);
  if (e == hipSuccess) e = hipStreamSynchronize(ctx->stream);
  if (e != hipSuccess) { smesh_renderer_destroy(r); return fail_hip(e, "primitive id table upload", __FILE__, __LINE__); }
  *out = r;
  return SMESH_OK;
}

int smesh_renderer_create_texels(const float* vertices, uint64_t V, const int32_t* faces, uint64_t F,
                                 const smesh_camera_t* cameras, uint64_t K, float tpp, int device,
                                 smesh_renderer_t** out) {
  if (K && !cameras) return fail(SMESH_ERR_INVALID, "NULL cameras");
  if (K > 0xFFFFFFFFull) return fail(SMESH_ERR_INVALID, "too many cameras");
  DeviceCtx* ctx;
  SMESH_TRY(get_ctx(device, &ctx));
  std::lock_guard<std::recursive_mutex> lock(ctx->mu);

  std::vector<int32_t> hf(faces, faces + 3 * F);
  for (uint64_t f = 0; f < F; f++) {
    int32_t* face = &hf[3 * f];
    bool valid = true;
    for (int k = 0; k < 3; k++) if (face[k] < 0 || (uint64_t)face[k] >= V) valid = false;
    if (!valid) continue;
    float diffs[3];
    for (int k = 0; k < 3; k++) {
      const float* p0 = vertices + 3 * (size_t)face[k];
      const float* p1 = vertices + 3 * (size_t)face[(k + 1) % 3];
      const float* p2 = vertices + 3 * (size_t)face[(k + 2) % 3];
      const float ax = p1[0] - p0[0], ay = p1[1] - p0[1], az = p1[2] - p0[2];
      const float bx = p2[0] - p0[0], by = p2[1] - p0[1], bz = p2[2] - p0[2];
      const float dot = ax * bx + ay * by + az * bz;
      const float la = std::sqrt(ax * ax + ay * ay + az * az), lb = std::sqrt(bx * bx + by * by + bz * bz);
      float cosv = dot / (la * lb);
      cosv = cosv > 1.0f ? 1.0f : (cosv < -1.0f ? -1.0f : cosv);
      diffs[k] = std::fabs(std::acos(cosv) - 1.57079632679489661923f);
    }
    int best = 0;
    for (int k = 1; k < 3; k++) if (diffs[k] < diffs[best]) best = k;
    if (best != 0) { std::swap(face[0], face[best]); std::swap(diffs[0], diffs[best]); }
    if (diffs[1] >= diffs[2]) std::swap(face[1], face[2]);
  }

  smesh_renderer* r = nullptr;
  SMESH_TRY(create_common(vertices, V, hf.data(), F, device, &r));
  r->texels = true;
  if (!r->side[0].kinds && dev_malloc(reinterpret_cast<void**>(&r->side[0].kinds), std::max<uint64_t>(F, 16)) != hipSuccess) {
    smesh_renderer_destroy(r);
    return fail(SMESH_ERR_RUNTIME, "texel renderer: allocation of the kind bytes failed");
  }
  r->h_faces = std::move(hf);
  r->h_res.assign(F, 0);
  r->h_first.assign(F, 0);

  std::vector<float> best(F, 0.0f);
  if (F && K) {
    smesh_camera_t* d_cams = nullptr;
    float* d_best = nullptr;
    int32_t* d_faces = nullptr;
    hipError_t e = dev_malloc(reinterpret_cast<void**>(&d_cams), K * sizeof(smesh_camera_t));
    if (e == hipSuccess) e = dev_malloc(reinterpret_cast<void**>(&d_best), F * 4);
    if (e == hipSuccess) e = dev_malloc(reinterpret_cast<void**>(&d_faces), F * 12);
    if (e == hipSuccess) e = hipMemcpyAsync(d_cams, cameras, K * sizeof(smesh_camera_t), hipMemcpyHostToDevice, ctx->stream);
    if (e == hipSuccess) e = hipMemcpyAsync(d_faces, faces, F * 12, hipMemcpyHostToDevice, ctx->stream);
    if (e == hipSuccess) {
      hipLaunchKernelGGL(k_texel_area, dim3((uint32_t)div_up(F, 128)), dim3(128), 0, ctx->stream, r->verts, d_faces, F, V,
                         d_cams, (uint32_t)K, d_best);
      e = hipGetLastError();
    }
    if (e == hipSuccess) e = hipMemcpyAsync(best.data(), d_best, F * 4, hipMemcpyDeviceToHost, ctx->stream);
// ... 77 lines not shown
  *P = r->num_primitives;
  *first = r->tex_first;
  *res = r->tex_res;
  return SMESH_OK;
}

extern "C" {

int smesh_renderer_render_device(smesh_renderer_t* r, const smesh_camera_t* cam, uint32_t** indices_dev, float** depth_dev) {
  if (!r || !indices_dev || !depth_dev) return fail(SMESH_ERR_INVALID, "NULL argument");
  SMESH_TRY(check_camera(cam));
  std::lock_guard<std::mutex> g(r->mu);
  std::lock_guard<std::recursive_mutex> lock(r->ctx->mu);
  SMESH_HIP(hipSetDevice(r->ctx->device));
  ImagePair* im;
  SMESH_TRY(acquire_image(r, cam->width * cam->height, &im));
  const int side = (int)(r->render_seq++ % (uint64_t)kRecordSides);
  if (side != 0) SMESH_HIP(alloc_side(r, side));
  r->last_idx[side] = nullptr; r->rec_valid[side] = false;
  SMESH_TRY(render_into(r, cam, im->idx, im->depth, nullptr, side));
  for (int sd = 0; sd < kRecordSides; sd++)
    if (r->last_idx[sd] == im->idx) r->last_idx[sd] = nullptr;
  r->last_idx[side] = im->idx; r->last_W[side] = cam->width; r->last_H[side] = cam->height;
  r->rec_valid[side] = true;
  r->hash_valid[side] = false;
  im->idx_out = im->depth_out = true;
  *indices_dev = im->idx;
  *depth_dev = im->depth;
  return SMESH_OK;
}

int smesh_renderer_release_image(smesh_renderer_t* r, void* indices_dev, void* depth_dev) {
  if (!r) return fail(SMESH_ERR_INVALID, "NULL renderer");
  std::lock_guard<std::mutex> g(r->mu);
  for (auto& im : r->images) {
    if (indices_dev && im.idx == indices_dev) im.idx_out = false;
    if (depth_dev && im.depth == depth_dev) im.depth_out = false;
  }
  return SMESH_OK;
}

int smesh_renderer_render(smesh_renderer_t* r, const smesh_camera_t* cam, uint32_t* indices_out, float* depth_out) {
  if (!r || !indices_out) return fail(SMESH_ERR_INVALID, "NULL argument");
  SMESH_TRY(check_camera(cam));
  std::lock_guard<std::mutex> g(r->mu);
  DeviceCtx* ctx = r->ctx;
  std::lock_guard<std::recursive_mutex> lock(ctx->mu);
  SMESH_HIP(hipSetDevice(ctx->device));
  const uint64_t N = cam->width * cam->height;
  SMESH_TRY(r->own_idx.reserve(N * 8));
  uint32_t* d_idx = static_cast<uint32_t*>(r->own_idx.ptr);
  float* d_depth = reinterpret_cast<float*>(d_idx + N);
  r->last_idx[0] = nullptr; r->rec_valid[0] = false;
  SMESH_TRY(render_into(r, cam, d_idx, d_depth));
  SMESH_HIP(hipMemcpyAsync(indices_out, d_idx, N * 4, hipMemcpyDeviceToHost, ctx->stream));
  if (depth_out) SMESH_HIP(hipMemcpyAsync(depth_out, d_depth, N * 4, hipMemcpyDeviceToHost, ctx->stream));
  SMESH_HIP(hipStreamSynchronize(ctx->stream));
  return SMESH_OK;
}

static int fuse_view_impl(smesh_renderer_t* r, smesh_aggregator_t* a, const smesh_camera_t* cam, const ViewInput& in, const float* weights,
                          int memkind) {
  if (!r || !a || !in.image) return fail(SMESH_ERR_INVALID, "NULL argument");
  SMESH_TRY(check_camera(cam));
  DeviceCtx* ctx = r->ctx;
  if (smesh_aggregator_ctx(a) != ctx) return fail(SMESH_ERR_INVALID, "renderer and aggregator live on different devices");
  std::lock_guard<std::mutex> g(r->mu);
  std::lock_guard<std::mutex> g2(smesh_aggregator_mutex(a));
  std::lock_guard<std::recursive_mutex> lock(ctx->mu);
  SMESH_HIP(hipSetDevice(ctx->device));
  SMESH_TRY(smesh_aggregator_join_exchange(a));
  const uint64_t W = cam->width, H = cam->height, N = W * H;
  const int slot = 0;
  SMESH_TRY(main_after_raster(r));
  r->main_pending = true;
  if (r->fused[slot].bytes < N * 8) {
    SMESH_HIP(hipStreamSynchronize(ctx->raster_stream));
    SMESH_HIP(hipStreamSynchronize(ctx->stream));
    SMESH_TRY(r->fused[slot].reserve(N * 8));
  }
  uint32_t* d_idx = static_cast<uint32_t*>(r->fused[slot].ptr);
  r->last_idx[slot] = nullptr; r->rec_valid[slot] = false;
  const int tri_path = scans_all_planes(r, a, in.kind, N) ? kLabelsPlaneLevel : plane_optional_level(r, a);
  SMESH_TRY(render_into(r, cam, d_idx, nullptr, ctx->stream, slot, tri_path));
  SMESH_TRY(fuse_rendered(r, a, slot, d_idx, in, weights, memkind, W, H));
  r->fused_seq++;
  return SMESH_OK;
}

int smesh_fuse_view(smesh_renderer_t* r, smesh_aggregator_t* a, const smesh_camera_t* cam, const float* probs,
                    const float* weights, int memkind) {
  return fuse_view_impl(r, a, cam, ViewInput::f32(probs), weights, memkind);
}

static int fuse_views_impl(smesh_renderer_t* r, smesh_aggregator_t* a, const smesh_camera_t* cams, uint64_t n, const ViewInput& in,
                           const void* const* probs, const float* const* weights, int memkind) {
  const bool own_kernel = in.kind != ViewInput::F32;
  if (!r || !a || (n && (!cams || !probs))) return fail(SMESH_ERR_INVALID, "NULL argument");
  for (uint64_t i = 0; i < n; i++) {
    SMESH_TRY(check_camera(&cams[i]));
    if (!probs[i]) return fail(SMESH_ERR_INVALID, "NULL probs image");
  }
  DeviceCtx* ctx = r->ctx;
  if (smesh_aggregator_ctx(a) != ctx) return fail(SMESH_ERR_INVALID, "renderer and aggregator live on different devices");
  static const bool pairs_off = env_int("SMESH_FUSE_PAIRS", 1) == 0;
  bool pairable;
  int tri_path;
  {
    std::lock_guard<std::mutex> g2(smesh_aggregator_mutex(a));
    tri_path = plane_optional_level(r, a);
    pairable = !pairs_off && memkind == SMESH_MEM_DEVICE && !r->texels && r->F != 0 && smesh_aggregator_can_fuse_triangles(a, r->F) &&
               smesh_aggregator_can_fuse_pair(a);
    if (own_kernel) {
      tri_path = kLabelsPlaneLevel;
      pairable = !pairs_off && memkind == SMESH_MEM_DEVICE && r->F != 0;
    }
  }
  static const bool raster_pairs_off = env_int("SMESH_RASTER_PAIRS", 1) == 0;
  uint64_t i = 0;
  while (i < n) {
    int gn = (int)std::min<uint64_t>((uint64_t)kMaxGroup, n - i);
    bool grouped = !raster_pairs_off && memkind == SMESH_MEM_DEVICE && r->F != 0 && r->V != 0 && gn >= 2;
    for (int v = 0; v < gn && grouped; v++) grouped = queues_fit_group(cams[i + v].width, cams[i + v].height);
    if ((!pairable && !grouped) || i + 1 >= n) {
      SMESH_TRY(fuse_view_impl(r, a, &cams[i], in.at(probs[i]), weights ? weights[i] : nullptr, memkind));
      i += 1;
      continue;
    }
    std::lock_guard<std::mutex> g(r->mu);
    std::lock_guard<std::mutex> g2(smesh_aggregator_mutex(a));
    std::lock_guard<std::recursive_mutex> lock(ctx->mu);
    SMESH_HIP(hipSetDevice(ctx->device));
    SMESH_TRY(smesh_aggregator_join_exchange(a));
    const bool group_pipeline_on = opt_group_pipeline();
    const bool use_pipeline = grouped && group_pipeline_on;
    if (!use_pipeline) {
      SMESH_TRY(main_after_raster(r));
      r->main_pending = true;
    }
    const bool group_pipeline = group_pipeline_on;
    int base = 0;
    if (use_pipeline) {
      const int bank = (int)(r->group_seq++ & 1u);
      base = bank * kMaxGroup;
      for (int b = 0; b < 2; b++) {
        if (!r->ev_bank_rendered[b]) SMESH_HIP(hipEventCreateWithFlags(&r->ev_bank_rendered[b], hipEventDisableTiming));
        if (!r->ev_bank_consumed[b]) SMESH_HIP(hipEventCreateWithFlags(&r->ev_bank_consumed[b], hipEventDisableTiming));
      }
      if (r->bank_used[bank]) SMESH_HIP(hipStreamWaitEvent(ctx->raster_stream, r->ev_bank_consumed[bank], 0));
      if (r->main_pending || !r->bank_used[bank]) {
        if (!r->ev_main_fence) SMESH_HIP(hipEventCreateWithFlags(&r->ev_main_fence, hipEventDisableTiming));
        SMESH_HIP(hipEventRecord(r->ev_main_fence, ctx->stream));
        SMESH_HIP(hipStreamWaitEvent(ctx->raster_stream, r->ev_main_fence, 0));
        r->main_pending = false;
      }
      if (!r->bank_used[bank ^ 1]) SMESH_TRY(prepare_group_slots(r, &cams[i], gn, ctx->raster_stream, (bank ^ 1) * kMaxGroup));
      SMESH_TRY(render_group_into(r, &cams[i], gn, ctx->raster_stream, base, -1, tri_path));
      SMESH_HIP(hipEventRecord(r->ev_bank_rendered[bank], ctx->raster_stream));
      SMESH_HIP(hipStreamWaitEvent(ctx->stream, r->ev_bank_rendered[bank], 0));
      r->bank_used[bank] = true;
      r->raster_pending = true;
    } else if (grouped) {
      SMESH_TRY(render_group_into(r, &cams[i], gn, ctx->stream, 0, -1, tri_path));
    } else {
      gn = 2;
      SMESH_HIP(alloc_side(r, 1));
      for (int v = 0; v < 2; v++) {
        const uint64_t N = (uint64_t)cams[i + v].width * cams[i + v].height;
        if (r->fused[v].bytes < N * 8) {
          SMESH_HIP(hipStreamSynchronize(ctx->stream));
          SMESH_TRY(r->fused[v].reserve(N * 8));
        }
        r->last_idx[v] = nullptr; r->rec_valid[v] = false;
        SMESH_TRY(render_into(r, &cams[i + v], static_cast<uint32_t*>(r->fused[v].ptr), nullptr, ctx->stream, v));
      }
    }
    static const bool texel_multi_off = env_int("SMESH_TEXEL_MULTI", 1) == 0;
    bool texel_multi = false;
    if (grouped && !pairable && r->texels && !texel_multi_off) texel_multi = smesh_aggregator_can_fuse_texels(a, r->num_primitives);
    if (texel_multi) {
      ProfScope fuse_region(ctx, SMESH_PROF_FUSE_SCATTER);
      RenderedView rv[kMaxGroup];
      for (int j = 0; j < gn; j++) {
        const smesh_renderer::Side& sd = r->side[base + j];
        const uint64_t k = i + (uint64_t)j;
        rv[j] = rendered_view(sd, static_cast<const uint32_t*>(r->fused[base + j].ptr), in.at(probs[k]), weights ? weights[k] : nullptr, cams[k].width,
                              cams[k].height, false);
        rv[j].no_big = no_big_possible(r, &cams[k]);
        rv[j].kinds = sd.kinds;
      }
      SMESH_TRY(smesh_aggregator_fuse_texels_multi(a, r->F, r->tex_first, r->tex_res, r->big_capacity, rv, gn));
      smesh_note_fuse("k_fuse_texel", "render-records");
    }
    for (int j = 0; j < gn && !pairable && !texel_multi; j++) {
      const uint64_t k = i + (uint64_t)j;
      SMESH_TRY(fuse_rendered(r, a, base + j, static_cast<const uint32_t*>(r->fused[base + j].ptr), in.at(probs[k]), weights ? weights[k] : nullptr,
                              SMESH_MEM_DEVICE, cams[k].width, cams[k].height));
    }
    if (pairable) {
      ProfScope fuse_region(ctx, SMESH_PROF_FUSE_SCATTER);
      static const int label_views_cap = std::max(1, env_int("SMESH_FUSE_VIEWS", 8));
      const int max_nv = own_kernel ? std::min(8, label_views_cap) : smesh_aggregator_max_fused_views(a);
      for (int j = 0; j < gn;) {
        int nv = 1;
        while (nv * 2 <= std::min(max_nv, gn - j)) nv *= 2;
        RenderedView rv[kMaxGroup];
        for (int v = 0; v < nv; v++) {
          const smesh_renderer::Side& sd = r->side[base + j + v];
          const uint64_t k = i + (uint64_t)(j + v);
          rv[v] = rendered_view(sd, static_cast<const uint32_t*>(r->fused[base + j + v].ptr), in.at(probs[k]), weights ? weights[k] : nullptr,
                                cams[k].width, cams[k].height, true);
          rv[v].no_big = no_big_possible(r, &cams[k]);
          rv[v].beside = raster_pipeline_neighbour(r);
          rv[v].fine = box_extent_bound(r->bounds, &cams[k]) <= 48.0;
        }
        switch (in.kind) {
          case ViewInput::SAMPLED: SMESH_TRY(smesh_sampled_fuse_triangles(a, r->F, r->big_capacity, rv, nv, in.src)); break;
          case ViewInput::HALF: SMESH_TRY(smesh_half_fuse_triangles(a, r->F, r->big_capacity, rv, nv, in.dtype_or_bytes)); break;
          case ViewInput::LABELS: SMESH_TRY(smesh_labels_fuse_triangles(a, r->F, r->big_capacity, rv, nv, in.dtype_or_bytes)); break;
          case ViewInput::F32: SMESH_TRY(smesh_aggregator_fuse_triangles(a, r->F, r->prim_id, r->big_capacity, rv, nv)); break;
        }
        j += nv;
      }
    }
    if (pairable && in.kind == ViewInput::SAMPLED) note_fuse_sampled(in.src.dtype);
    else if (pairable && in.kind == ViewInput::HALF) note_fuse_half(in.dtype_or_bytes);
    else if (pairable) smesh_note_fuse(in.kind == ViewInput::LABELS ? "k_fuse_tri_labels" : smesh_aggregator_fuse_kernel_name(a, r->prim_id != nullptr), "render-records");
    if (grouped && group_pipeline) SMESH_HIP(hipEventRecord(r->ev_bank_consumed[base / kMaxGroup], ctx->stream));
    r->fused_seq += (uint64_t)gn;
    i += (uint64_t)gn;
  }
  return SMESH_OK;
}

int smesh_fuse_views(smesh_renderer_t* r, smesh_aggregator_t* a, const smesh_camera_t* cams, uint64_t n,
                     const float* const* probs, const float* const* weights, int memkind) {
  return fuse_views_impl(r, a, cams, n, ViewInput::f32(nullptr), reinterpret_cast<const void* const*>(probs), weights, memkind);
}

}

DeviceCtx* smesh_renderer_ctx(smesh_renderer* r) { return r->ctx; }

int smesh_renderer_fuse_views_labels(smesh_renderer* r, smesh_aggregator* a, const smesh_camera_t* cams, uint64_t n, const void* const* planes,
                                     const float* const* weights, const ViewInput& in) {
  bool native = true;
// ... 448 lines not shown
```

Measured before the change: 17890 views/s.

## Pack per-triangle raster records into 8-byte compact words with full-record fallback

Adds a compact 8-byte record format that packs x0, y0, a 2-bit kind and a 6x6 coverage mask into a single word. Records that are boxed, or small records wider than 6, spill to a full 16-byte array stored after the compact words. The rasterizer writes this format, and the triangle fuse kernel reads it when the aggregator fuses small views by mask and the index plane is optional. The goal is to halve record traffic between raster and fuse on the hot path, at the cost of extra bit unpacking, a second indirect load for large or wide triangles, and more code paths.

```diff
diff --git a/semantic_meshes_amd/csrc/common.hpp b/semantic_meshes_amd/csrc/common.hpp
--- a/semantic_meshes_amd/csrc/common.hpp
+++ b/semantic_meshes_amd/csrc/common.hpp
@@ -12,6 +12,7 @@
 #include <vector>
 
 #include "../../include/smesh.h"
+#include "records.hpp"
 
 namespace smesh {
 
@@ -82,6 +83,8 @@
 bool opt_group_pipeline();
 constexpr int kRasterMeshletsDefault = 1;
 bool opt_raster_meshlets();
+constexpr int kCompactRecordsDefault = 1;
+bool opt_compact_records();
 constexpr int kPipelineFitDefault = 1;
 constexpr int kPipelineFuseWaves = 5;
 int opt_pipeline_fit();
@@ -155,6 +158,7 @@
   uint32_t big_capacity;
   uint32_t tri_blocks;
   uint32_t big_blocks;
+  uint32_t compact = 0u;
   const uint32_t* prim_id;
   const uint32_t* tex_first;
   const uint32_t* tex_res;
@@ -199,6 +203,7 @@
   bool fine = false;
   PipelineNeighbour beside;
   const void* image = nullptr;
+  bool compact = false;
 };
 
 constexpr int kMidBox = 256;
diff --git a/semantic_meshes_amd/csrc/context.cpp b/semantic_meshes_amd/csrc/context.cpp
--- a/semantic_meshes_amd/csrc/context.cpp
+++ b/semantic_meshes_amd/csrc/context.cpp
@@ -72,6 +72,17 @@
     const char* e = getenv("SMESH_RASTER_MESHLETS");
     v = e ? (atoi(e) != 0 ? 1 : 0) : kRasterMeshletsDefault;
     g_raster_meshlets.store(v);
+  }
+  return v != 0;
+}
+
+static std::atomic<int> g_compact_records{-1};
+bool opt_compact_records() {
+  int v = g_compact_records.load();
+  if (v < 0) {
+    const char* e = getenv("SMESH_COMPACT_RECORDS");
+    v = e ? (atoi(e) != 0 ? 1 : 0) : kCompactRecordsDefault;
+    g_compact_records.store(v);
   }
   return v != 0;
 }
@@ -332,6 +343,7 @@
 void smesh_last_fuse_instance(int* slot, int* views);
 uint32_t smesh_last_fuse_lds_pad();
 int smesh_last_fuse_beside();
+int smesh_last_record_format();
 int smesh_last_fuse_probs_dtype();
 
 extern "C" {
@@ -344,6 +356,7 @@
   if (!name) return fail(SMESH_ERR_INVALID, "option name is NULL");
   if (!strcmp(name, "group_pipeline")) { g_group_pipeline.store(value != 0 ? 1 : 0); return SMESH_OK; }
   if (!strcmp(name, "raster_meshlets")) { g_raster_meshlets.store(value != 0 ? 1 : 0); return SMESH_OK; }
+  if (!strcmp(name, "compact_records")) { g_compact_records.store(value != 0 ? 1 : 0); return SMESH_OK; }
   if (!strcmp(name, "pipeline_fit")) { g_pipeline_fit.store(value != 0 ? 1 : 0); return SMESH_OK; }
   if (!strcmp(name, "pipeline_fuse_waves")) { g_pipeline_fuse_waves.store((int)std::min<int64_t>(32, std::max<int64_t>(2, value))); return SMESH_OK; }
   if (!strcmp(name, "pipeline_fuse_pad")) { g_pipeline_fuse_pad.store((int)std::min<int64_t>(65536 - 16384, std::max<int64_t>(-1, value))); return SMESH_OK; }
@@ -358,6 +371,8 @@
   if (!name || !value) return fail(SMESH_ERR_INVALID, "NULL argument");
   if (!strcmp(name, "group_pipeline")) { *value = opt_group_pipeline() ? 1 : 0; return SMESH_OK; }
   if (!strcmp(name, "raster_meshlets")) { *value = opt_raster_meshlets() ? 1 : 0; return SMESH_OK; }
+  if (!strcmp(name, "compact_records")) { *value = opt_compact_records() ? 1 : 0; return SMESH_OK; }
+  if (!strcmp(name, "last_record_format")) { *value = (int64_t)smesh_last_record_format(); return SMESH_OK; }
   if (!strcmp(name, "pipeline_fit")) { *value = opt_pipeline_fit(); return SMESH_OK; }
   if (!strcmp(name, "pipeline_fuse_waves")) { *value = opt_pipeline_fuse_waves(); return SMESH_OK; }
   if (!strcmp(name, "pipeline_fuse_pad")) { *value = opt_pipeline_fuse_pad(); return SMESH_OK; }
diff --git a/semantic_meshes_amd/csrc/fuse_mid.inc.hpp b/semantic_meshes_amd/csrc/fuse_mid.inc.hpp
--- a/semantic_meshes_amd/csrc/fuse_mid.inc.hpp
+++ b/semantic_meshes_amd/csrc/fuse_mid.inc.hpp
@@ -66,7 +66,7 @@
     if (jsel >= 0) {
       const TriView& w = vw.v[jsel];
       e.fi = w.big_queue[(uint64_t)a.big_capacity + qq];
-      e.rec = w.frags[e.fi];
+      e.rec = full_records(a, w.frags)[e.fi];
       e.view = jsel;
     }
     return e;
diff --git a/semantic_meshes_amd/csrc/fuse_tri.inc.hpp b/semantic_meshes_amd/csrc/fuse_tri.inc.hpp
--- a/semantic_meshes_amd/csrc/fuse_tri.inc.hpp
+++ b/semantic_meshes_amd/csrc/fuse_tri.inc.hpp
@@ -295,7 +295,41 @@
   return w * h <= kMidBox;
 }
 
-template <int CT, int KIND, bool EXACT, int NV>
+__device__ __forceinline__ const TriFrag* full_records(const TriFuseArgs& a, const TriFrag* __restrict__ frags) {
+  return a.compact ? reinterpret_cast<const TriFrag*>(reinterpret_cast<const char*>(frags) + rec_full_offset(a.F)) : frags;
+}
+template <int FORMAT>
+__device__ __forceinline__ TriFrag load_record(const TriFuseArgs& a, const TriFrag* __restrict__ frags, const uint32_t f) {
+  if (FORMAT == 0 || (FORMAT == 2 && !a.compact)) return frags[f];
+  const unsigned long long w = reinterpret_cast<const unsigned long long*>(frags)[f];
+  const uint32_t kind = rec_kind(w);
+  if (kind >= 2u) return full_records(a, frags)[f];
+  TriFrag r;
+  r.x0 = (uint16_t)rec_x0(w); r.y0 = (uint16_t)rec_y0(w); r.kind = (uint16_t)kind; r.pad = 0;
+  r.mask = kind == 1u ? rec_word_mask64(w) : 0ull;
+  return r;
+}
+template <int NV, bool MIDK>
+__device__ __forceinline__ void load_compact_views(const TriFuseArgs& a, const TriViews<NV>& vw, const uint64_t f, uint32_t (&org)[NV],
+                                                   unsigned long long (&msk)[NV], bool& big, bool& large) {
+#pragma unroll
+  for (int v = 0; v < NV; v++) msk[v] = reinterpret_cast<const unsigned long long*>(vw.v[v].frags)[f];
+#pragma unroll
+  for (int v = 0; v < NV; v++) {
+    const unsigned long long w = msk[v];
+    const uint32_t kind = rec_kind(w);
+    org[v] = rec_x0(w) | (rec_y0(w) << 16);
+    msk[v] = kind == 1u ? rec_word_mask64(w) : 0ull;
+    if (kind >= 2u) {
+      const TriFrag rec = full_records(a, vw.v[v].frags)[f];
+      msk[v] = rec.kind == 1 ? rec.mask : 0ull;
+      big = big || rec.kind == 2;
+      large = large || (rec.kind == 2 && !(MIDK && a.mid && mid_box(rec, 0u, 0u)));
+    }
+  }
+}
+
+template <int CT, int KIND, bool EXACT, int NV, int FORMAT>
 __device__ __forceinline__ void fuse_big_triangles(const TriFuseArgs& a, const TriViews<NV>& vw, uint32_t worker, uint32_t nworkers,
                                                    uint32_t* __restrict__ lds_list) {
   uint32_t len[NV], total = 0u;
@@ -324,7 +358,7 @@
 #pragma unroll
         for (int i = 0; i < NV; i++) {
           if (i <= jsel) {
-            const TriFrag rec = vw.v[i].frags[fi];
+            const TriFrag rec = load_record<FORMAT>(a, vw.v[i].frags, fi);
             const bool counts = rec.kind == 2 && !(a.mid && mid_box(rec, vw.v[i].W, vw.v[i].H));
             if (i < jsel) earlier = earlier || counts;
             else mine = counts;
@@ -341,7 +375,7 @@
       const uint32_t f = a.prim_id ? a.prim_id[fq] : fq;
 #pragma unroll
       for (int j = 0; j < NV; j++) {
-        const TriFrag rec = vw.v[j].frags[fq];
+        const TriFrag rec = load_record<FORMAT>(a, vw.v[j].frags, fq);
         if (rec.kind == 0 || (a.mid && rec.kind == 2 && mid_box(rec, 0u, 0u))) continue;
         const TriFuseArgs x = with_view(a, vw.v[j]);
         int x1, y1;
@@ -369,7 +403,12 @@
     const uint32_t tail = blockIdx.x - a.tri_blocks;
     if (tail < a.big_blocks) {
       uint32_t* lds_list = reinterpret_cast<uint32_t*>(srow);
-      fuse_big_triangles<CT, KIND, EXACT, NV>(a, vw, tail, a.big_blocks, lds_list);
+      if constexpr (fuse_tri_min_waves(CT, KIND, NV) > 1) {
+        if (a.compact) fuse_big_triangles<CT, KIND, EXACT, NV, 1>(a, vw, tail, a.big_blocks, lds_list);
+        else fuse_big_triangles<CT, KIND, EXACT, NV, 0>(a, vw, tail, a.big_blocks, lds_list);
+      } else {
+        fuse_big_triangles<CT, KIND, EXACT, NV, 2>(a, vw, tail, a.big_blocks, lds_list);
+      }
     } else if constexpr (KIND != SMESH_AGG_MUL) {
       constexpr int MCT = (CT + 7) / 8 * 8;
       fuse_mid_entries<MCT, KIND, NV>(a, vw, tail - a.big_blocks, gridDim.x - a.tri_blocks - a.big_blocks, (lds_u16*)srow);
@@ -383,7 +422,9 @@
   bool big = false, large = false;
 #pragma unroll
   for (int v = 0; v < NV; v++) { org[v] = 0u; msk[v] = 0ull; }
-  if (f < a.F) {
+  if (f < a.F && a.compact) {
+    load_compact_views<NV, KIND != SMESH_AGG_MUL>(a, vw, f, org, msk, big, large);
+  } else if (f < a.F) {
 #pragma unroll
     for (int v = 0; v < NV; v++) {
       const TriFrag rec = vw.v[v].frags[f];
diff --git a/semantic_meshes_amd/csrc/fusion.hip b/semantic_meshes_amd/csrc/fusion.hip
--- a/semantic_meshes_amd/csrc/fusion.hip
+++ b/semantic_meshes_amd/csrc/fusion.hip
@@ -2112,6 +2112,8 @@
   return a->C <= 40u || (a->C <= (uint32_t)kFuseTriMaxC && a->kind == SMESH_AGG_MUL && smesh_aggregator_max_fused_views(a) <= 2);
 }
 
+bool smesh_aggregator_reads_compact_records(smesh_aggregator* a) { return smesh_aggregator_fuses_small_views_by_mask(a); }
+
 bool smesh_aggregator_takes_strided_probs(smesh_aggregator* a, int64_t ps0, int64_t ps1, int nviews) {
   if (ps0 <= 0 || ps1 <= 0 || ps0 > 0xFFFFFFFFll || ps1 > 0xFFFFFFFFll) return false;
   return a->C <= kFuseTriMaxC && !(a->C > 40u && nviews > 2);
@@ -2188,6 +2190,10 @@
     else tri_ct = a->C <= 8 ? 8 : a->C <= 16 ? 16 : a->C <= 24 ? 24 : a->C <= 32 ? 32 : a->C <= 40 ? 41 : 48;
   }
   const bool specialised = tri_ct != 0;
+  t.compact = views[0].compact ? 1u : 0u;
+  for (int v = 1; v < nviews; v++)
+    if (views[v].compact != views[0].compact) return fail(SMESH_ERR_INVALID, "fuse_triangles: views with different record formats in one launch");
+  if (t.compact && (!specialised || prim_id)) return fail(SMESH_ERR_INVALID, "fuse_triangles: compact records need k_fuse_tri and the caller's face order");
   float* pw = nullptr;
   uint32_t* amax = nullptr;
   uint64_t scratch_stride = N;
diff --git a/semantic_meshes_amd/csrc/raster.hip b/semantic_meshes_amd/csrc/raster.hip
--- a/semantic_meshes_amd/csrc/raster.hip
+++ b/semantic_meshes_amd/csrc/raster.hip
@@ -26,6 +26,7 @@
 bool smesh_aggregator_takes_strided_probs(smesh_aggregator* a, int64_t ps0, int64_t ps1, int nviews);
 int smesh_aggregator_dense_probs(smesh_aggregator* a, const float* d_probs, const int64_t ps[3], uint64_t W, uint64_t H, const float** out);
 bool smesh_aggregator_fuses_small_views_by_mask(smesh_aggregator* a);
+bool smesh_aggregator_reads_compact_records(smesh_aggregator* a);
 int smesh_aggregator_fuse_triangles(smesh_aggregator* a, uint64_t F, const uint32_t* prim_id, uint32_t big_capacity,
                                     const RenderedView* views, int nviews, int part = 0, int nparts = 1);
 void smesh_fuse_part_rows(uint64_t F, int part, int nparts, uint64_t* f_lo, uint64_t* f_hi);
@@ -247,6 +248,7 @@
   uint32_t* huge_queue;
   uint32_t* big_count;
   uint32_t big_capacity;
+  uint32_t compact;
   TriFrag* frags;
   uint8_t* kinds;
   FragQueues q;
@@ -260,6 +262,17 @@
 };
 
 __device__ __forceinline__ uint64_t key_index(uint32_t x, uint32_t y, uint32_t H) { return (uint64_t)x * H + y; }
+
+__device__ __forceinline__ TriFrag* full_records(const RasterArgs& a) {
+  return a.compact ? reinterpret_cast<TriFrag*>(reinterpret_cast<char*>(a.frags) + rec_full_offset(a.F)) : a.frags;
+}
+__device__ __forceinline__ unsigned long long* record_words(const RasterArgs& a) { return reinterpret_cast<unsigned long long*>(a.frags); }
+
+__device__ __forceinline__ void store_compact_record(const RasterArgs& a, const uint64_t f, const TriFrag& rec, const bool wide) {
+  const uint32_t kind = rec_kind_of(rec.kind, wide ? 8 : 1, 1);
+  record_words(a)[f] = rec_pack(rec.x0, rec.y0, kind, rec.mask);
+  if (kind >= 2u) full_records(a)[f] = rec;
+}
 
 __device__ __forceinline__ ScreenVertex screen_vertex(const RasterArgs& a, const int32_t i) {
   if (a.sv) return a.sv[i];
@@ -703,8 +716,7 @@
   const int lane = threadIdx.x & 63;
   const int part = kSpreadMode ? part_in : -1;
   const bool owner = part <= 0 && !listed;
-  TriFrag rec;
-  rec.x0 = 0; rec.y0 = 0; rec.kind = 0; rec.pad = 0; rec.mask = 0ull;
+  bool placed = false, boxed = false;
   Tri t;
   t.x0 = 0; t.y0 = 0; t.x1 = -1; t.y1 = -1;
   unsigned long long cover = 0ull;
@@ -717,13 +729,12 @@
   else { if (f < a.F) have = load_tri_ex<NULLABLE_SV>(a, f, t, i0, i1, i2); }
   if (have) {
     const int bw = t.x1 - t.x0 + 1, bh = t.y1 - t.y0 + 1;
-    rec.x0 = (uint16_t)t.x0; rec.y0 = (uint16_t)t.y0;
+    placed = true;
     CX0 = t.x0; CY0 = t.y0;
     if (bw > 8 || bh > 8 || have == 2) {
       q_big = owner;
       q_mid = owner && bw * bh <= kMidBox;
-      rec.kind = 2;
-      rec.mask = (unsigned long long)(uint32_t)t.x1 | ((unsigned long long)(uint32_t)t.y1 << 16);
+      boxed = true;
       if (bw <= kLaneBox && bh <= kLaneBox && have == 1) {
         if (part < 0) lanebox = true;
         else {
@@ -793,12 +804,21 @@
   }
   {
     const unsigned long long mask = emit_cover<kTex>(a, t, f, pid, CX0, CY0, cover, sub);
-    if (mask && small) rec.kind = 1;
-    if (rec.kind == 1) rec.mask = mask;
+    small = small && mask != 0ull;
+    cover = mask;
   }
   if (owner) {
-    if (a.frags && f < a.F && (rec.kind != 0 || !a.kinds)) a.frags[f] = rec;
-    if (a.kinds && f < a.F) a.kinds[f] = (uint8_t)rec.kind;
+    TriFrag rec;
+    rec.x0 = placed ? (uint16_t)t.x0 : (uint16_t)0; rec.y0 = placed ? (uint16_t)t.y0 : (uint16_t)0; rec.pad = 0;
+    rec.kind = boxed ? 2 : (small ? 1 : 0);
+    rec.mask = boxed ? ((unsigned long long)(uint32_t)t.x1 | ((unsigned long long)(uint32_t)t.y1 << 16)) : (small ? cover : 0ull);
+    const bool wide = small && (t.x1 - t.x0 >= kRecBox || t.y1 - t.y0 >= kRecBox);
+    if (a.compact) {
+      if (f < a.F) store_compact_record(a, f, rec, wide);
+    } else {
+      if (a.frags && f < a.F && (rec.kind != 0 || !a.kinds)) a.frags[f] = rec;
+      if (a.kinds && f < a.F) a.kinds[f] = (uint8_t)rec.kind;
+    }
   }
   if constexpr (kWgPush && !kSpreadMode) {
     if (a.balance >= 2u) {
@@ -1016,7 +1036,7 @@
     const uint32_t qi = qb + (uint32_t)t;
     if (qi < nbig) {
       const uint32_t f = a.huge_queue[qi];
-      const TriFrag rec = a.frags[f];
+      const TriFrag rec = full_records(a)[f];
       const int bx1 = (int)(rec.mask & 0xFFFFu), by1 = (int)((rec.mask >> 16) & 0xFFFFu);
       if (rec.kind == 2 && (int)rec.x0 <= tx1 && bx1 >= (int)x0 && (int)rec.y0 <= ty1 && by1 >= (int)y0)
         s_hits[atomicAdd(&s_nhits, 1u)] = f;
@@ -1122,10 +1142,22 @@
       auto lost = [&](const unsigned long long key, const uint32_t pin) {
         if (key == kNullKey || skeys[pin] == key) return;
         const uint32_t f = (uint32_t)(key & 0xFFFFFFFFull);
-        const TriFrag rec = a.frags[f];
+        TriFrag* __restrict__ full = a.frags;
+        if (a.compact) {
+          const unsigned long long w = record_words(a)[f];
+          const uint32_t kind = rec_kind(w);
+          if (kind == 1u) {
+            const int bit = rec_bit((int)(x0 + (pin >> 6) - rec_x0(w)), (int)(y0 + (pin & 63u) - rec_y0(w)));
+            atomicAnd(&record_words(a)[f], ~(1ull << bit));
+            return;
+          }
+          if (kind != 3u) return;
+          full = full_records(a);
+        }
+        const TriFrag rec = full[f];
         if (rec.kind != 1) return;
         const int bit = (int)(x0 + (pin >> 6) - rec.x0) * 8 + (int)(y0 + (pin & 63u) - rec.y0);
-        atomicAnd(&a.frags[f].mask, ~(1ull << bit));
+        atomicAnd(&full[f].mask, ~(1ull << bit));
       };
 #pragma unroll
       for (uint32_t k = 0; k < kSpec; k++)
@@ -1292,6 +1324,7 @@
     uint32_t* big_queue = nullptr;
     uint32_t* big_count = nullptr;
     TriFrag* frags = nullptr;
+    bool compact = false;
     uint8_t* kinds = nullptr;
   } side[kSides];
   uint32_t big_capacity = 0;
@@ -1400,6 +1433,14 @@
   return smesh_aggregator_fuses_small_views_by_mask(a) ? 2 : 1;
 }
 
+bool compact_records_wanted(smesh_renderer* r, smesh_aggregator* a, const smesh_camera_t* cams, int n) {
+  if (!opt_compact_records() || !plane_optional_allowed(r) || plane_optional_level(r, a) != 2 || !smesh_aggregator_reads_compact_records(a)) return false;
+  for (int v = 0; v < n; v++)
+    if (!rec_image_fits(cams[v].width, cams[v].height)) return false;
+  return true;
+}
+thread_local int g_last_record_format = 16;
+
 constexpr uint32_t kRasterXcdRun = 8;
 
 uint64_t frag_cap_forced() {
@@ -1492,6 +1533,7 @@
     a.balance = (vs.med_queue && (knob >= 0 ? knob != 0 : (cam && depth_spread(r, cam) > 6.0))) ? (nviews > 1 ? 1u : 2u) : 0u;
   }
   a.frags = r->side[side].frags;
+  a.compact = 0u;
   a.kinds = r->side[side].kinds;
   a.q = FragQueues();
   a.idx_optional = 0u;
@@ -1518,9 +1560,11 @@
 }
 
 int render_into(smesh_renderer* r, const smesh_camera_t* cam, uint32_t* d_idx, float* d_depth, hipStream_t st = nullptr,
-                int side = 0, int idx_optional = 0) {
+                int side = 0, int idx_optional = 0, bool compact = false) {
   DeviceCtx* ctx = r->ctx;
   r->last_render_side = side;
+  r->side[side].compact = false;
+  g_last_record_format = 16;
   if (!st) {
     st = ctx->stream;
     SMESH_TRY(main_after_raster(r));
@@ -1546,6 +1590,11 @@
     int qs = SMESH_OK;
     if (raster_path() == RasterPath::Frag && ensure_queues(r, vs, W, H, st, &qs)) {
       a.q = vs.fq;
+      if (compact && a.idx_optional == 2u && a.frags && !a.kinds) {
+        a.compact = 1u;
+        r->side[side].compact = true;
+        g_last_record_format = 8;
+      }
       {
         const uint32_t nblocks = (uint32_t)div_up(div_up(r->F, a.tpw), 4);
         const uint32_t chunk = nblocks >= 64u ? kRasterXcdRun : 0u;
@@ -1639,9 +1688,11 @@
 }
 
 int render_group_into(smesh_renderer* r, const smesh_camera_t* cams, int n, hipStream_t st, int base = 0, int side_base = -1,
-                      int idx_optional = 0, bool with_depth = false) {
+                      int idx_optional = 0, bool with_depth = false, bool compact = false) {
   if (side_base < 0) side_base = base;
   if (!plane_optional_allowed(r) || with_depth) idx_optional = 0;
+  compact = compact && idx_optional == 2 && !r->texels;
+  g_last_record_format = compact ? 8 : 16;
   DeviceCtx* ctx = r->ctx;
   ProjectGroup pg;
   RasterGroup rg;
@@ -1670,6 +1721,8 @@
     rg.view[v].cam = pg.cam[v];
     rg.view[v].q = vs.fq;
     rg.view[v].idx_optional = (uint32_t)idx_optional;
+    rg.view[v].compact = compact ? 1u : 0u;
+    r->side[side_base + v].compact = compact;
     rg.idx[v] = static_cast<uint32_t*>(r->fused[side_base + v].ptr);
     tiles += (uint32_t)(div_up(W, kQW) * div_up(H, kQH));
     rg.tile_end[v] = tiles;
@@ -1783,7 +1836,7 @@
   if (sd.frags) return hipSuccess;
   hipError_t e = dev_malloc(reinterpret_cast<void**>(&sd.big_queue), (size_t)r->big_capacity * 8);
   if (e == hipSuccess) e = dev_malloc(reinterpret_cast<void**>(&sd.big_count), 32);
-  if (e == hipSuccess) e = dev_malloc(reinterpret_cast<void**>(&sd.frags), std::max<uint64_t>(r->F * sizeof(TriFrag), 16));
+  if (e == hipSuccess) e = dev_malloc(reinterpret_cast<void**>(&sd.frags), std::max<uint64_t>(r->texels ? r->F * sizeof(TriFrag) : rec_alloc_bytes(r->F), 16));
   if (e == hipSuccess && r->texels) e = dev_malloc(reinterpret_cast<void**>(&sd.kinds), std::max<uint64_t>(r->F, 16));
   if (e == hipSuccess) e = hipMemsetAsync(sd.big_count, 0, 32, r->ctx->stream);
   if (e == hipSuccess) e = hipStreamSynchronize(r->ctx->stream);
@@ -1990,6 +2043,7 @@
                                   bool mid_queue) {
   RenderedView rv{sd.frags, sd.big_queue, sd.big_count, d_idx, in.probs(), d_w, W, H, in.ps0, in.ps1, mid_queue};
   if (in.kind != ViewInput::F32) rv.image = in.image;
+  rv.compact = sd.compact;
   return rv;
 }
 
@@ -2051,7 +2105,8 @@
     SMESH_HIP(hipStreamSynchronize(ctx->stream));
   }
   if (!r->texels && smesh_aggregator_can_fuse_triangles(a, r->F)) {
-    const RenderedView rv{r->side[slot].frags, r->side[slot].big_queue, r->side[slot].big_count, d_idx, d_probs, d_w, W, H, ps0, ps1, true};
+    RenderedView rv{r->side[slot].frags, r->side[slot].big_queue, r->side[slot].big_count, d_idx, d_probs, d_w, W, H, ps0, ps1, true};
+    rv.compact = r->side[slot].compact;
     SMESH_TRY(smesh_aggregator_fuse_triangles(a, r->F, r->prim_id, r->big_capacity, &rv, 1));
     smesh_note_fuse(smesh_aggregator_fuse_kernel_name(a, r->prim_id != nullptr), "render-records");
   } else if (r->texels && smesh_aggregator_can_fuse_texels(a, r->num_primitives)) {
@@ -2069,6 +2124,9 @@
 const char* smesh_last_fuse_kernel(void) { return g_last_fuse_kernel; }
 const char* smesh_last_add_path(void) { return g_last_add_path; }
 const char* smesh_last_raster_path(void) { return g_last_raster_path; }
+}
+int smesh_last_record_format() { return g_last_record_format; }
+extern "C" {
 
 int smesh_renderer_create_triangles(const float* vertices, uint64_t V, const int32_t* faces, uint64_t F, int device,
                                     smesh_renderer_t** out) {
@@ -2312,7 +2370,8 @@
   uint32_t* d_idx = static_cast<uint32_t*>(r->fused[slot].ptr);
   r->last_idx[slot] = nullptr; r->rec_valid[slot] = false;
   const int tri_path = scans_all_planes(r, a, in.kind, N) ? kLabelsPlaneLevel : plane_optional_level(r, a);
-  SMESH_TRY(render_into(r, cam, d_idx, nullptr, ctx->stream, slot, tri_path));
+  const bool compact = in.kind == ViewInput::F32 && tri_path == 2 && compact_records_wanted(r, a, cam, 1);
+  SMESH_TRY(render_into(r, cam, d_idx, nullptr, ctx->stream, slot, tri_path, compact));
   SMESH_TRY(fuse_rendered(r, a, slot, d_idx, in, weights, memkind, W, H));
   r->fused_seq++;
   return SMESH_OK;
@@ -2369,6 +2428,7 @@
       r->main_pending = true;
     }
     const bool group_pipeline = group_pipeline_on;
+    const bool compact = grouped && !own_kernel && tri_path == 2 && compact_records_wanted(r, a, &cams[i], gn);
     int base = 0;
     if (use_pipeline) {
       const int bank = (int)(r->group_seq++ & 1u);
@@ -2385,13 +2445,13 @@
         r->main_pending = false;
       }
       if (!r->bank_used[bank ^ 1]) SMESH_TRY(prepare_group_slots(r, &cams[i], gn, ctx->raster_stream, (bank ^ 1) * kMaxGroup));
-      SMESH_TRY(render_group_into(r, &cams[i], gn, ctx->raster_stream, base, -1, tri_path));
+      SMESH_TRY(render_group_into(r, &cams[i], gn, ctx->raster_stream, base, -1, tri_path, false, compact));
       SMESH_HIP(hipEventRecord(r->ev_bank_rendered[bank], ctx->raster_stream));
       SMESH_HIP(hipStreamWaitEvent(ctx->stream, r->ev_bank_rendered[bank], 0));
       r->bank_used[bank] = true;
       r->raster_pending = true;
     } else if (grouped) {
-      SMESH_TRY(render_group_into(r, &cams[i], gn, ctx->stream, 0, -1, tri_path));
+      SMESH_TRY(render_group_into(r, &cams[i], gn, ctx->stream, 0, -1, tri_path, false, compact));
     } else {
       gn = 2;
       SMESH_HIP(alloc_side(r, 1));
diff --git a/semantic_meshes_amd/csrc/records.hpp b/semantic_meshes_amd/csrc/records.hpp
--- /dev/null
+++ b/semantic_meshes_amd/csrc/records.hpp
@@ -0,0 +1,51 @@
+#pragma once
+
+#include <cstddef>
+#include <cstdint>
+
+#if defined(__HIPCC__)
+#define SMESH_REC_HD __host__ __device__ inline
+#else
+#define SMESH_REC_HD inline
+#endif
+
+namespace smesh {
+
+constexpr int kRecBox = 6;
+constexpr uint32_t kRecMaxImage = 8192;
+constexpr uint64_t kRecMask36 = (1ull << 36) - 1ull;
+
+SMESH_REC_HD bool rec_image_fits(uint64_t W, uint64_t H) { return W <= kRecMaxImage && H <= kRecMaxImage; }
+
+SMESH_REC_HD uint64_t rec_full_offset(uint64_t F) { return (F * 8ull + 255ull) & ~255ull; }
+SMESH_REC_HD uint64_t rec_alloc_bytes(uint64_t F) { return rec_full_offset(F) + F * 16ull; }
+
+SMESH_REC_HD uint32_t rec_kind_of(uint32_t kind16, int bw, int bh) {
+  if (kind16 != 1u) return kind16;
+  return (bw > kRecBox || bh > kRecBox) ? 3u : 1u;
+}
+
+SMESH_REC_HD uint64_t rec_mask36(uint64_t m64) {
+  const uint32_t lo = (uint32_t)m64 & 0x00FFFFFFu, hi = (uint32_t)(m64 >> 24) & 0x00FFFFFFu;
+  const uint32_t a = (lo & 0x3Fu) | ((lo >> 2) & 0xFC0u) | ((lo >> 4) & 0x3F000u);
+  const uint32_t b = (hi & 0x3Fu) | ((hi >> 2) & 0xFC0u) | ((hi >> 4) & 0x3F000u);
+  return (uint64_t)a | ((uint64_t)b << 18);
+}
+SMESH_REC_HD uint64_t rec_mask64(uint64_t m36) {
+  const uint32_t a = (uint32_t)m36 & 0x3FFFFu, b = (uint32_t)(m36 >> 18) & 0x3FFFFu;
+  const uint32_t lo = (a & 0x3Fu) | ((a & 0xFC0u) << 2) | ((a & 0x3F000u) << 4);
+  const uint32_t hi = (b & 0x3Fu) | ((b & 0xFC0u) << 2) | ((b & 0x3F000u) << 4);
+  return (uint64_t)lo | ((uint64_t)hi << 24);
+}
+
+SMESH_REC_HD uint64_t rec_pack(uint32_t x0, uint32_t y0, uint32_t kind, uint64_t mask64) {
+  return (kind == 1u ? rec_mask36(mask64) : 0ull) | ((uint64_t)(x0 & 0x1FFFu) << 36) | ((uint64_t)(y0 & 0x1FFFu) << 49) | ((uint64_t)(kind & 3u) << 62);
+}
+SMESH_REC_HD uint32_t rec_kind(uint64_t w) { return (uint32_t)(w >> 62); }
+SMESH_REC_HD uint32_t rec_x0(uint64_t w) { return (uint32_t)(w >> 36) & 0x1FFFu; }
+SMESH_REC_HD uint32_t rec_y0(uint64_t w) { return (uint32_t)(w >> 49) & 0x1FFFu; }
+SMESH_REC_HD uint64_t rec_word_mask64(uint64_t w) { return rec_mask64(w & kRecMask36); }
+
+SMESH_REC_HD int rec_bit(int dx, int dy) { return dx * kRecBox + dy; }
+
+}
```

New measurement: 19270 views/s, median of 6. 7.7% higher.
